# joedownard/skill-chaining-with-graphs

Hardware: AMD Instinct MI355X
Metric: env-steps/sec (whole node), 65 536 parallel Pinball envs at 1/2/4/8 MI355X (higher is better)
Workload: dtype f32

## Files before the change

### include/scg_abi.h

```cpp
#ifndef SCG_ABI_H
#define SCG_ABI_H
#include <stdint.h>

#ifdef __cplusplus
extern "C" {
#endif

#define SCG_ABI_VERSION 5
#define SCG_NUM_ACTIONS 5
#define SCG_FOURIER_ORDER 5
#define SCG_NUM_FEATURES 1296
#define SCG_MAX_OPTIONS 5
#define SCG_MAX_EDGES 256
#define SCG_CLF_STRIDE 8

typedef enum {
    SCG_OK = 0,
    SCG_ERR_INVALID = -1,
    SCG_ERR_NO_DEVICE = -2,
    SCG_ERR_HIP = -3,
    SCG_ERR_STATE = -4,
    SCG_ERR_ASYNC = -5
} scg_status;

typedef struct scg_ctx scg_ctx;

typedef struct {
    int32_t n_envs;
    int32_t n_options;
    int32_t fourier_order;
    int32_t device;
    int64_t env_id_base;
    uint64_t seed;
    float gamma, alpha, epsilon, r_option_success;
    int32_t max_episode_steps, max_option_steps;
    int32_t update_count_floor;
    int32_t reoffer_period;
} scg_config;

#define SCG_STEP_LEARN 1u
#define SCG_STEP_APPLY 2u
#define SCG_STEP_INTERRUPT 4u

int scg_abi_version(void);
int scg_block_envs(void);
const char *scg_strerror(int status);
const char *scg_last_error(const scg_ctx *ctx);

int scg_create(scg_ctx **out, const scg_config *cfg);
int scg_destroy(scg_ctx *ctx);
int scg_set_hparams(scg_ctx *ctx, float gamma, float alpha, float epsilon, float r_option_success,
                    int32_t max_episode_steps, int32_t max_option_steps, int32_t update_count_floor, int32_t reoffer_period);

int scg_set_map(scg_ctx *ctx, const float *edges, int32_t n_edges, const float *starts, int32_t n_starts,
                const float map_scalars[6], const float *scale);

int scg_step(scg_ctx *ctx, float *x, float *y, float *vx, float *vy, int32_t *option_id,
             int32_t *opt_steps, int32_t *ep_steps, float *qcache, uint8_t *action, float *reward,
             uint8_t *done, float *W, const float *clf, uint32_t enabled_mask, uint64_t t,
             uint32_t flags, void *stream);

typedef struct {
    float *ep_return;
    double *ret_sum;
    int32_t *episodes, *goals, *len_sum;
    int32_t *vf_steps, *entries, *declines, *successes;
    uint8_t *finished;
} scg_rollout_stats;
#define SCG_ROLLOUT_BEGIN 1u
#define SCG_ROLLOUT_ONE_EPISODE 2u
#define SCG_ROLLOUT_MAX_STEPS 1024
int scg_rollout(scg_ctx *ctx, float *x, float *y, float *vx, float *vy, int32_t *option_id, int32_t *opt_steps,
                int32_t *ep_steps, float *qcache, uint8_t *action, float *reward, uint8_t *done,
                const float *W, const float *clf, uint32_t enabled_mask, uint64_t t0, int32_t n_steps,
                uint32_t flags, const scg_rollout_stats *stats, void *stream);

typedef struct {
    uint8_t *outcome;
    int32_t *steps;
    float *ret, *disc_ret, *v0, *end_x, *end_y, *end_vx, *end_vy;
} scg_trial_out;
#define SCG_TRIAL_SUCCESS 1u
#define SCG_TRIAL_EPISODE_END 2u
#define SCG_TRIAL_LEFT_INITIATION 3u
#define SCG_TRIAL_TIMEOUT 4u
#define SCG_TRIAL_MAX_STEPS SCG_ROLLOUT_MAX_STEPS
int scg_option_trials(scg_ctx *ctx, int32_t n, const float *x, const float *y, const float *vx, const float *vy,
                      const int32_t *option, const float *W, const float *clf, uint32_t enabled_mask, uint64_t t0,
                      const scg_trial_out *out, void *stream);

typedef struct {
    int32_t first, n, rows;
    int32_t *len;
    float *x, *y, *vx, *vy, *reward;
    uint8_t *action, *done, *vf, *term;
    int8_t *option_id;
} scg_record;
#define SCG_ROLLOUT_BEGIN_AT 4u
int scg_rollout_record(scg_ctx *ctx, float *x, float *y, float *vx, float *vy, int32_t *option_id, int32_t *opt_steps,
                       int32_t *ep_steps, float *qcache, uint8_t *action, float *reward, uint8_t *done,
                       const float *W, const float *clf, uint32_t enabled_mask, uint64_t t0, int32_t n_steps,
                       uint32_t flags, const scg_rollout_stats *stats, const scg_record *rec, void *stream);
int scg_option_trials_record(scg_ctx *ctx, int32_t n, const float *x, const float *y, const float *vx, const float *vy,
                             const int32_t *option, const float *W, const float *clf, uint32_t enabled_mask, uint64_t t0,
                             const scg_trial_out *out, const scg_record *rec, void *stream);

#define SCG_ROLLOUT_TERM_INTERRUPTED 5u
int scg_rollout_interrupt(scg_ctx *ctx, float *x, float *y, float *vx, float *vy, int32_t *option_id, int32_t *opt_steps,
                          int32_t *ep_steps, float *qcache, uint8_t *action, float *reward, uint8_t *done,
                          const float *W, const float *clf, uint32_t enabled_mask, uint64_t t0, int32_t n_steps,
                          uint32_t flags, const scg_rollout_stats *stats, int32_t *interrupts, const scg_record *rec,
                          void *stream);

int scg_grad_buffers(scg_ctx *ctx, float **G, int32_t **n_k);
int scg_set_grad_buffers(scg_ctx *ctx, float *G, int32_t *n_k);
int scg_apply_update(scg_ctx *ctx, float *W, const float *G, const int32_t *n_k, void *stream);
int scg_set_grad_buffer_packed(scg_ctx *ctx, float *G_packed);
int scg_apply_update_packed(scg_ctx *ctx, float *W, const float *G_packed, void *stream);
int scg_apply_update_slots(scg_ctx *ctx, float *W, const float *slots, int32_t n_slots, int64_t slot_stride, void *stream);

int scg_peer_export(scg_ctx *ctx, void *handle_out);
int scg_peer_open(scg_ctx *ctx, int32_t n_ranks, int32_t rank, const void *handles);
int scg_peer_exchange_apply(scg_ctx *ctx, float *W, void *stream);


int scg_pinball_step(scg_ctx *ctx, int32_t n, float *x, float *y, float *vx, float *vy,
                     const uint8_t *action, float *reward, uint8_t *goal, void *stream);
int scg_fourier_features(scg_ctx *ctx, int32_t n, const float *x, const float *y, const float *vx,
                         const float *vy, float *phi, void *stream);
int scg_q_values(scg_ctx *ctx, int32_t n, const float *x, const float *y, const float *vx,
                 const float *vy, const float *Wk, float *q, void *stream);
int scg_q_update(scg_ctx *ctx, int32_t n, int32_t k, const float *x, const float *y, const float *vx,
                 const float *vy, const uint8_t *action, const float *r, const float *cont,
                 const float *xn, const float *yn, const float *vxn, const float *vyn, float *W,
                 uint32_t flags, void *stream);
int scg_classifier_predict(scg_ctx *ctx, int32_t n, const float *x, const float *y, const float *w8,
                           uint8_t *out, void *stream);
int scg_fit_initiation(scg_ctx *ctx, int32_t n_fit, const float *xy, const uint8_t *label,
                       const int32_t *offsets, float *w, int32_t iters, float lr, float l2, void *stream);

int scg_set_option_parents(scg_ctx *ctx, const int32_t *parents);

int scg_invalidate_order(scg_ctx *ctx);

int scg_set_trace_buffers(scg_ctx *ctx, float *ring_x, float *ring_y, int32_t ring_len, uint8_t *events,
                          int32_t *ev_len);
int scg_harvest(scg_ctx *ctx, int32_t n_sel, const int32_t *sel_env, const float *ring_x, const float *ring_y,
                int32_t ring_len, const int32_t *ev_len, int32_t l_pos, int32_t l_neg, float *out_xy,
                uint8_t *out_label, void *stream);

int scg_collect_examples(scg_ctx *ctx, uint32_t event_bits, uint8_t *prev_in, int32_t l_pos, int32_t l_neg,
                         float *ex_xy, uint8_t *ex_label, int32_t *count, int32_t cap, void *stream);
int scg_arm_collect(scg_ctx *ctx, uint32_t event_bits, const uint8_t *prev_in, int32_t l_pos, int32_t l_neg, const int32_t *count);
int scg_collect_frontier(scg_ctx *ctx, uint32_t target_mask, uint32_t cover_mask, const float *clf, int32_t l_pos, int32_t l_neg,
                         float *ex_xy, uint8_t *ex_label, int32_t *count, int32_t cap, void *stream);

int scg_set_gestation(scg_ctx *ctx, uint32_t gest_mask, int32_t *succ_counts);

#define SCG_ASYNC_FIT_TIMEOUT 0x1u
#define SCG_ASYNC_STEP_HANDOFF 0x2u
#define SCG_ASYNC_PEER_TIMEOUT 0x4u
int scg_async_status(scg_ctx *ctx, void *stream, int32_t synchronize, uint32_t *word_out);
int scg_clear_async_error(scg_ctx *ctx);
int scg_set_fit_timeout(scg_ctx *ctx, double seconds);
int scg_set_peer_timeout(scg_ctx *ctx, double seconds);
int scg_decode_async_word(uint32_t word, char *buf, int32_t buf_len);
int scg_debug_raise_async(scg_ctx *ctx, uint32_t word);

int scg_profile_reset(scg_ctx *ctx, int32_t enable);
int scg_profile_read(scg_ctx *ctx, double *kernel_ms_sum, int64_t *launches);

#ifdef __cplusplus
}
#endif
#endif
```

### skill-chaining-with-graphs_amd/_lib.py

```python
from __future__ import annotations

import ctypes as C
import os

_HERE = os.path.dirname(os.path.abspath(__file__))
LIB_PATH = os.environ.get("SCG_LIB") or os.path.join(_HERE, "csrc", "libscg_hip.so")

NUM_ACTIONS = 5
FOURIER_ORDER = 5
NUM_FEATURES = 1296
MAX_OPTIONS = 5
MAX_EDGES = 256
CLF_STRIDE = 8

STEP_LEARN = 1
STEP_APPLY = 2
STEP_INTERRUPT = 4
ROLLOUT_BEGIN = 1
ROLLOUT_ONE_EPISODE = 2
ROLLOUT_BEGIN_AT = 4
ROLLOUT_MAX_STEPS = 1024
TRIAL_SUCCESS = 1
TRIAL_EPISODE_END = 2
TRIAL_LEFT_INITIATION = 3
TRIAL_TIMEOUT = 4
TRIAL_MAX_STEPS = ROLLOUT_MAX_STEPS
ROLLOUT_TERM_INTERRUPTED = 5
ABI_VERSION = 5
ASYNC_FIT_TIMEOUT = 0x1
ASYNC_STEP_HANDOFF = 0x2
ASYNC_PEER_TIMEOUT = 0x4
PEER_HANDLE_BYTES = 64
PEER_MAX_RANKS = 8


class ScgError(RuntimeError):
    pass


class ScgConfig(C.Structure):
    _fields_ = [
        ("n_envs", C.c_int32),
        ("n_options", C.c_int32),
        ("fourier_order", C.c_int32),
        ("device", C.c_int32),
        ("env_id_base", C.c_int64),
        ("seed", C.c_uint64),
        ("gamma", C.c_float),
        ("alpha", C.c_float),
        ("epsilon", C.c_float),
        ("r_option_success", C.c_float),
        ("max_episode_steps", C.c_int32),
        ("max_option_steps", C.c_int32),
        ("update_count_floor", C.c_int32),
        ("reoffer_period", C.c_int32),
    ]


class RolloutStats(C.Structure):
    _fields_ = [
        ("ep_return", C.c_void_p),
        ("ret_sum", C.c_void_p),
        ("episodes", C.c_void_p),
        ("goals", C.c_void_p),
        ("len_sum", C.c_void_p),
        ("vf_steps", C.c_void_p),
        ("entries", C.c_void_p),
        ("declines", C.c_void_p),
        ("successes", C.c_void_p),
        ("finished", C.c_void_p),
    ]


class TrialOut(C.Structure):
    _fields_ = [
        ("outcome", C.c_void_p),
        ("steps", C.c_void_p),
        ("ret", C.c_void_p),
        ("disc_ret", C.c_void_p),
        ("v0", C.c_void_p),
        ("end_x", C.c_void_p),
        ("end_y", C.c_void_p),
        ("end_vx", C.c_void_p),
        ("end_vy", C.c_void_p),
    ]


class Record(C.Structure):
    _fields_ = [
        ("first", C.c_int32),
        ("n", C.c_int32),
        ("rows", C.c_int32),
        ("len", C.c_void_p),
        ("x", C.c_void_p),
        ("y", C.c_void_p),
        ("vx", C.c_void_p),
        ("vy", C.c_void_p),
        ("reward", C.c_void_p),
        ("action", C.c_void_p),
        ("done", C.c_void_p),
        ("vf", C.c_void_p),
        ("term", C.c_void_p),
        ("option_id", C.c_void_p),
    ]


_P = C.c_void_p
_SIGS = {
    "scg_abi_version": (C.c_int, []),
    "scg_block_envs": (C.c_int, []),
    "scg_strerror": (C.c_char_p, [C.c_int]),
    "scg_last_error": (C.c_char_p, [_P]),
    "scg_create": (C.c_int, [C.POINTER(_P), C.POINTER(ScgConfig)]),
    "scg_destroy": (C.c_int, [_P]),
    "scg_set_hparams": (C.c_int, [_P, C.c_float, C.c_float, C.c_float, C.c_float, C.c_int32, C.c_int32, C.c_int32, C.c_int32]),
    "scg_set_map": (C.c_int, [_P, _P, C.c_int32, _P, C.c_int32, _P, _P]),
    "scg_step": (C.c_int, [_P] + [_P] * 13 + [C.c_uint32, C.c_uint64, C.c_uint32, _P]),
    "scg_rollout": (C.c_int, [_P] + [_P] * 13 + [C.c_uint32, C.c_uint64, C.c_int32, C.c_uint32, C.POINTER(RolloutStats), _P]),
    "scg_option_trials": (C.c_int, [_P, C.c_int32] + [_P] * 7 + [C.c_uint32, C.c_uint64, C.POINTER(TrialOut), _P]),
    "scg_rollout_record": (C.c_int, [_P] + [_P] * 13 + [C.c_uint32, C.c_uint64, C.c_int32, C.c_uint32, C.POINTER(RolloutStats),
                                                         C.POINTER(Record), _P]),
    "scg_option_trials_record": (C.c_int, [_P, C.c_int32] + [_P] * 7 + [C.c_uint32, C.c_uint64, C.POINTER(TrialOut),
                                                                       C.POINTER(Record), _P]),
    "scg_rollout_interrupt": (C.c_int, [_P] + [_P] * 13 + [C.c_uint32, C.c_uint64, C.c_int32, C.c_uint32, C.POINTER(RolloutStats),
                                                            _P, C.POINTER(Record), _P]),
    "scg_grad_buffers": (C.c_int, [_P, C.POINTER(_P), C.POINTER(_P)]),
    "scg_set_grad_buffers": (C.c_int, [_P, _P, _P]),
    "scg_apply_update": (C.c_int, [_P, _P, _P, _P, _P]),
    "scg_set_grad_buffer_packed": (C.c_int, [_P, _P]),
    "scg_apply_update_packed": (C.c_int, [_P, _P, _P, _P]),
    "scg_apply_update_slots": (C.c_int, [_P, _P, _P, C.c_int32, C.c_int64, _P]),
    "scg_pinball_step": (C.c_int, [_P, C.c_int32] + [_P] * 7 + [_P]),
    "scg_fourier_features": (C.c_int, [_P, C.c_int32] + [_P] * 5 + [_P]),
    "scg_q_values": (C.c_int, [_P, C.c_int32] + [_P] * 6 + [_P]),
    "scg_q_update": (C.c_int, [_P, C.c_int32, C.c_int32] + [_P] * 12 + [C.c_uint32, _P]),
    "scg_classifier_predict": (C.c_int, [_P, C.c_int32] + [_P] * 4 + [_P]),
    "scg_set_option_parents": (C.c_int, [_P, _P]),
    "scg_invalidate_order": (C.c_int, [_P]),
    "scg_set_trace_buffers": (C.c_int, [_P, _P, _P, C.c_int32, _P, _P]),
    "scg_harvest": (C.c_int, [_P, C.c_int32, _P, _P, _P, C.c_int32, _P, C.c_int32, C.c_int32, _P, _P, _P]),
    "scg_collect_examples": (C.c_int, [_P, C.c_uint32, _P, C.c_int32, C.c_int32, _P, _P, _P, C.c_int32, _P]),
    "scg_arm_collect": (C.c_int, [_P, C.c_uint32, _P, C.c_int32, C.c_int32, _P]),
    "scg_collect_frontier": (C.c_int, [_P, C.c_uint32, C.c_uint32, _P, C.c_int32, C.c_int32, _P, _P, _P, C.c_int32, _P]),
    "scg_set_gestation": (C.c_int, [_P, C.c_uint32, _P]),
    "scg_profile_reset": (C.c_int, [_P, C.c_int32]),
    "scg_profile_read": (C.c_int, [_P, C.POINTER(C.c_double), C.POINTER(C.c_int64)]),
    "scg_fit_initiation": (C.c_int, [_P, C.c_int32, _P, _P, _P, _P, C.c_int32, C.c_float, C.c_float, _P]),
    "scg_async_status": (C.c_int, [_P, _P, C.c_int32, C.POINTER(C.c_uint32)]),
    "scg_clear_async_error": (C.c_int, [_P]),
    "scg_set_fit_timeout": (C.c_int, [_P, C.c_double]),
    "scg_set_peer_timeout": (C.c_int, [_P, C.c_double]),
    "scg_peer_export": (C.c_int, [_P, _P]),
    "scg_peer_open": (C.c_int, [_P, C.c_int32, C.c_int32, _P]),
    "scg_peer_exchange_apply": (C.c_int, [_P, _P, _P]),
    "scg_decode_async_word": (C.c_int, [C.c_uint32, C.c_char_p, C.c_int32]),
    "scg_debug_raise_async": (C.c_int, [_P, C.c_uint32]),
}
EXPORTED_SYMBOLS = tuple(_SIGS)

BLOCK_ENVS_DEFAULT = 256
BLOCK_ENVS_BUILDS = (64, 128, 256)

CHIP_CUS = 256


def auto_block_envs(n_envs: int) -> int:
    for b in BLOCK_ENVS_BUILDS:
        if -(-int(n_envs) // b) <= CHIP_CUS:
            return b
    return BLOCK_ENVS_DEFAULT


_libs = {}


def lib_path(block_envs: int | None = None) -> str:
    if block_envs in (None, BLOCK_ENVS_DEFAULT):
        return LIB_PATH
    if block_envs not in BLOCK_ENVS_BUILDS:
        raise ScgError(f"block_envs must be one of {BLOCK_ENVS_BUILDS}")
    return os.path.join(_HERE, "csrc", f"libscg_hip_b{block_envs}.so")


def load(block_envs: int | None = None, path: str | None = None) -> C.CDLL:
    key = (BLOCK_ENVS_DEFAULT if block_envs is None else int(block_envs)) if path is None else os.path.abspath(path)
    if key in _libs:
        return _libs[key]
    if path is None:
        path = lib_path(key)
    if not os.path.exists(path):
        raise ScgError(
            f"{path} is missing: the HIP extension has not been built "
            "(run `python -c 'import __graft_entry__ as g; g.build()'` or `make -C "
            f"{os.path.dirname(path)}`). There is no CPU fallback."
        )
    lib = C.CDLL(path)
    try:
        ver = int(lib.scg_abi_version())
    except AttributeError:
        raise ScgError(f"{path} does not export scg_abi_version: not a libscg_hip.so") from None
    if ver != ABI_VERSION:
        raise ScgError(f"{path} implements ABI version {ver}, this binding expects {ABI_VERSION} "
                       "(include/scg_abi.h): rebuild the library (a stale .so?)")
    for name, (res, args) in _SIGS.items():
        try:
            fn = getattr(lib, name)
        except AttributeError:
            raise ScgError(f"{path} does not export {name} although it reports ABI version {ver}: rebuild it") from None
        fn.restype = res
        fn.argtypes = args
    if block_envs is not None and isinstance(key, int) and int(lib.scg_block_envs()) != key:
        raise ScgError(f"{path} is built for {int(lib.scg_block_envs())}-env blocks, not {key}: rebuild it")
    _libs[key] = lib
    return lib


def block_envs(block_envs: int | None = None) -> int:
    return int(load(block_envs).scg_block_envs())


def check(status: int, ctx=None, what: str = "") -> None:
    if status == 0:
        return
    lib = load()
    msg = lib.scg_last_error(ctx).decode() if True else ""
    raise ScgError(f"{what or 'scg call'} failed ({lib.scg_strerror(status).decode()}): {msg}")
```

### skill-chaining-with-graphs_amd/core.py

```python
from __future__ import annotations

import ctypes as C
import os
from typing import Optional, Sequence

import numpy as np
import torch

from . import _lib
from ._lib import (CLF_STRIDE, MAX_OPTIONS, NUM_ACTIONS, NUM_FEATURES, STEP_APPLY, STEP_INTERRUPT, STEP_LEARN, ScgConfig,
                   ScgError)
from .maps import PinballMap


def fourier_scale_table(order: int = 5, n_vars: int = 4) -> np.ndarray:
    n = order + 1
    idx = np.arange(n ** n_vars)
    c = np.stack([(idx // n ** (n_vars - 1 - d)) % n for d in range(n_vars)], 1).astype(np.float64)
    norm = np.sqrt((c * c).sum(1))
    norm[0] = 1.0
    return (1.0 / norm).astype(np.float32)


def _ptr(t: Optional[torch.Tensor]) -> C.c_void_p:
# ... 259 lines not shown
        self._chk(count, torch.int32, 1, "count")
        if prev_in is not None:
            self._chk(prev_in, torch.uint8, self.n_envs, "prev_in")
        if l_pos < 0 or l_neg < 0 or l_pos + l_neg < 1 or not (0 < event_bits < 64):
            raise ScgError("collect_examples: bad argument")
        self._call("scg_collect_examples", C.c_uint32(event_bits), _ptr(prev_in), l_pos, l_neg, _ptr(ex_xy), _ptr(ex_label),
                   _ptr(count), cap, self._stream())
        if rearm:
            self._call("scg_arm_collect", C.c_uint32(event_bits), _ptr(prev_in), l_pos, l_neg, _ptr(count))
            self._armed = (prev_in, count)
        else:
            self.disarm_collect()

    def collect_frontier(self, target_mask: int, cover_mask: int, clf: torch.Tensor, l_pos: int, l_neg: int,
                         ex_xy: torch.Tensor, ex_label: torch.Tensor, count: torch.Tensor) -> None:
        if getattr(self, "_trace", None) is None:
            raise ScgError("collect_frontier: trace buffers are not attached (set_trace_buffers)")
        cap = ex_label.numel() // self.n_vf
        if cap < 1 or ex_label.numel() != self.n_vf * cap:
            raise ScgError(f"collect_frontier: ex_label must hold n_vf = {self.n_vf} buffers of cap >= 1 examples")
        self._chk(ex_xy, torch.float32, 2 * self.n_vf * cap, "ex_xy"); self._chk(ex_label, torch.uint8, self.n_vf * cap, "ex_label")
        self._chk(count, torch.int32, self.n_vf, "count"); self._chk(clf, torch.float32, self.n_vf * CLF_STRIDE, "clf")
        nodes = (1 << self.n_vf) - 1
        if l_pos < 0 or l_neg < 0 or l_pos + l_neg < 1 or not (0 <= target_mask <= nodes) or not (0 <= cover_mask <= nodes) \
                or cover_mask & 1 or target_mask & ~cover_mask & ~1:
            raise ScgError("collect_frontier: bad argument")
        self._call("scg_collect_frontier", C.c_uint32(target_mask), C.c_uint32(cover_mask), _ptr(clf), l_pos, l_neg, _ptr(ex_xy),
                   _ptr(ex_label), _ptr(count), cap, self._stream())

    def disarm_collect(self) -> None:
        self._call("scg_arm_collect", C.c_uint32(0), None, 0, 0, None)
        self._armed = None

    def set_gestation(self, gest_mask: int) -> torch.Tensor:
        if not hasattr(self, "_gest_succ"):
            self._gest_succ = torch.zeros(self.n_vf, dtype=torch.int32, device=self.device)
        self._call("scg_set_gestation", C.c_uint32(gest_mask), _ptr(self._gest_succ))
        self.gest_mask = gest_mask
        return self._gest_succ

    def grad_buffers(self):
        if not hasattr(self, "_gbuf"):
            G = torch.zeros((self.n_vf, NUM_ACTIONS, NUM_FEATURES), dtype=torch.float32, device=self.device)
            n = torch.zeros((self.n_vf,), dtype=torch.int32, device=self.device)
            self._call("scg_set_grad_buffers", _ptr(G), _ptr(n))
            self._gbuf = (G, n)
            self.__dict__.pop("_gpacked", None)
        return self._gbuf

    def grad_packed(self) -> torch.Tensor:
        if not hasattr(self, "_gpacked"):
            gp = torch.zeros(self.n_vf * NUM_ACTIONS * NUM_FEATURES + self.n_vf, dtype=torch.float32, device=self.device)
            self._call("scg_set_grad_buffer_packed", _ptr(gp))
            self._gpacked = gp
            self.__dict__.pop("_gbuf", None)
        return self._gpacked

    def apply_update_packed(self, W: torch.Tensor, gp: torch.Tensor) -> None:
        self._chk(W, torch.float32, self.n_vf * NUM_ACTIONS * NUM_FEATURES, "W")
        self._chk(gp, torch.float32, self.n_vf * NUM_ACTIONS * NUM_FEATURES + self.n_vf, "G_packed")
        self._call("scg_apply_update_packed", _ptr(W), _ptr(gp), self._stream())

    def apply_update_slots(self, W: torch.Tensor, slots: torch.Tensor) -> None:
        per = self.n_vf * NUM_ACTIONS * NUM_FEATURES + self.n_vf
        if slots.dim() != 2 or slots.shape[1] != per or not slots.is_contiguous():
            raise ScgError(f"slots must be a contiguous [n_ranks, {per}] tensor")
        self._chk(W, torch.float32, self.n_vf * NUM_ACTIONS * NUM_FEATURES, "W")
        self._chk(slots, torch.float32, slots.shape[0] * per, "slots")
        self._call("scg_apply_update_slots", _ptr(W), _ptr(slots), C.c_int32(slots.shape[0]), C.c_int64(per), self._stream())

    def apply_update(self, W: torch.Tensor, G: torch.Tensor, n_k: torch.Tensor) -> None:
        self._chk(W, torch.float32, self.n_vf * NUM_ACTIONS * NUM_FEATURES, "W")
        self._chk(G, torch.float32, self.n_vf * NUM_ACTIONS * NUM_FEATURES, "G")
        self._chk(n_k, torch.int32, self.n_vf, "n_k")
        self._call("scg_apply_update", _ptr(W), _ptr(G), _ptr(n_k), self._stream())

    def _chk4(self, s: Sequence[torch.Tensor], n: int, name: str):
        if len(s) != 4:
            raise ScgError(f"{name}: need (x, y, vx, vy)")
        return [self._chk(t, torch.float32, n, f"{name}[{i}]") for i, t in enumerate(s)]

    def pinball_step(self, s, action: torch.Tensor):
        n = s[0].numel()
        x, y, vx, vy = self._chk4(s, n, "state")
        self._chk(action, torch.uint8, n, "action")
        if n and int(action.max()) >= NUM_ACTIONS:
            raise ScgError("action out of range [0, 5)")
        reward = torch.empty(n, dtype=torch.float32, device=self.device)
        goal = torch.empty(n, dtype=torch.uint8, device=self.device)
        self._call("scg_pinball_step", n, _ptr(x), _ptr(y), _ptr(vx), _ptr(vy), _ptr(action), _ptr(reward),
                   _ptr(goal), self._stream())
        return reward, goal

    def features(self, s) -> torch.Tensor:
        n = s[0].numel()
        x, y, vx, vy = self._chk4(s, n, "state")
        phi = torch.empty((n, NUM_FEATURES), dtype=torch.float32, device=self.device)
        self._call("scg_fourier_features", n, _ptr(x), _ptr(y), _ptr(vx), _ptr(vy), _ptr(phi), self._stream())
        return phi

    def q_values(self, s, Wk: torch.Tensor) -> torch.Tensor:
        n = s[0].numel()
        x, y, vx, vy = self._chk4(s, n, "state")
        self._chk(Wk, torch.float32, NUM_ACTIONS * NUM_FEATURES, "Wk")
        q = torch.empty((NUM_ACTIONS, n), dtype=torch.float32, device=self.device)
        self._call("scg_q_values", n, _ptr(x), _ptr(y), _ptr(vx), _ptr(vy), _ptr(Wk), _ptr(q), self._stream())
        return q

    def q_update(self, k: int, s, action, r, cont, sn, W: torch.Tensor, apply: bool = True) -> None:
        n = s[0].numel()
        if n > self.n_envs:
            raise ScgError("q_update: more transitions than the context's n_envs")
        x, y, vx, vy = self._chk4(s, n, "s")
        xn, yn, vxn, vyn = self._chk4(sn, n, "s_next")
        self._chk(action, torch.uint8, n, "action"); self._chk(r, torch.float32, n, "r")
        self._chk(cont, torch.float32, n, "cont")
        self._chk(W, torch.float32, self.n_vf * NUM_ACTIONS * NUM_FEATURES, "W")
        if n and int(action.max()) >= NUM_ACTIONS:
            raise ScgError("action out of range [0, 5)")
        self._call("scg_q_update", n, k, _ptr(x), _ptr(y), _ptr(vx), _ptr(vy), _ptr(action), _ptr(r), _ptr(cont),
                   _ptr(xn), _ptr(yn), _ptr(vxn), _ptr(vyn), _ptr(W), C.c_uint32(STEP_APPLY if apply else 0),
                   self._stream())

    def classifier_predict(self, x: torch.Tensor, y: torch.Tensor, w8: torch.Tensor) -> torch.Tensor:
        n = x.numel()
        self._chk(x, torch.float32, n, "x"); self._chk(y, torch.float32, n, "y")
        self._chk(w8, torch.float32, CLF_STRIDE, "w8")
        out = torch.empty(n, dtype=torch.uint8, device=self.device)
        self._call("scg_classifier_predict", n, _ptr(x), _ptr(y), _ptr(w8), _ptr(out), self._stream())
        return out

    def fit_initiation(self, xy: torch.Tensor, label: torch.Tensor, offsets: torch.Tensor, w: torch.Tensor,
                       iters: int = 200, lr: float = 1.0, l2: float = 1e-4) -> None:
        n_fit = offsets.numel() - 1
        self._chk(offsets, torch.int32, n_fit + 1, "offsets")
        off = offsets.cpu()
        m = int(off[-1])
        if n_fit < 0 or int(off[0]) != 0 or bool((off[1:] < off[:-1]).any()):
            raise ScgError("offsets must start at 0 and be non-decreasing")
        self._chk(xy, torch.float32, 2 * m, "xy"); self._chk(label, torch.uint8, m, "label")
        self._chk(w, torch.float32, n_fit * CLF_STRIDE, "w")
        self._call("scg_fit_initiation", n_fit, _ptr(xy), _ptr(label), _ptr(offsets), _ptr(w), iters,
                   C.c_float(lr), C.c_float(l2), self._stream())
        self.async_status(synchronize=True)

    def async_status(self, synchronize: bool = False) -> int:
        word = C.c_uint32(0)
        self._call("scg_async_status", self._stream(), 1 if synchronize else 0, C.byref(word))
        return int(word.value)

    def clear_async_error(self) -> None:
        self._call("scg_clear_async_error")

    def set_fit_timeout(self, seconds: float) -> None:
        self._call("scg_set_fit_timeout", C.c_double(seconds))

    def peer_export(self) -> bytes:
        buf = C.create_string_buffer(_lib.PEER_HANDLE_BYTES)
        self._call("scg_peer_export", C.cast(buf, C.c_void_p))
        return buf.raw

    def peer_open(self, n_ranks: int, rank: int, handles) -> None:
        handles = [bytes(h) for h in handles]
        if len(handles) != n_ranks or any(len(h) != _lib.PEER_HANDLE_BYTES for h in handles):
            raise ScgError(f"peer_open: need {n_ranks} handles of {_lib.PEER_HANDLE_BYTES} bytes")
        blob = C.create_string_buffer(b"".join(handles), n_ranks * _lib.PEER_HANDLE_BYTES)
        self._call("scg_peer_open", C.c_int32(n_ranks), C.c_int32(rank), C.cast(blob, C.c_void_p))
        self.peer_ranks = int(n_ranks)

    def peer_exchange_apply(self, W: torch.Tensor) -> None:
        self._chk(W, torch.float32, self.n_vf * NUM_ACTIONS * NUM_FEATURES, "W")
        self._call("scg_peer_exchange_apply", _ptr(W), self._stream())

    def set_peer_timeout(self, seconds: float) -> None:
        self._call("scg_set_peer_timeout", C.c_double(seconds))

    @property
    def step_grid(self) -> int:
        return -(-self.n_envs // self.block_envs)


class EnvState:

    def __init__(self, n: int, device: torch.device, pmap: PinballMap):
        z = lambda dt: torch.zeros(n, dtype=dt, device=device)
        sx, sy = float(pmap.starts[0][0]), float(pmap.starts[0][1])
        self.n = n
        self.x = torch.full((n,), sx, dtype=torch.float32, device=device)
        self.y = torch.full((n,), sy, dtype=torch.float32, device=device)
        self.vx, self.vy = z(torch.float32), z(torch.float32)
        self.option_id, self.opt_steps, self.ep_steps = z(torch.int32), z(torch.int32), z(torch.int32)
        self.qcache = torch.zeros((NUM_ACTIONS, n), dtype=torch.float32, device=device)
        self.action, self.done = z(torch.uint8), z(torch.uint8)
        self.reward = z(torch.float32)

    def state(self):
        return (self.x, self.y, self.vx, self.vy)
```

### skill-chaining-with-graphs_amd/csrc/scg_kernels.hip

```cpp
#include "scg_device.hpp"
#include "../../include/scg_abi.h"
#include <cstdio>
#include <cstdlib>
#include <cstring>
#include <cmath>
#include <mutex>
#include <new>
#include <type_traits>
#include <vector>

using namespace scg;
typedef float f4v __attribute__((ext_vector_type(4)));
typedef unsigned u4v __attribute__((ext_vector_type(4)));

template <typename T>
__device__ __forceinline__ void gstore(T *p, T v) { *p = v; }

__device__ __forceinline__ void store_wt(float *p, f4v v) {
    asm volatile("global_store_dwordx4 %0, %1, off sc1\n\ts_nop 2" :: "v"(p), "v"(v) : "memory");
}

constexpr int OREC = 4;

struct StepArgs {
    float *x, *y, *vx, *vy;
    int32_t *option_id, *opt_steps, *ep_steps;
    int32_t *hist_next;
    float4 *qalt;
    float4 *outrec;
    float *qcache;
    uint8_t *action;
    float *reward;
    uint8_t *done;
    const float *cont_in;
    const float *xn, *yn, *vxn, *vyn;
    const float *W;
    const float *clf;
    const float *edges;
    const uint64_t *cellmask;
    const int32_t *perm;
    float *ring_x, *ring_y;
    uint8_t *events;
    int32_t *ev_len;
    int32_t ring_mask;
    const float *starts;
    float *slabs;
    int32_t *cnts;
    unsigned long long *stamps;
    uint32_t *async_word;
    int32_t *fail_flag;
    int32_t n, n_vf, k_lo, k_hi;
    uint32_t enabled, learn;
    uint32_t gest;
    int32_t *gest_succ;
    uint32_t parents;
    uint64_t t, seed;
    int64_t env_base;
    float gamma, epsilon, r_succ;
    int32_t max_ep, max_opt;
    uint32_t reoffer_mask;
    MapScalars ms;
};

__device__ __forceinline__ void block_lds_sync() {
    asm volatile("s_waitcnt lgkmcnt(0)\n\ts_barrier" ::: "memory");
}

__device__ __forceinline__ bool in_set(const StepArgs &A, int k, float x, float y) {
    if (k < 1 || k >= A.n_vf) return false;
    if (!((A.enabled >> k) & 1u)) return false;
    return clf_z(A.clf + CLF_STRIDE * k, x, y) > 0.0f;
}

#include "scg_eval.hpp"
#include "scg_step_kernel.hpp"
#include "scg_rollout_kernel.hpp"
#include "scg_trial_kernel.hpp"

__attribute__((visibility("hidden"))) hipError_t launch_rollout_record(const RolloutRecArgs &A, int grid, hipStream_t s);
__attribute__((visibility("hidden"))) hipError_t launch_trial_record(const TrialRecArgs &A, int grid, hipStream_t s);
__attribute__((visibility("hidden"))) hipError_t launch_rollout_interrupt(const RolloutIntArgs &A, int grid, hipStream_t s);
__attribute__((visibility("hidden"))) hipError_t launch_rollout_interrupt_record(const RolloutIntRecArgs &A, int grid, hipStream_t s);

struct ReduceArgs {
    const float *slabs;
    const int32_t *cnts;
    float *G;
    int32_t *n_k;
    float *nk_f;
    float *W;
    const float *scale;
    int32_t nblk, n_vf;
    float alpha;
    uint32_t apply;
    int32_t nk_floor;
    const int32_t *option_id;
    int32_t *hist, *hist_zero, *perm;
    int32_t n, nrow;
    const float4 *outrec;
    const float4 *qalt;
    int32_t *invperm;
    float *x, *y, *vx, *vy, *reward;
    int32_t *option_id_out, *opt_steps, *ep_steps;
    uint8_t *action, *done;
    float *qcache;
    int32_t sort;
    const int32_t *fail_flag;
    const uint8_t *c_events, *c_prev;
    const int32_t *c_evlen, *c_count;
    int32_t *c_rows;
    uint32_t c_bits;
    int32_t c_L, c_ring_len;
};

constexpr int SEG = 16;
constexpr int RED_WAVES = 16;
constexpr int RED_THREADS = 64 * RED_WAVES;
constexpr int RED_SPW = 2;
constexpr int RED_COLS = NACT * NF / 4;
constexpr int RED_NCOL = (RED_COLS + 63) / 64;

__device__ __forceinline__ uint32_t div_magic(uint32_t d) { return 0xFFFFFFFFu / d + 1u; }
__device__ __forceinline__ int div_by(int r, int d, uint32_t m) { return d == 1 ? r : (int)__umulhi((uint32_t)r, m); }
__device__ __forceinline__ int collect_v(int e, int n, const uint8_t *events, const uint8_t *prev_in, uint32_t bits,
                                         const int32_t *ev_len, int ring_len, int L, bool &in_out);
constexpr int NKEY = 7, HSTRIDE = 8;
__device__ __forceinline__ int sort_key(int o, int n_vf) {
    if (o <= 0) return o > -n_vf ? 0 : n_vf;
    return o < n_vf ? o : n_vf;
}
struct OrderLayout {
    int chunked, c, g, U, Ftot;
    uint32_t mc, mg;
    int start[NKEY];
    int cnt[NKEY], n[NKEY], F[NKEY];
    int pad_lo[NKEY], pad_n[NKEY], pad_pos[NKEY], tail_lo, tail_pos;
};
__device__ __forceinline__ void order_layout(const int tot[NKEY], int n_envs, OrderLayout &L) {
    int S = 0, Rn = 0;
#pragma unroll
    for (int k = 1; k < NKEY; ++k) { S += tot[k]; Rn += tot[k] > 0 ? 1 : 0; L.n[k] = tot[k]; }
    L.n[0] = tot[0];
    const int Bf = n_envs / BLOCK_ENVS;
    int c = BLOCK_ENVS;
    if (Bf > Rn && S > 0) c = min(BLOCK_ENVS, (S + (Bf - Rn) - 1) / (Bf - Rn));
    int U = 0, F = 0;
    L.start[0] = 0; L.cnt[0] = 0; L.F[0] = 0;
    L.mc = div_magic((uint32_t)c);
    L.mg = div_magic((uint32_t)max(BLOCK_ENVS - c, 1));
#pragma unroll
    for (int k = 1; k < NKEY; ++k) {
        L.cnt[k] = div_by(tot[k] + c - 1, c, L.mc);
        L.start[k] = U * BLOCK_ENVS; L.F[k] = F;
        U += L.cnt[k]; F += L.cnt[k] * BLOCK_ENVS - tot[k];
    }
    L.c = c; L.g = BLOCK_ENVS - c; L.U = U; L.Ftot = F;
    L.chunked = (U * BLOCK_ENVS <= n_envs) ? 1 : 0;
    if (!L.chunked) {
        int P = 0, used = 0;
        L.c = 1 << 30;
        L.mc = div_magic(1u << 30);
        L.pad_lo[0] = 0; L.pad_n[0] = 0; L.pad_pos[0] = 0;
#pragma unroll
        for (int k = 1; k < NKEY; ++k) {
            L.start[k] = P; P += tot[k];
            const int need = tot[k] > 0 ? (BLOCK_ENVS - P % BLOCK_ENVS) % BLOCK_ENVS : 0;
            const int pad = min(need, tot[0] - used);
            L.pad_lo[k] = used; L.pad_n[k] = pad; L.pad_pos[k] = P; used += pad; P += pad;
        }
        L.tail_lo = used; L.tail_pos = P;
    }
}
__device__ __forceinline__ int order_posk(const OrderLayout &L, int start, int r) {
    const int t = div_by(r, L.c, L.mc);
    return start + BLOCK_ENVS * t + (r - t * L.c);
}
__device__ __forceinline__ int order_pos0(const OrderLayout &L, int r) {
    if (!L.chunked) {
        int pos = L.tail_pos + (r - L.tail_lo);
#pragma unroll
        for (int k = 1; k < NKEY; ++k)
            if (r >= L.pad_lo[k] && r < L.pad_lo[k] + L.pad_n[k]) pos = L.pad_pos[k] + (r - L.pad_lo[k]);
        return pos;
    }
    int pos = L.U * BLOCK_ENVS + (r - L.Ftot);
    int st = 0, cn = 0, nk = 0, f0 = 0;
    bool in_run = false;
#pragma unroll
    for (int k = 1; k < NKEY; ++k) {
        const int fills = L.cnt[k] * BLOCK_ENVS - L.n[k];
        if (r >= L.F[k] && r < L.F[k] + fills) { in_run = true; st = L.start[k]; cn = L.cnt[k]; nk = L.n[k]; f0 = L.F[k]; }
    }
    if (in_run) {
        const int rp = r - f0, nfull = cn - 1;
        if (L.g > 0 && rp < nfull * L.g) {
            const int t = div_by(rp, L.g, L.mg);
            pos = st + BLOCK_ENVS * t + L.c + (rp - t * L.g);
        } else {
            pos = st + BLOCK_ENVS * nfull + (nk - nfull * L.c) + (rp - nfull * L.g);
        }
    }
    return pos;
}

__device__ __forceinline__ void commit_and_place_row(const ReduceArgs &R, int row, int wv, int lane, int (*s_x)[40]) {
    int zoff = 0;
    asm volatile("" : "+v"(zoff));
    const int step_failed = R.fail_flag[zoff];
    const bool act = wv < 4 && row < R.nrow;
    const int e = row * 256 + wv * 64 + lane;
    const bool ok = act && e < R.n;
    const int pos_old = ok ? R.invperm[e] : 0;
    int tot[NKEY], pre[NKEY];
#pragma unroll
    for (int k = 0; k < NKEY; ++k) { tot[k] = 0; pre[k] = 0; }
    if (act && R.sort) {
        for (int r = wv * 64 + lane; r < R.nrow; r += 256) {
#pragma unroll
            for (int k = 0; k < NKEY; ++k) {
                const int h = R.hist[r * HSTRIDE + k];
                tot[k] += h;
                if (r < row) pre[k] += h;
            }
        }
    }
    float4 ra = make_float4(0.0f, 0.0f, 0.0f, 0.0f), rb = ra, rq = ra;
    float q4 = 0.0f;
    if (ok) {
        const float4 *r = R.outrec + (size_t)pos_old * OREC;
        const float4 r3 = r[3];
        ra = r[0]; rb = r[1]; rq = r[2]; q4 = r3.x;
        if (__float_as_uint(r3.y) == OREC_DECLINED) {
            rq = R.qalt[(size_t)pos_old * 2]; q4 = R.qalt[(size_t)pos_old * 2 + 1].x;
            rb.y = __uint_as_float(__float_as_uint(rb.y) | 0x01000000u);
        }
    }
    int key = -1;
    uint64_t km[NKEY];
    if (act) {
        if (R.sort) {
#pragma unroll
            for (int k = 0; k < NKEY; ++k) {
#pragma unroll
                for (int m = 1; m < 64; m <<= 1) { tot[k] += __shfl_xor(tot[k], m, 64); pre[k] += __shfl_xor(pre[k], m, 64); }
            }
        }
        const unsigned bits = __float_as_uint(rb.y);
        if (ok && !step_failed) {
            const int on = (int)((bits >> 16) & 255u);
            const bool declined = (bits >> 24) & 1u;
            const int oid = declined ? -on : (on ? on : -(int)((bits >> 28) & 7u));
            key = sort_key(oid, R.n_vf);
            R.x[e] = ra.x; R.y[e] = ra.y; R.vx[e] = ra.z; R.vy[e] = ra.w;
            R.reward[e] = rb.x; R.action[e] = (uint8_t)(bits & 255u); R.done[e] = (uint8_t)((bits >> 8) & 255u);
            R.option_id_out[e] = oid; R.opt_steps[e] = __float_as_int(rb.z); R.ep_steps[e] = __float_as_int(rb.w);
            if (R.qcache) {
                const size_t n = (size_t)R.n;
                R.qcache[e] = rq.x; R.qcache[n + e] = rq.y; R.qcache[2 * n + e] = rq.z;
                R.qcache[3 * n + e] = rq.w; R.qcache[4 * n + e] = q4;
            }
        }
        if (R.sort) {
#pragma unroll
            for (int k = 0; k < NKEY; ++k) km[k] = __ballot(key == k);
            if (lane < 3 * NKEY) {
                int v = 0;
#pragma unroll
                for (int k = 0; k < NKEY; ++k) {
                    if (lane == k) v = tot[k];
                    if (lane == NKEY + k) v = pre[k];
                    if (lane == 2 * NKEY + k) v = __popcll(km[k]);
                }
                s_x[wv][lane] = v;
            }
        }
    }
    if (R.c_rows && act) {
        bool in;
        int v = collect_v(e, R.n, R.c_events, R.c_prev, R.c_bits, R.c_evlen, R.c_ring_len, R.c_L, in);
#pragma unroll
        for (int m = 1; m < 64; m <<= 1) v += __shfl_xor(v, m, 64);
        if (lane == 0) s_x[wv][3 * NKEY] = v;
    }
    if (!R.sort && !R.c_rows) return;
    __syncthreads();
    if (R.c_rows && wv == 0 && lane == 0 && row < R.nrow) {
        R.c_rows[row] = s_x[0][3 * NKEY] + s_x[1][3 * NKEY] + s_x[2][3 * NKEY] + s_x[3][3 * NKEY];
        if (row == 0) R.c_rows[R.nrow] = *R.c_count;
    }
    if (!R.sort || !act) return;
    int off[NKEY];
#pragma unroll
    for (int k = 0; k < NKEY; ++k) {
        tot[k] = s_x[0][k] + s_x[1][k] + s_x[2][k] + s_x[3][k];
        off[k] = s_x[0][NKEY + k] + s_x[1][NKEY + k] + s_x[2][NKEY + k] + s_x[3][NKEY + k];
#pragma unroll
        for (int w = 0; w < 3; ++w) off[k] += w < wv ? s_x[w][2 * NKEY + k] : 0;
    }
    OrderLayout L;
    order_layout(tot, R.n, L);
    int rk = -1, st = 0;
#pragma unroll
    for (int k = 0; k < NKEY; ++k)
        if (key == k) { rk = off[k] + __popcll(km[k] & ((1ull << lane) - 1ull)); st = L.start[k]; }
    if (rk >= 0 && !step_failed) {
        const int pos = key == 0 ? order_pos0(L, rk) : order_posk(L, st, rk);
        R.perm[pos] = e; R.invperm[e] = pos;
    }
    if (wv == 0 && lane < HSTRIDE) R.hist_zero[row * HSTRIDE + lane] = 0;
}

template <int BATCH>
__global__ __launch_bounds__(RED_THREADS, BATCH == 16 ? 4 : 8) void reduce_kernel(const ReduceArgs R) {
    __shared__ float4 s_T[RED_WAVES * RED_SPW][64];
    __shared__ int s_cnt[RED_WAVES * RED_SPW];
    __shared__ int s_x[4][40];
    const int sy_rows = (int)gridDim.y - R.n_vf;
    const int k = (int)blockIdx.y >= sy_rows ? (int)blockIdx.y - sy_rows : -1;
    const int rowy = (int)blockIdx.y;
    const int tid = threadIdx.x, lane = tid & 63, wave = __builtin_amdgcn_readfirstlane(tid >> 6);
    if (k < 0) {
        const int row = rowy * (int)gridDim.x + blockIdx.x;
        commit_and_place_row(R, row, wave, lane, s_x);
        return;
    }
    const int i4 = blockIdx.x * 64 + lane;
    const bool live = i4 < RED_COLS;
    const size_t slab_stride = (size_t)R.n_vf * RED_COLS * sizeof(float4);
    const char *slab_k = reinterpret_cast<const char *>(R.slabs) + (size_t)k * RED_COLS * sizeof(float4);
    const unsigned col_off = (unsigned)(live ? i4 : 0) * (unsigned)sizeof(float4);
    const int nseg = (R.nblk + SEG - 1) / SEG;
    float4 S = make_float4(0.0f, 0.0f, 0.0f, 0.0f);
    int nk = 0;
    float4 w_old = make_float4(0.0f, 0.0f, 0.0f, 0.0f), sc = w_old;
    int step_failed = 0;
    for (int sg0 = 0; sg0 < nseg; sg0 += RED_WAVES * RED_SPW) {
        int cs[RED_SPW];
#pragma unroll
        for (int j = 0; j < RED_SPW; ++j) {
            const int bl = (sg0 + j * RED_WAVES + wave) * SEG + lane;
            cs[j] = (lane < SEG && bl < R.nblk) ? R.cnts[(unsigned)(bl * R.n_vf + k)] : 0;
        }
#pragma unroll
        for (int j = 0; j < RED_SPW; ++j) {
            const int b0 = (sg0 + j * RED_WAVES + wave) * SEG;
            int c = cs[j];
            const unsigned mask = (unsigned)__ballot(c > 0);
#pragma unroll
            for (int m = 1; m < SEG; m <<= 1) c += __shfl_xor(c, m, 64);
            float4 T = make_float4(0.0f, 0.0f, 0.0f, 0.0f);
            if (mask) {
                const __amdgpu_buffer_rsrc_t seg = __builtin_amdgcn_make_buffer_rsrc(
                    const_cast<char *>(slab_k + (size_t)b0 * slab_stride), 0, 0x7fffffff, 0x00020000);
#pragma unroll
                for (int h = 0; h < SEG; h += BATCH) {
                    if (!((mask >> h) & ((1u << BATCH) - 1u))) continue;
                    u4v v[BATCH];
#pragma unroll
                    for (int u = 0; u < BATCH; ++u) {
                        v[u] = (u4v){0u, 0u, 0u, 0u};
                        if ((mask >> (h + u)) & 1u) v[u] = __builtin_amdgcn_raw_buffer_load_b128(seg, (int)col_off, (int)((h + u) * (unsigned)slab_stride), 0);
                    }
#pragma unroll
                    for (int u = 0; u < BATCH; ++u) {
                        if ((mask >> (h + u)) & 1u) {
                            T.x = T.x + __uint_as_float(v[u][0]); T.y = T.y + __uint_as_float(v[u][1]);
                            T.z = T.z + __uint_as_float(v[u][2]); T.w = T.w + __uint_as_float(v[u][3]);
                        }
                    }
                }
            }
            s_T[j * RED_WAVES + wave][lane] = T;
            if (lane == 0) s_cnt[j * RED_WAVES + wave] = c;
        }
        if (wave == 0 && R.apply && sg0 + RED_WAVES * RED_SPW >= nseg) {
            step_failed = *R.fail_flag;
            int col = live ? i4 : 0;
            asm volatile("" : "+v"(col));
            w_old = reinterpret_cast<const float4 *>(R.W)[(size_t)k * RED_COLS + col];
            sc = *reinterpret_cast<const float4 *>(R.scale + (col * 4) % NF);
        }
        __syncthreads();
        if (wave == 0) {
#pragma unroll
            for (int u = 0; u < RED_WAVES * RED_SPW; ++u) {
                const int cu = s_cnt[u];
                if (cu > 0) {
                    const float4 t = s_T[u][lane];
                    S.x = S.x + t.x; S.y = S.y + t.y; S.z = S.z + t.z; S.w = S.w + t.w;
                    nk += cu;
                }
            }
        }
        __syncthreads();
    }
    if (wave != 0) return;
    if (blockIdx.x == 0 && lane == 0) {
        R.n_k[k] = nk;
        if (R.nk_f) R.nk_f[k] = (float)nk;
    }
    if (!live) return;
    reinterpret_cast<float4 *>(R.G)[(size_t)k * RED_COLS + i4] = S;
    if (R.apply && nk > 0 && !step_failed) {
        const float step = R.alpha / (float)max(nk, R.nk_floor);
        float4 w = w_old;
        w.x = fmaf(step * sc.x, S.x, w.x); w.y = fmaf(step * sc.y, S.y, w.y);
        w.z = fmaf(step * sc.z, S.z, w.z); w.w = fmaf(step * sc.w, S.w, w.w);
        int col = i4;
        asm volatile("" : "+v"(col));
        reinterpret_cast<float4 *>(R.W)[(size_t)k * RED_COLS + col] = w;
    }
}

__global__ __launch_bounds__(256) void commit_kernel(const ReduceArgs R) {
    __shared__ int s_x[4][40];
    commit_and_place_row(R, blockIdx.x, threadIdx.x >> 6, threadIdx.x & 63, s_x);
}

__global__ __launch_bounds__(256) void apply_kernel(float *W, const float *G, const int32_t *n_k, const float *nk_f,
                                                    const float *scale, float alpha, int nk_floor) {
    const int k = blockIdx.y;
    const int i = blockIdx.x * 256 + threadIdx.x;
    if (i >= NACT * NF) return;
    const int nk = n_k ? n_k[k] : (int)(nk_f[k] + 0.5f);
    if (nk <= 0) return;
    const float step = alpha / (float)max(nk, nk_floor);
    const int f = i % NF;
    float *w = W + (size_t)k * NACT * NF + i;
    *w = fmaf(step * scale[f], G[(size_t)k * NACT * NF + i], *w);
}

__global__ __launch_bounds__(256) void apply_slots_kernel(float *W, const float *slots, int n_slots, long stride, int n_vf,
                                                          const float *scale, float alpha, int nk_floor) {
    const int k = blockIdx.y;
    const int i = blockIdx.x * 256 + threadIdx.x;
    if (i >= NACT * NF) return;
    const size_t at = (size_t)k * NACT * NF + i, cnt_at = (size_t)n_vf * NACT * NF + k;
    float g = slots[at], nkf = slots[cnt_at];
    for (int r = 1; r < n_slots; ++r) {
        g = g + slots[(size_t)r * stride + at];
        nkf = nkf + slots[(size_t)r * stride + cnt_at];
    }
    const int nk = (int)(nkf + 0.5f);
    if (nk <= 0) return;
    const float step = alpha / (float)max(nk, nk_floor);
    float *w = W + at;
    *w = fmaf(step * scale[i % NF], g, *w);
}

constexpr int PEER_MAX = 8;
constexpr size_t PEER_HDR = 256;

struct PeerView {
    const float *buf[PEER_MAX][2];
    const uint32_t *epoch[PEER_MAX];
    const uint32_t *voidw[PEER_MAX];
};

__device__ __forceinline__ bool epoch_reached(uint32_t v, uint32_t need) { return (int32_t)(v - need) >= 0; }

__global__ __launch_bounds__(64) void peer_publish_kernel(uint32_t *epoch, uint32_t *voidw, int parity, const int32_t *fail,
                                                          uint32_t value) {
    if (threadIdx.x != 0) return;
    const int32_t f = __hip_atomic_load(fail, __ATOMIC_RELAXED, __HIP_MEMORY_SCOPE_AGENT);
    __hip_atomic_store(&voidw[parity], f ? 1u : 0u, __ATOMIC_RELAXED, __HIP_MEMORY_SCOPE_SYSTEM);
    __builtin_amdgcn_fence(__ATOMIC_RELEASE, "");
    asm volatile("s_waitcnt vmcnt(0)" ::: "memory");
    __hip_atomic_store(epoch, value, __ATOMIC_RELAXED, __HIP_MEMORY_SCOPE_SYSTEM);
}

__global__ __launch_bounds__(64) void peer_wait_kernel(const PeerView P, int n_ranks, int parity, uint32_t need,
                                                       unsigned long long timeout_ticks, int32_t *go, uint32_t *async_word) {
    const int lane = threadIdx.x;
    bool late = false, voided = false;
    if (lane < n_ranks) {
        unsigned long long t0 = 0;
        int spins = 0;
        while (!epoch_reached(__hip_atomic_load(P.epoch[lane], __ATOMIC_RELAXED, __HIP_MEMORY_SCOPE_SYSTEM), need)) {
            __builtin_amdgcn_s_sleep(2);
            if ((++spins & 63) == 0) {
                const unsigned long long now = __builtin_amdgcn_s_memrealtime();
                if (t0 == 0) t0 = now;
                else if (now - t0 > timeout_ticks) { late = true; break; }
            }
        }
    }
    __builtin_amdgcn_fence(__ATOMIC_ACQUIRE, "");
    if (lane < n_ranks && !late)
        voided = __hip_atomic_load(&P.voidw[lane][parity], __ATOMIC_RELAXED, __HIP_MEMORY_SCOPE_SYSTEM) != 0u;
    const bool any_late = __ballot(late) != 0, any_void = __ballot(voided) != 0;
    if (lane == 0) {
        if (any_late) __hip_atomic_fetch_or(async_word, SCG_ASYNC_PEER_TIMEOUT, __ATOMIC_RELAXED, __HIP_MEMORY_SCOPE_SYSTEM);
        else if (any_void) __hip_atomic_fetch_or(async_word, SCG_ASYNC_STEP_HANDOFF, __ATOMIC_RELAXED, __HIP_MEMORY_SCOPE_SYSTEM);
        __hip_atomic_store(go, (any_late || any_void) ? 0 : 1, __ATOMIC_RELAXED, __HIP_MEMORY_SCOPE_AGENT);
    }
}

__global__ __launch_bounds__(256) void apply_peers_kernel(float *W, const PeerView P, int n_ranks, int parity, uint32_t need,
                                                          const int32_t *go, int n_vf, const float *scale, float alpha,
                                                          int nk_floor) {
    __shared__ int s_ok;
    if (threadIdx.x == 0) {
        int ok = __hip_atomic_load(go, __ATOMIC_RELAXED, __HIP_MEMORY_SCOPE_AGENT);
        for (int r = 0; r < n_ranks; ++r)
            ok &= epoch_reached(__hip_atomic_load(P.epoch[r], __ATOMIC_RELAXED, __HIP_MEMORY_SCOPE_SYSTEM), need) ? 1 : 0;
        __builtin_amdgcn_fence(__ATOMIC_ACQUIRE, "");
        s_ok = ok;
    }
    __syncthreads();
    if (!s_ok) return;
    const int k = blockIdx.y;
    const int i = blockIdx.x * 256 + threadIdx.x;
    if (i >= NACT * NF) return;
    const size_t at = (size_t)k * NACT * NF + i, cnt_at = (size_t)n_vf * NACT * NF + k;
    float g = P.buf[0][parity][at], nkf = P.buf[0][parity][cnt_at];
    for (int r = 1; r < n_ranks; ++r) {
        g = g + P.buf[r][parity][at];
        nkf = nkf + P.buf[r][parity][cnt_at];
    }
    const int nk = (int)(nkf + 0.5f);
    if (nk <= 0) return;
    const float step = alpha / (float)max(nk, nk_floor);
    float *w = W + at;
    *w = fmaf(step * scale[i % NF], g, *w);
}

__global__ __launch_bounds__(256) void sort_hist_kernel(const int32_t *option_id, int n, int n_vf, int32_t *hist) {
    __shared__ int s_c[4][HSTRIDE];
    const int tid = threadIdx.x, lane = tid & 63, wave = tid >> 6;
    const int e = blockIdx.x * 256 + tid;
    const int o = e < n ? sort_key(option_id[e], n_vf) : -1;
#pragma unroll
    for (int k = 0; k < NKEY; ++k) {
        const uint64_t m = __ballot(o == k);
        if (lane == 0) s_c[wave][k] = __popcll(m);
    }
    __syncthreads();
    if (tid < NKEY) hist[blockIdx.x * HSTRIDE + tid] = s_c[0][tid] + s_c[1][tid] + s_c[2][tid] + s_c[3][tid];
}

__global__ __launch_bounds__(256) void sort_scatter_kernel(const int32_t *option_id, int n, int n_vf, int nblk,
                                                           const int32_t *hist, int32_t *perm, int32_t *invperm) {
    __shared__ int s_c[4][HSTRIDE];
    __shared__ int s_off[HSTRIDE];
    const int tid = threadIdx.x, lane = tid & 63, wave = tid >> 6, b = blockIdx.x;
    __shared__ int s_tot[HSTRIDE], s_pre[HSTRIDE], s_part[4][2 * HSTRIDE];
    int tot[NKEY], pre[NKEY];
#pragma unroll
    for (int kk = 0; kk < NKEY; ++kk) { tot[kk] = 0; pre[kk] = 0; }
    for (int bb0 = 0; bb0 < nblk; bb0 += 256) {
        const int bb = bb0 + tid;
        if (bb < nblk) {
#pragma unroll
            for (int kk = 0; kk < NKEY; ++kk) {
                const int h = hist[bb * HSTRIDE + kk];
                tot[kk] += h;
                if (bb < b) pre[kk] += h;
            }
        }
    }
#pragma unroll
    for (int kk = 0; kk < NKEY; ++kk) {
#pragma unroll
        for (int m = 1; m < 64; m <<= 1) { tot[kk] += __shfl_xor(tot[kk], m, 64); pre[kk] += __shfl_xor(pre[kk], m, 64); }
        if (lane == 0) { s_part[wave][kk] = tot[kk]; s_part[wave][HSTRIDE + kk] = pre[kk]; }
    }
    __syncthreads();
    if (tid < NKEY) {
        s_tot[tid] = s_part[0][tid] + s_part[1][tid] + s_part[2][tid] + s_part[3][tid];
// ... 264 lines not shown
}

__global__ __launch_bounds__(64) void features_kernel(int n, const float *x, const float *y, const float *vx,
                                                      const float *vy, float *phi) {
    __shared__ float2 s_pw[20];
    __shared__ float2 s_abcd[72];
    const int lane = threadIdx.x;
    for (int e = blockIdx.x; e < n; e += gridDim.x) {
        if (lane == 0) state_powers(x[e], y[e], vx[e], vy[e], s_pw);
        wave_lds_sync();
        for (int p = lane; p < 72; p += 64) {
            const int q = p % 36, d0 = p < 36 ? 0 : 2;
            float2 v = pow_at(s_pw, d0 + 1, q % 6);
            for (int c = 1; c <= q / 6; ++c) v = cmul(v, pow_at(s_pw, d0, 1));
            s_abcd[p] = v;
        }
        wave_lds_sync();
        for (int f = lane; f < NF; f += 64) {
            const float2 ab = s_abcd[f / 36], cd = s_abcd[36 + f % 36];
            phi[(size_t)e * NF + f] = fmaf(-ab.y, cd.y, ab.x * cd.x);
        }
        wave_lds_sync();
    }
}

__global__ __launch_bounds__(256) void predict_kernel(int n, const float *x, const float *y, const float *w8,
                                                      uint8_t *out) {
    const int e = blockIdx.x * 256 + threadIdx.x;
    if (e < n) out[e] = clf_z(w8, x[e], y[e]) > 0.0f ? 1 : 0;
}

constexpr int FIT_G = 8, FIT_T = 1024, FIT_EPT = 8, FIT_BATCH = 8;
constexpr int FIT_STRIDE = FIT_G * FIT_T;

__global__ __launch_bounds__(FIT_T) void fit_kernel(const float *xy, const uint8_t *label, const int32_t *offsets,
                                                    float *w, int iters, float lr, float l2, int q0,
                                                    unsigned long long *part, unsigned long long timeout_ticks,
                                                    uint32_t *async_word) {
    __shared__ float sw[8];
    __shared__ float swave[FIT_T / 64][6];
    __shared__ int s_abort;
    const int ql = blockIdx.y, q = q0 + ql, j = blockIdx.x;
    const int tid = threadIdx.x, lane = tid & 63, wave = tid >> 6;
    const int i0 = offsets[q], M = offsets[q + 1] - offsets[q];
    if (M <= 0) return;
    if (tid < 8) sw[tid] = w[CLF_STRIDE * q + tid];
    if (tid == 0) s_abort = 0;
    const int gamma = j * FIT_T + tid;
    float cu[FIT_EPT], cv[FIT_EPT], cl[FIT_EPT];
#pragma unroll
    for (int e = 0; e < FIT_EPT; ++e) {
        const int i = gamma + FIT_STRIDE * e;
        cu[e] = 0.0f; cv[e] = 0.0f; cl[e] = 0.0f;
        if (i < M) {
            cu[e] = fmaf(xy[2 * (size_t)(i0 + i)], 2.0f, -1.0f);
            cv[e] = fmaf(xy[2 * (size_t)(i0 + i) + 1], 2.0f, -1.0f);
            cl[e] = (float)label[i0 + i];
        }
    }
    const float invM = 1.0f / (float)M;
    unsigned long long *my_part = part + (size_t)ql * 2 * FIT_G * 8;
    for (int it = 0; it < iters; ++it) {
        __syncthreads();
        float wl[6];
#pragma unroll
        for (int jj = 0; jj < 6; ++jj) wl[jj] = sw[jj];
        float g[6] = {0.0f, 0.0f, 0.0f, 0.0f, 0.0f, 0.0f};
        auto one = [&](float u, float v, float lbl) {
            const float psi[6] = {1.0f, u, v, u * u, u * v, v * v};
            float z = wl[0];
            z = fmaf(wl[1], u, z); z = fmaf(wl[2], v, z);
            z = fmaf(wl[3], psi[3], z); z = fmaf(wl[4], psi[4], z); z = fmaf(wl[5], psi[5], z);
            const float e = sigmoid_spec(z) - lbl;
#pragma unroll
            for (int jj = 0; jj < 6; ++jj) g[jj] = fmaf(e, psi[jj], g[jj]);
        };
#pragma unroll
        for (int e = 0; e < FIT_EPT; ++e)
            if (gamma + FIT_STRIDE * e < M) one(cu[e], cv[e], cl[e]);
        for (int i = gamma + FIT_STRIDE * FIT_EPT; i < M; i += FIT_STRIDE)
            one(fmaf(xy[2 * (size_t)(i0 + i)], 2.0f, -1.0f), fmaf(xy[2 * (size_t)(i0 + i) + 1], 2.0f, -1.0f), (float)label[i0 + i]);
#pragma unroll
        for (int jj = 0; jj < 6; ++jj) {
            g[jj] = wave_sum(g[jj]);
            if (lane == 0) swave[wave][jj] = g[jj];
        }
        __syncthreads();
        unsigned long long *buf = my_part + (it & 1) * FIT_G * 8;
        const unsigned long long tag = (unsigned long long)(unsigned)(it + 1) << 32;
        if (tid < 6) {
            float ps = swave[0][tid];
#pragma unroll
            for (int wv = 1; wv < FIT_T / 64; ++wv) ps = ps + swave[wv][tid];
            __hip_atomic_store(&buf[j * 8 + tid], tag | __float_as_uint(ps), __ATOMIC_RELAXED, __HIP_MEMORY_SCOPE_AGENT);
        }
        if (wave == 0) {
            unsigned long long v = tag;
            if (lane < 6 * FIT_G) {
                const unsigned long long *src = &buf[(lane / 6) * 8 + lane % 6];
                unsigned long long t0 = 0;
                int spins = 0;
                while (((v = __hip_atomic_load(src, __ATOMIC_RELAXED, __HIP_MEMORY_SCOPE_AGENT)) >> 32) != (tag >> 32)) {
                    __builtin_amdgcn_s_sleep(1);
                    if ((++spins & 255) == 0) {
                        const unsigned long long now = __builtin_amdgcn_s_memrealtime();
                        if (t0 == 0) t0 = now;
                        else if (now - t0 > timeout_ticks) { s_abort = 1; break; }
                    }
                }
            }
            const float val = __uint_as_float((unsigned)v);
            const int c = lane < 6 ? lane : 0;
            float gs = __shfl(val, c, 64);
#pragma unroll
            for (int jw = 1; jw < FIT_G; ++jw) gs = gs + __shfl(val, jw * 6 + c, 64);
            if (lane < 6) {
                const float reg = (lane > 0) ? l2 * sw[lane] : 0.0f;
                sw[lane] = sw[lane] - lr * ((gs * invM) + reg);
            }
        }
        __syncthreads();
        if (s_abort) break;
    }
    __syncthreads();
    if (s_abort) {
        if (j == 0 && tid == 0 && async_word)
            __hip_atomic_fetch_or(async_word, SCG_ASYNC_FIT_TIMEOUT | (0x100u << (q & 15)), __ATOMIC_RELAXED, __HIP_MEMORY_SCOPE_SYSTEM);
        return;
    }
    if (j == 0 && tid < 6) w[CLF_STRIDE * q + tid] = sw[tid];
}

struct scg_ctx {
    scg_config cfg;
    int n_vf;
    int nblk;
    int n_cu;
    bool have_map;
    MapScalars ms;
    float *d_edges, *d_starts, *d_scale;
    uint64_t *d_cellmask;
    int32_t *d_perm, *d_hist;
    int32_t *d_collect_rows;
    int32_t *d_frontier_rows;
    uint32_t arm_bits;
    const uint8_t *arm_prev;
    const int32_t *arm_count;
    int32_t arm_L;
    bool arm_rows_ready;
    unsigned long long *d_fit_part;
    uint32_t *h_async;
    uint32_t *d_async;
    int32_t *d_fail;
    double fit_timeout_s;
    float4 *d_outrec;
    float4 *d_qalt;
    int32_t *d_invperm;
    int32_t *d_hist2[2];
    int hist_parity;
    bool hist_dirty;
    bool order_valid;
    const int32_t *order_ids;
    uint32_t parents;
    uint32_t gest;
    int32_t *gest_succ;
    float *ring_x, *ring_y;
    uint8_t *events;
    int32_t *ev_len;
    int32_t ring_len;
    unsigned long long *d_stamps;
    float *d_slabs;
    int32_t *d_cnts;
    float *d_G;
    int32_t *d_nk;
    float *G_out;
    int32_t *nk_out;
    float *nkf_out;
    bool prof_on;
    int prof_every;
    long long prof_seen;
    std::vector<hipEvent_t> *prof_ev;
    size_t prof_used;
    char *peer_region;
    size_t peer_bytes, peer_op_stride;
    hipIpcMemHandle_t peer_handle;
    int peer_n, peer_rank;
    char *peer_base[PEER_MAX];
    bool peer_mapped[PEER_MAX];
    uint32_t peer_e;
    int32_t *d_peer_go;
    double peer_timeout_s;
    char err[256];
};

static std::mutex g_peer_mu;
static std::vector<std::pair<hipIpcMemHandle_t, char *>> g_peer_regions;

static thread_local char g_err[256] = "";

#define SCG_HIP(ctx, call)                                                                     \
    do {                                                                                       \
        hipError_t e_ = (call);                                                                \
        if (e_ != hipSuccess) {                                                                \
            snprintf((ctx) ? (ctx)->err : g_err, 256, "%s failed: %s", #call, hipGetErrorString(e_)); \
            return SCG_ERR_HIP;                                                                \
        }                                                                                      \
    } while (0)

static int fail(scg_ctx *ctx, int code, const char *msg) {
    snprintf(ctx ? ctx->err : g_err, 256, "%s", msg);
    return code;
}

static int decode_async(uint32_t word, char *buf, size_t n) {
    if (word == 0) { if (buf && n) buf[0] = 0; return SCG_OK; }
    if (buf && n) {
        if (word & SCG_ASYNC_STEP_HANDOFF)
            snprintf(buf, n, "an earlier scg_step gave up inside a workgroup: a bounded hand-off poll between its wavefront subsets ran "
                     "out (a logic error or a hung wavefront); the block's partial gradients were dropped and the step's outputs for "
                     "its envs are unspecified — restore the state. scg_clear_async_error() re-arms the context");
        else if (word & SCG_ASYNC_PEER_TIMEOUT)
            snprintf(buf, n, "an earlier scg_peer_exchange_apply gave up: the peer wait ran out (a peer rank did not publish its "
                     "operand within the peer timeout: stopped, hung or out of step); the weights were left unchanged. "
                     "scg_clear_async_error() re-arms the context");
        else if (word & SCG_ASYNC_FIT_TIMEOUT)
            snprintf(buf, n, "an earlier scg_fit_initiation gave up (problem mask 0x%x): its workgroups did not become "
                     "co-resident within the fit timeout (card shared with other work?); the affected classifier rows were "
                     "left unchanged. scg_clear_async_error() re-arms the context", (word >> 8) & 0xffffu);
        else
            snprintf(buf, n, "unknown asynchronous device status 0x%x", word);
    }
    return SCG_ERR_ASYNC;
}
static int async_pending(scg_ctx *c);
#define SCG_CHECK_ASYNC(c) do { if (async_pending(c)) return SCG_ERR_ASYNC; } while (0)

struct DeviceGuard {
    int prev = -1;
    bool ok = true;
    explicit DeviceGuard(int dev) {
        int cur = -1;
        if (hipGetDevice(&cur) != hipSuccess) { ok = false; return; }
        if (cur != dev) {
            if (hipSetDevice(dev) != hipSuccess) { ok = false; return; }
            prev = cur;
        }
    }
    ~DeviceGuard() { if (prev >= 0) (void)hipSetDevice(prev); }
    DeviceGuard(const DeviceGuard &) = delete;
    DeviceGuard &operator=(const DeviceGuard &) = delete;
};
#define SCG_ON_DEVICE(c, what)                                                                   \
    DeviceGuard dev_guard_((c)->cfg.device);                                                     \
    if (!dev_guard_.ok) return fail((c), SCG_ERR_HIP, what ": cannot make the context's device current")

static int async_pending(scg_ctx *c) {
    if (!c || !c->h_async) return 0;
    const uint32_t w = *reinterpret_cast<volatile uint32_t *>(c->h_async);
    if (w == 0) return 0;
    decode_async(w, c->err, sizeof(c->err));
    return 1;
}

extern "C" {

int scg_abi_version(void) { return SCG_ABI_VERSION; }

int scg_decode_async_word(uint32_t word, char *buf, int32_t buf_len) {
    return decode_async(word, buf, buf_len > 0 ? (size_t)buf_len : 0);
}

int scg_async_status(scg_ctx *c, void *stream, int32_t synchronize, uint32_t *word_out) {
    if (!c) return fail(nullptr, SCG_ERR_INVALID, "scg_async_status: null ctx");
    if (synchronize) {
        SCG_ON_DEVICE(c, "scg_async_status");
        SCG_HIP(c, hipStreamSynchronize(reinterpret_cast<hipStream_t>(stream)));
    }
    const uint32_t w = c->h_async ? *reinterpret_cast<volatile uint32_t *>(c->h_async) : 0u;
    if (word_out) *word_out = w;
    return decode_async(w, c->err, sizeof(c->err));
}

int scg_clear_async_error(scg_ctx *c) {
    if (!c) return fail(nullptr, SCG_ERR_INVALID, "scg_clear_async_error: null ctx");
    if (c->h_async) *reinterpret_cast<volatile uint32_t *>(c->h_async) = 0u;
    if (c->d_fail) {
        DeviceGuard g(c->cfg.device);
        if (g.ok) (void)hipMemset(c->d_fail, 0, sizeof(int32_t));
    }
    c->order_valid = false; c->hist_dirty = true; c->arm_rows_ready = false;
    return SCG_OK;
}

int scg_set_fit_timeout(scg_ctx *c, double seconds) {
    if (!c) return fail(nullptr, SCG_ERR_INVALID, "scg_set_fit_timeout: null ctx");
    if (!(seconds >= 0.0) || seconds > 3600.0) return fail(c, SCG_ERR_INVALID, "scg_set_fit_timeout: seconds must be in [0, 3600]");
    c->fit_timeout_s = seconds;
    return SCG_OK;
}

int scg_set_peer_timeout(scg_ctx *c, double seconds) {
    if (!c) return fail(nullptr, SCG_ERR_INVALID, "scg_set_peer_timeout: null ctx");
    if (!(seconds >= 0.0) || seconds > 3600.0) return fail(c, SCG_ERR_INVALID, "scg_set_peer_timeout: seconds must be in [0, 3600]");
    c->peer_timeout_s = seconds;
    return SCG_OK;
}

int scg_debug_raise_async(scg_ctx *c, uint32_t word) {
    if (!c || !c->h_async) return fail(c, SCG_ERR_INVALID, "scg_debug_raise_async: null ctx");
    *reinterpret_cast<volatile uint32_t *>(c->h_async) |= word;
    return SCG_OK;
}

int scg_block_envs(void) { return BLOCK_ENVS; }

const char *scg_strerror(int status) {
    switch (status) {
        case SCG_OK: return "ok";
        case SCG_ERR_INVALID: return "invalid argument";
        case SCG_ERR_NO_DEVICE: return "no usable HIP device";
        case SCG_ERR_HIP: return "HIP runtime error";
        case SCG_ERR_STATE: return "call order / state error";
        case SCG_ERR_ASYNC: return "an earlier launch failed on the device";
        default: return "unknown status";
    }
}

const char *scg_last_error(const scg_ctx *ctx) { return ctx ? ctx->err : g_err; }

int scg_create(scg_ctx **out, const scg_config *cfg) {
    if (!out || !cfg) return fail(nullptr, SCG_ERR_INVALID, "scg_create: null argument");
    *out = nullptr;
    if (cfg->n_envs < 1) return fail(nullptr, SCG_ERR_INVALID, "scg_create: n_envs must be >= 1");
    if (cfg->n_options < 0 || cfg->n_options > SCG_MAX_OPTIONS)
        return fail(nullptr, SCG_ERR_INVALID, "scg_create: n_options out of range [0,5]");
    if (cfg->update_count_floor < 0) return fail(nullptr, SCG_ERR_INVALID, "scg_create: update_count_floor must be >= 0");
    if (cfg->reoffer_period < 0 || (cfg->reoffer_period & (cfg->reoffer_period - 1)))
        return fail(nullptr, SCG_ERR_INVALID, "scg_create: reoffer_period must be a power of two (or 0)");
    if (cfg->fourier_order != SCG_FOURIER_ORDER)
        return fail(nullptr, SCG_ERR_INVALID, "scg_create: only Fourier order 5 is built");
    int ndev = 0;
    if (hipGetDeviceCount(&ndev) != hipSuccess || ndev < 1)
        return fail(nullptr, SCG_ERR_NO_DEVICE, "scg_create: no HIP device visible");
    if (cfg->device < 0 || cfg->device >= ndev)
        return fail(nullptr, SCG_ERR_INVALID, "scg_create: device ordinal out of range");
    scg_ctx *c = new (std::nothrow) scg_ctx();
    if (!c) return fail(nullptr, SCG_ERR_INVALID, "scg_create: out of host memory");
    memset(c, 0, sizeof(*c));
    c->cfg = *cfg;
    c->n_vf = cfg->n_options + 1;
    c->nblk = (cfg->n_envs + BLOCK_ENVS - 1) / BLOCK_ENVS;
    if (hipDeviceGetAttribute(&c->n_cu, hipDeviceAttributeMultiprocessorCount, cfg->device) != hipSuccess || c->n_cu <= 0) c->n_cu = 256;
    int st = SCG_OK;
    DeviceGuard dev_guard_(cfg->device);
    do {
        if (!dev_guard_.ok) { st = SCG_ERR_HIP; break; }
        const size_t slab_bytes = (size_t)c->nblk * c->n_vf * NACT * NF * sizeof(float);
        if (hipMalloc(&c->d_slabs, slab_bytes) != hipSuccess) { st = SCG_ERR_HIP; break; }
        if (hipMalloc(&c->d_cnts, (size_t)c->nblk * c->n_vf * sizeof(int32_t)) != hipSuccess) { st = SCG_ERR_HIP; break; }
        if (hipMalloc(&c->d_G, (size_t)c->n_vf * NACT * NF * sizeof(float)) != hipSuccess) { st = SCG_ERR_HIP; break; }
        if (hipMalloc(&c->d_nk, MAX_VF * sizeof(int32_t)) != hipSuccess) { st = SCG_ERR_HIP; break; }
        if (hipMalloc(&c->d_edges, MAX_EDGES * 8 * sizeof(float)) != hipSuccess) { st = SCG_ERR_HIP; break; }
        if (hipMalloc(&c->d_scale, NF * sizeof(float)) != hipSuccess) { st = SCG_ERR_HIP; break; }
        if (hipMalloc(&c->d_perm, (size_t)c->nblk * BLOCK_ENVS * sizeof(int32_t)) != hipSuccess) { st = SCG_ERR_HIP; break; }
        if (hipMalloc(&c->d_hist, (size_t)((c->cfg.n_envs + 255) / 256) * HSTRIDE * sizeof(int32_t)) != hipSuccess) { st = SCG_ERR_HIP; break; }
        if (hipMalloc(&c->d_collect_rows, (size_t)((cfg->n_envs + COL_ROW - 1) / COL_ROW + 1) * sizeof(int32_t)) != hipSuccess) { st = SCG_ERR_HIP; break; }
        if (hipMalloc(&c->d_frontier_rows, (size_t)MAX_VF * ((cfg->n_envs + COL_ROW - 1) / COL_ROW + 1) * sizeof(int32_t)) != hipSuccess) { st = SCG_ERR_HIP; break; }
        if (hipMalloc(&c->d_fit_part, (size_t)FIT_BATCH * 2 * FIT_G * 8 * sizeof(unsigned long long)) != hipSuccess) { st = SCG_ERR_HIP; break; }
        if (hipHostMalloc(reinterpret_cast<void **>(&c->h_async), 64, hipHostMallocMapped) != hipSuccess) { st = SCG_ERR_HIP; break; }
        *c->h_async = 0u;
        if (hipHostGetDevicePointer(reinterpret_cast<void **>(&c->d_async), c->h_async, 0) != hipSuccess) { st = SCG_ERR_HIP; break; }
        if (hipMalloc(&c->d_fail, sizeof(int32_t)) != hipSuccess || hipMemset(c->d_fail, 0, sizeof(int32_t)) != hipSuccess) { st = SCG_ERR_HIP; break; }
        if (hipMalloc(&c->d_outrec, (size_t)c->nblk * BLOCK_ENVS * OREC * sizeof(float4)) != hipSuccess) { st = SCG_ERR_HIP; break; }
        if (hipMalloc(&c->d_qalt, (size_t)c->nblk * BLOCK_ENVS * 2 * sizeof(float4)) != hipSuccess) { st = SCG_ERR_HIP; break; }
        if (hipMalloc(&c->d_invperm, (size_t)c->nblk * BLOCK_ENVS * sizeof(int32_t)) != hipSuccess) { st = SCG_ERR_HIP; break; }
        {
            const size_t hb = (size_t)((c->cfg.n_envs + 255) / 256) * HSTRIDE * sizeof(int32_t);
            if (hipMalloc(&c->d_hist2[0], hb) != hipSuccess || hipMalloc(&c->d_hist2[1], hb) != hipSuccess) { st = SCG_ERR_HIP; break; }
            if (hipMemset(c->d_hist2[0], 0, hb) != hipSuccess || hipMemset(c->d_hist2[1], 0, hb) != hipSuccess) { st = SCG_ERR_HIP; break; }
        }
        if (hipMalloc(&c->d_cellmask, (size_t)CELL_G * CELL_G * 4 * sizeof(uint64_t)) != hipSuccess) { st = SCG_ERR_HIP; break; }
        if (hipMemset(c->d_cnts, 0, (size_t)c->nblk * c->n_vf * sizeof(int32_t)) != hipSuccess) { st = SCG_ERR_HIP; break; }
        if (hipMemset(c->d_G, 0, (size_t)c->n_vf * NACT * NF * sizeof(float)) != hipSuccess) { st = SCG_ERR_HIP; break; }
        if (hipMemset(c->d_nk, 0, MAX_VF * sizeof(int32_t)) != hipSuccess) { st = SCG_ERR_HIP; break; }
    } while (0);
    if (st != SCG_OK) {
        snprintf(g_err, 256, "scg_create: device allocation/setup failed: %s", hipGetErrorString(hipGetLastError()));
        scg_destroy(c);
        return st;
    }
#ifdef SCG_STAMPS_LITE
    if (hipMalloc(&c->d_stamps, (size_t)c->nblk * STAMP_SLOTS * sizeof(unsigned long long)) == hipSuccess)
        (void)hipMemset(c->d_stamps, 0, (size_t)c->nblk * STAMP_SLOTS * sizeof(unsigned long long));
#endif
    c->parents = 0;
    for (int k = 1; k < MAX_VF; ++k) c->parents |= (uint32_t)(k - 1) << (3 * k);
    c->G_out = c->d_G; c->nk_out = c->d_nk;
    c->fit_timeout_s = 2.0;
    c->peer_timeout_s = 2.0;
    *out = c;
    return SCG_OK;
}

int scg_destroy(scg_ctx *c) {
    if (!c) return SCG_OK;
    (void)hipFree(c->d_slabs); (void)hipFree(c->d_cnts); (void)hipFree(c->d_G); (void)hipFree(c->d_nk);
    (void)hipFree(c->d_hist2[0]); (void)hipFree(c->d_hist2[1]); (void)hipFree(c->d_outrec); (void)hipFree(c->d_qalt); (void)hipFree(c->d_invperm);
    (void)hipFree(c->d_edges); (void)hipFree(c->d_starts); (void)hipFree(c->d_scale); (void)hipFree(c->d_cellmask); (void)hipFree(c->d_perm); (void)hipFree(c->d_hist);
    (void)hipFree(c->d_fit_part); (void)hipFree(c->d_collect_rows); (void)hipFree(c->d_frontier_rows); (void)hipFree(c->d_fail);
    if (c->h_async) (void)hipHostFree(c->h_async);
    if (c->peer_region) {
        DeviceGuard g(c->cfg.device);
        for (int r = 0; r < PEER_MAX; ++r)
            if (c->peer_mapped[r]) (void)hipIpcCloseMemHandle(c->peer_base[r]);
        {
            std::lock_guard<std::mutex> lk(g_peer_mu);
            for (size_t i = 0; i < g_peer_regions.size(); ++i)
                if (g_peer_regions[i].second == c->peer_region) { g_peer_regions.erase(g_peer_regions.begin() + i); break; }
        }
        (void)hipFree(c->peer_region); (void)hipFree(c->d_peer_go);
    }
    if (c->prof_ev) {
        for (hipEvent_t e : *c->prof_ev) (void)hipEventDestroy(e);
        delete c->prof_ev;
    }
    delete c;
    return SCG_OK;
}

int scg_set_hparams(scg_ctx *c, float gamma, float alpha, float epsilon, float r_option_success,
                    int32_t max_episode_steps, int32_t max_option_steps, int32_t update_count_floor, int32_t reoffer_period) {
    if (!c) return fail(nullptr, SCG_ERR_INVALID, "scg_set_hparams: null ctx");
    c->cfg.gamma = gamma; c->cfg.alpha = alpha; c->cfg.epsilon = epsilon;
    c->cfg.r_option_success = r_option_success;
    c->cfg.max_episode_steps = max_episode_steps; c->cfg.max_option_steps = max_option_steps;
    c->cfg.update_count_floor = update_count_floor < 0 ? 0 : update_count_floor;
    if (reoffer_period < 0 || (reoffer_period & (reoffer_period - 1))) return fail(c, SCG_ERR_INVALID, "scg_set_hparams: reoffer_period must be a power of two (or 0)");
    c->cfg.reoffer_period = reoffer_period;
    return SCG_OK;
}

int scg_set_map(scg_ctx *c, const float *edges, int32_t n_edges, const float *starts, int32_t n_starts,
                const float map_scalars[6], const float *scale) {
    if (!c) return fail(nullptr, SCG_ERR_INVALID, "scg_set_map: null ctx");
    if (!edges || !starts || !map_scalars || !scale) return fail(c, SCG_ERR_INVALID, "scg_set_map: null argument");
    if (n_edges < 0 || n_edges > MAX_EDGES) return fail(c, SCG_ERR_INVALID, "scg_set_map: n_edges out of range [0,256]");
    if (n_starts < 1) return fail(c, SCG_ERR_INVALID, "scg_set_map: need at least one start position");
    SCG_ON_DEVICE(c, "scg_set_map");
    if (c->d_starts) { (void)hipFree(c->d_starts); c->d_starts = nullptr; }
    SCG_HIP(c, hipMalloc(&c->d_starts, (size_t)n_starts * 2 * sizeof(float)));
    if (n_edges > 0) SCG_HIP(c, hipMemcpy(c->d_edges, edges, (size_t)n_edges * 8 * sizeof(float), hipMemcpyHostToDevice));
    SCG_HIP(c, hipMemcpy(c->d_starts, starts, (size_t)n_starts * 2 * sizeof(float), hipMemcpyHostToDevice));
    SCG_HIP(c, hipMemcpy(c->d_scale, scale, NF * sizeof(float), hipMemcpyHostToDevice));
    const float R = map_scalars[0];
    c->ms.hstep = map_scalars[1]; c->ms.R2 = map_scalars[2];
    c->ms.TX = map_scalars[3]; c->ms.TY = map_scalars[4]; c->ms.TR2 = map_scalars[5];
    c->ms.R = R; c->ms.TR = (float)(std::sqrt((double)map_scalars[5]) * 1.0001);
    {
        std::vector<uint64_t> cm((size_t)CELL_G * CELL_G * 4, 0);
        const double vmax = 2.0 * std::sqrt(2.0) * 1.001;
        const double reach = (double)R * (1.02 + 1.10 * vmax) * 1.01 + 0.5 * std::sqrt(2.0) / CELL_G + 1e-6;
        for (int cy = 0; cy < CELL_G; ++cy)
            for (int cx = 0; cx < CELL_G; ++cx) {
                const double px = (cx + 0.5) / CELL_G, py = (cy + 0.5) / CELL_G;
                for (int j = 0; j < n_edges; ++j) {
                    const float *E = edges + 8 * j;
                    const double dx = px - E[0], dy = py - E[1];
                    double t = (dx * E[2] + dy * E[3]) * E[4];
                    t = t < 0 ? 0 : (t > 1 ? 1 : t);
                    const double qx = E[0] + E[2] * t - px, qy = E[1] + E[3] * t - py;
                    if (std::sqrt(qx * qx + qy * qy) <= reach)
                        cm[((size_t)cy * CELL_G + cx) * 4 + (j >> 6)] |= (1ull << (j & 63));
                }
            }
        SCG_HIP(c, hipMemcpy(c->d_cellmask, cm.data(), cm.size() * sizeof(uint64_t), hipMemcpyHostToDevice));
    }
    c->ms.n_edges = n_edges; c->ms.n_starts = n_starts;
    c->have_map = true;
    return SCG_OK;
}

struct PeerTarget {
    scg_ctx *c;
    float *G, *nkf;
    int32_t *nk;
    explicit PeerTarget(scg_ctx *ctx) : c(ctx), G(ctx->G_out), nkf(ctx->nkf_out), nk(ctx->nk_out) {
        if (!c->peer_n) return;
        float *op = reinterpret_cast<float *>(c->peer_region + PEER_HDR + (c->peer_e & 1u) * c->peer_op_stride);
        c->G_out = op; c->nkf_out = op + (size_t)c->n_vf * NACT * NF; c->nk_out = c->d_nk;
    }
    ~PeerTarget() { c->G_out = G; c->nkf_out = nkf; c->nk_out = nk; }
};

extern "C++" template <typename Args>
static void fill_shared(const scg_ctx *c, Args &A) {
    memset(&A, 0, sizeof(A));
    A.n = c->cfg.n_envs; A.n_vf = c->n_vf;
    A.seed = c->cfg.seed; A.env_base = c->cfg.env_id_base;
    A.epsilon = c->cfg.epsilon; A.max_ep = c->cfg.max_episode_steps; A.max_opt = c->cfg.max_option_steps;
    A.reoffer_mask = c->cfg.reoffer_period > 1 ? (uint32_t)(c->cfg.reoffer_period - 1) : 0u;
    A.parents = c->parents; A.gest = c->gest;
    A.ms = c->ms;
    A.edges = c->d_edges; A.starts = c->d_starts; A.cellmask = c->d_cellmask;
}

static void fill_common(const scg_ctx *c, StepArgs &A) {
    fill_shared(c, A);
    A.gamma = c->cfg.gamma; A.r_succ = c->cfg.r_option_success;
    A.slabs = c->d_slabs; A.cnts = c->d_cnts;
    A.gest_succ = c->gest_succ;
    A.ring_x = c->ring_x; A.ring_y = c->ring_y; A.events = c->events; A.ev_len = c->ev_len;
    A.ring_mask = c->ring_len > 0 ? c->ring_len - 1 : 0;
    A.stamps = c->d_stamps;
    A.async_word = c->d_async; A.fail_flag = c->d_fail;
}

static int launch_reduce(scg_ctx *c, float *W, uint32_t apply, int nblk, hipStream_t s,
                         const StepArgs *st = nullptr, bool sort = false, bool reduce = true) {
    ReduceArgs R;
    memset(&R, 0, sizeof(R));
    R.slabs = c->d_slabs; R.cnts = c->d_cnts; R.G = c->G_out; R.n_k = c->nk_out; R.nk_f = c->nkf_out; R.W = W; R.scale = c->d_scale;
    R.nblk = nblk; R.n_vf = c->n_vf; R.alpha = c->cfg.alpha; R.apply = apply; R.fail_flag = c->d_fail; R.nk_floor = c->cfg.update_count_floor;
    const int nrow = st ? (c->cfg.n_envs + 255) / 256 : 0;
    R.n = c->cfg.n_envs; R.nrow = nrow;
    if (st) {
        R.outrec = c->d_outrec; R.qalt = c->d_qalt; R.invperm = c->d_invperm; R.perm = c->d_perm; R.sort = sort ? 1 : 0;
        R.hist = c->d_hist2[c->hist_parity]; R.hist_zero = c->d_hist2[c->hist_parity ^ 1];
        R.x = st->x; R.y = st->y; R.vx = st->vx; R.vy = st->vy; R.reward = st->reward;
        R.option_id_out = st->option_id; R.opt_steps = st->opt_steps; R.ep_steps = st->ep_steps;
        R.action = st->action; R.done = st->done;
        R.qcache = st->k_hi >= 0 ? st->qcache : nullptr;
        if (c->arm_bits && c->events && c->ring_x) {
            R.c_events = c->events; R.c_prev = c->arm_prev; R.c_evlen = c->ev_len; R.c_count = c->arm_count;
            R.c_rows = c->d_collect_rows; R.c_bits = c->arm_bits; R.c_L = c->arm_L; R.c_ring_len = c->ring_len;
        }
    }
    if (!reduce) {
        hipLaunchKernelGGL(commit_kernel, dim3(nrow), dim3(256), 0, s, R);
        SCG_HIP(c, hipGetLastError());
        return SCG_OK;
    }
    const int sy = (nrow + RED_NCOL - 1) / RED_NCOL;
    if (RED_NCOL * (c->n_vf + sy) <= c->n_cu)
        hipLaunchKernelGGL(reduce_kernel<16>, dim3(RED_NCOL, c->n_vf + sy), dim3(RED_THREADS), 0, s, R);
    else
        hipLaunchKernelGGL(reduce_kernel<8>, dim3(RED_NCOL, c->n_vf + sy), dim3(RED_THREADS), 0, s, R);
    SCG_HIP(c, hipGetLastError());
    return SCG_OK;
}

int scg_step(scg_ctx *c, float *x, float *y, float *vx, float *vy, int32_t *option_id, int32_t *opt_steps,
             int32_t *ep_steps, float *qcache, uint8_t *action, float *reward, uint8_t *done, float *W,
             const float *clf, uint32_t enabled_mask, uint64_t t, uint32_t flags, void *stream) {
    if (!c) return fail(nullptr, SCG_ERR_INVALID, "scg_step: null ctx");
    if (!c->have_map) return fail(c, SCG_ERR_STATE, "scg_step: scg_set_map has not been called");
    if (!x || !y || !vx || !vy || !option_id || !opt_steps || !ep_steps || !qcache || !action || !reward ||
        !done || !W || !clf)
        return fail(c, SCG_ERR_INVALID, "scg_step: null array argument");
    if (c->peer_n && (flags & SCG_STEP_LEARN) && (flags & SCG_STEP_APPLY))
        return fail(c, SCG_ERR_INVALID, "scg_step: SCG_STEP_APPLY with a peer region open (the update is scg_peer_exchange_apply's)");
    if ((flags & SCG_STEP_INTERRUPT) && !(flags & SCG_STEP_LEARN))
        return fail(c, SCG_ERR_INVALID, "scg_step: SCG_STEP_INTERRUPT without SCG_STEP_LEARN (acting-only interruption is scg_rollout_interrupt)");
    SCG_CHECK_ASYNC(c);
    SCG_ON_DEVICE(c, "scg_step");
    if (c->arm_bits) {
        const void *ptrs[2] = {c->arm_count, c->arm_prev};
        for (const void *p : ptrs) {
            if (!p) continue;
            hipPointerAttribute_t at;
            if (hipPointerGetAttributes(&at, p) != hipSuccess || at.type != hipMemoryTypeDevice) {
                (void)hipGetLastError();
                c->arm_bits = 0; c->arm_rows_ready = false;
                return fail(c, SCG_ERR_STATE, "scg_step: the buffers announced with scg_arm_collect are no longer device memory "
                                              "(freed before scg_arm_collect(0)?); the trigger has been disarmed");
            }
        }
    }
    hipStream_t s = reinterpret_cast<hipStream_t>(stream);
    StepArgs A;
    fill_common(c, A);
    A.x = x; A.y = y; A.vx = vx; A.vy = vy;
    A.option_id = option_id; A.opt_steps = opt_steps; A.ep_steps = ep_steps; A.qcache = qcache;
    A.action = action; A.reward = reward; A.done = done;
    A.W = W; A.clf = clf;
    A.k_lo = 0; A.k_hi = c->n_vf - 1;
    A.enabled = enabled_mask; A.learn = (flags & SCG_STEP_LEARN) ? 1u : 0u; A.t = t;
    if (flags & 0x100u) A.k_hi = -1;
    if (!(c->order_valid && c->order_ids == option_id)) {
        const int nrow = (c->cfg.n_envs + 255) / 256;
        hipLaunchKernelGGL(sort_hist_kernel, dim3(nrow), dim3(256), 0, s, option_id, c->cfg.n_envs, c->n_vf, c->d_hist);
        hipLaunchKernelGGL(sort_scatter_kernel, dim3(nrow), dim3(256), 0, s, option_id, c->cfg.n_envs, c->n_vf, nrow,
                           c->d_hist, c->d_perm, c->d_invperm);
        SCG_HIP(c, hipGetLastError());
    }
    c->order_valid = false;
    if (c->hist_dirty) {
        const size_t hb = (size_t)((c->cfg.n_envs + 255) / 256) * HSTRIDE * sizeof(int32_t);
        SCG_HIP(c, hipMemsetAsync(c->d_hist2[0], 0, hb, s));
        SCG_HIP(c, hipMemsetAsync(c->d_hist2[1], 0, hb, s));
        c->hist_dirty = false;
    }
    const bool fold = (flags & SCG_STEP_LEARN) && !(flags & 0x200u);
    A.hist_next = fold ? c->d_hist2[c->hist_parity] : nullptr;
    A.perm = c->d_perm; A.outrec = c->d_outrec; A.qalt = c->d_qalt;
    hipEvent_t ev0 = nullptr, ev1 = nullptr;
    if (c->prof_on && (c->prof_seen++ % c->prof_every) == c->prof_every / 2) {
        if (!c->prof_ev) c->prof_ev = new std::vector<hipEvent_t>();
        while (c->prof_ev->size() < c->prof_used + 2) {
            hipEvent_t e;
            SCG_HIP(c, hipEventCreate(&e));
            c->prof_ev->push_back(e);
        }
        ev0 = (*c->prof_ev)[c->prof_used]; ev1 = (*c->prof_ev)[c->prof_used + 1];
        c->prof_used += 2;
        SCG_HIP(c, hipEventRecord(ev0, s));
    }
    if (flags & SCG_STEP_INTERRUPT)
        hipLaunchKernelGGL(td_kernel<MODE_FUSED_INT>, dim3(c->nblk), dim3(THREADS), 0, s, A);
    else
        hipLaunchKernelGGL(td_kernel<MODE_FUSED>, dim3(c->nblk), dim3(THREADS), 0, s, A);
    SCG_HIP(c, hipGetLastError());
    if (ev1) SCG_HIP(c, hipEventRecord(ev1, s));
    c->arm_rows_ready = c->arm_bits && c->events && c->ring_x;
    if (!(flags & SCG_STEP_LEARN)) return launch_reduce(c, W, 0u, c->nblk, s, &A, false, false);
    PeerTarget peer_target(c);
    if (!fold) return launch_reduce(c, W, (flags & SCG_STEP_APPLY) ? 1u : 0u, c->nblk, s, &A, false);
    c->hist_dirty = true;
    const int rc = launch_reduce(c, W, (flags & SCG_STEP_APPLY) ? 1u : 0u, c->nblk, s, &A, true);
    if (rc != SCG_OK) return rc;
    c->hist_dirty = false;
    c->hist_parity ^= 1;
    c->order_valid = true; c->order_ids = option_id;
    return SCG_OK;
}

static bool rollout_epw(const scg_ctx *c, int n, int &epw) {
    epw = 2;
    while (epw < RO_MAX_EPW && (long long)n >= (long long)c->n_cu * RO_WAVES * epw * 2) epw *= 2;
    if (const char *ov = getenv("SCG_ROLLOUT_EPW")) {
        const int v = atoi(ov);
        if (v < 2 || v > RO_MAX_EPW || (v & (v - 1))) return false;
        epw = v;
    }
    return true;
}

static int fail_in(scg_ctx *c, int code, const char *fn, const char *why) {
    char msg[256];
    snprintf(msg, sizeof(msg), "%s: %s", fn, why);
    return fail(c, code, msg);
}

static int check_record(scg_ctx *c, const char *fn, const scg_record *rec, int N, long long min_rows) {
    const char *why = !rec->len ? "rec->len is required" : rec->n < 1 ? "rec->n must be >= 1"
                    : rec->first < 0 || (long long)rec->first + rec->n > N ? "rec->first .. first+n-1 outside the envs / entries"
                    : rec->rows < min_rows ? "rec->rows too small for the launch's pseudo-steps" : nullptr;
    return why ? fail_in(c, SCG_ERR_INVALID, fn, why) : SCG_OK;
}

static int rollout_launch(const char *fn, scg_ctx *c, float *x, float *y, float *vx, float *vy, int32_t *option_id, int32_t *opt_steps,
                          int32_t *ep_steps, float *qcache, uint8_t *action, float *reward, uint8_t *done,
                          const float *W, const float *clf, uint32_t enabled_mask, uint64_t t0, int32_t n_steps,
                          uint32_t flags, const scg_rollout_stats *stats, const scg_record *rec, bool at, void *stream,
                          bool intr = false, int32_t *interrupts = nullptr) {
    if (!c) return fail_in(nullptr, SCG_ERR_INVALID, fn, "null ctx");
    if (!c->have_map) return fail_in(c, SCG_ERR_STATE, fn, "scg_set_map has not been called");
    if (!x || !y || !vx || !vy || !option_id || !opt_steps || !ep_steps || !qcache || !action || !reward ||
        !done || !W || !clf)
        return fail_in(c, SCG_ERR_INVALID, fn, "null array argument");
    if (flags & ~(SCG_ROLLOUT_BEGIN | SCG_ROLLOUT_ONE_EPISODE)) return fail_in(c, SCG_ERR_INVALID, fn, "unknown flag");
    if (n_steps < 0 || n_steps > SCG_ROLLOUT_MAX_STEPS)
        return fail_in(c, SCG_ERR_INVALID, fn, "n_steps out of range [0, SCG_ROLLOUT_MAX_STEPS]");
    if (n_steps == 0 && !(flags & SCG_ROLLOUT_BEGIN))
        return fail_in(c, SCG_ERR_INVALID, fn, "n_steps == 0 without SCG_ROLLOUT_BEGIN (or _BEGIN_AT)");
    if ((flags & SCG_ROLLOUT_ONE_EPISODE) && !(stats && stats->finished))
        return fail_in(c, SCG_ERR_INVALID, fn, "SCG_ROLLOUT_ONE_EPISODE needs stats->finished");
    if (rec) {
        const int rc = check_record(c, fn, rec, c->cfg.n_envs, (long long)n_steps + ((flags & SCG_ROLLOUT_BEGIN) ? 1 : 0));
        if (rc != SCG_OK) return rc;
    }
    SCG_CHECK_ASYNC(c);
    DeviceGuard dev_guard_(c->cfg.device);
    if (!dev_guard_.ok) return fail_in(c, SCG_ERR_HIP, fn, "cannot make the context's device current");
    RolloutArgs R;
    fill_shared(c, R);
    R.x = x; R.y = y; R.vx = vx; R.vy = vy; R.option_id = option_id; R.opt_steps = opt_steps; R.ep_steps = ep_steps;
    R.qcache = qcache; R.action = action; R.reward = reward; R.done = done; R.W = W; R.clf = clf;
    if (stats) R.st = *stats;
    R.n_steps = n_steps;
    R.begin = (flags & SCG_ROLLOUT_BEGIN) ? 1u : 0u; R.one_episode = (flags & SCG_ROLLOUT_ONE_EPISODE) ? 1u : 0u;
    R.enabled = enabled_mask; R.t0 = t0;
    int epw;
    if (!rollout_epw(c, c->cfg.n_envs, epw)) return fail_in(c, SCG_ERR_INVALID, fn, "SCG_ROLLOUT_EPW must be 2, 4, 8, 16 or 32");
    R.epw = epw;
    const int grid = (c->cfg.n_envs + RO_WAVES * epw - 1) / (RO_WAVES * epw);
    c->order_valid = false;
    if (intr && (rec || at)) {
        RolloutIntRecArgs RR;
        memset(&RR, 0, sizeof(RR));
        static_cast<RolloutArgs &>(RR) = R;
        if (rec) RR.rec = *rec;
        RR.begin_at = at ? 1u : 0u;
        RR.interrupts = interrupts;
        SCG_HIP(c, launch_rollout_interrupt_record(RR, grid, reinterpret_cast<hipStream_t>(stream)));
        return SCG_OK;
    }
    if (intr) {
        RolloutIntArgs RI;
        memset(&RI, 0, sizeof(RI));
        static_cast<RolloutArgs &>(RI) = R;
        RI.interrupts = interrupts;
        SCG_HIP(c, launch_rollout_interrupt(RI, grid, reinterpret_cast<hipStream_t>(stream)));
        return SCG_OK;
    }
    if (rec || at) {
        RolloutRecArgs RR;
        memset(&RR, 0, sizeof(RR));
        static_cast<RolloutArgs &>(RR) = R;
        if (rec) RR.rec = *rec;
        RR.begin_at = at ? 1u : 0u;
        SCG_HIP(c, launch_rollout_record(RR, grid, reinterpret_cast<hipStream_t>(stream)));
        return SCG_OK;
    }
    hipLaunchKernelGGL((rollout_kernel<false, RolloutArgs>), dim3(grid), dim3(RO_THREADS), 0, reinterpret_cast<hipStream_t>(stream), R);
    SCG_HIP(c, hipGetLastError());
    return SCG_OK;
}

int scg_rollout(scg_ctx *c, float *x, float *y, float *vx, float *vy, int32_t *option_id, int32_t *opt_steps,
                int32_t *ep_steps, float *qcache, uint8_t *action, float *reward, uint8_t *done,
                const float *W, const float *clf, uint32_t enabled_mask, uint64_t t0, int32_t n_steps,
                uint32_t flags, const scg_rollout_stats *stats, void *stream) {
    return rollout_launch("scg_rollout", c, x, y, vx, vy, option_id, opt_steps, ep_steps, qcache, action, reward, done, W, clf,
                          enabled_mask, t0, n_steps, flags, stats, nullptr, false, stream);
}

int scg_rollout_record(scg_ctx *c, float *x, float *y, float *vx, float *vy, int32_t *option_id, int32_t *opt_steps,
                       int32_t *ep_steps, float *qcache, uint8_t *action, float *reward, uint8_t *done,
                       const float *W, const float *clf, uint32_t enabled_mask, uint64_t t0, int32_t n_steps,
                       uint32_t flags, const scg_rollout_stats *stats, const scg_record *rec, void *stream) {
    if (!c) return fail(nullptr, SCG_ERR_INVALID, "scg_rollout_record: null ctx");
    const bool at = (flags & SCG_ROLLOUT_BEGIN_AT) != 0;
    if (at && (flags & SCG_ROLLOUT_BEGIN))
        return fail(c, SCG_ERR_INVALID, "scg_rollout_record: SCG_ROLLOUT_BEGIN and SCG_ROLLOUT_BEGIN_AT together");
    const uint32_t fl = at ? (flags & ~SCG_ROLLOUT_BEGIN_AT) | SCG_ROLLOUT_BEGIN : flags;
    return rollout_launch("scg_rollout_record", c, x, y, vx, vy, option_id, opt_steps, ep_steps, qcache, action, reward, done,
                          W, clf, enabled_mask, t0, n_steps, fl, stats, rec, at, stream);
}

int scg_rollout_interrupt(scg_ctx *c, float *x, float *y, float *vx, float *vy, int32_t *option_id, int32_t *opt_steps,
                          int32_t *ep_steps, float *qcache, uint8_t *action, float *reward, uint8_t *done,
                          const float *W, const float *clf, uint32_t enabled_mask, uint64_t t0, int32_t n_steps,
                          uint32_t flags, const scg_rollout_stats *stats, int32_t *interrupts, const scg_record *rec,
                          void *stream) {
    if (!c) return fail(nullptr, SCG_ERR_INVALID, "scg_rollout_interrupt: null ctx");
    const bool at = (flags & SCG_ROLLOUT_BEGIN_AT) != 0;
    if (at && (flags & SCG_ROLLOUT_BEGIN))
        return fail(c, SCG_ERR_INVALID, "scg_rollout_interrupt: SCG_ROLLOUT_BEGIN and SCG_ROLLOUT_BEGIN_AT together");
    const uint32_t fl = at ? (flags & ~SCG_ROLLOUT_BEGIN_AT) | SCG_ROLLOUT_BEGIN : flags;
    return rollout_launch("scg_rollout_interrupt", c, x, y, vx, vy, option_id, opt_steps, ep_steps, qcache, action, reward, done,
                          W, clf, enabled_mask, t0, n_steps, fl, stats, rec, at, stream, true, interrupts);
}

static int trials_launch(const char *fn, scg_ctx *c, int32_t n, const float *x, const float *y, const float *vx, const float *vy,
                         const int32_t *option, const float *W, const float *clf, uint32_t enabled_mask, uint64_t t0,
                         const scg_trial_out *out, const scg_record *rec, void *stream) {
    if (!c) return fail_in(nullptr, SCG_ERR_INVALID, fn, "null ctx");
    if (!c->have_map) return fail_in(c, SCG_ERR_STATE, fn, "scg_set_map has not been called");
    if (!x || !y || !vx || !vy || !option || !W || !clf || !out || !out->outcome)
        return fail_in(c, SCG_ERR_INVALID, fn, "null array argument (or out->outcome)");
    if (n < 1) return fail_in(c, SCG_ERR_INVALID, fn, "n must be >= 1");
    if (std::min(c->cfg.max_option_steps, c->cfg.max_episode_steps) > SCG_TRIAL_MAX_STEPS)
        return fail_in(c, SCG_ERR_INVALID, fn, "min(max_option_steps, max_episode_steps) exceeds SCG_TRIAL_MAX_STEPS");
    if (rec) {
        const int rc = check_record(c, fn, rec, n, 1);
        if (rc != SCG_OK) return rc;
// ... 472 lines not shown
```

### skill-chaining-with-graphs_amd/csrc/scg_step_kernel.hpp

```cpp
#pragma once

constexpr int P_WAVES = BLOCK_ENVS / 64;
constexpr int LIST0 = P_WAVES;
constexpr int HELPER0 = 7;
constexpr int N_HELP = WAVES - HELPER0;
constexpr int P_POOL = HELPER0;
static_assert(HELPER0 >= P_WAVES && N_HELP >= 8 && N_HELP * 64 * 3 >= 12 * 2 * 64, "stage_w by the helper waves: at most three float4 per thread");
constexpr int OFF_RC = 0;
constexpr int OFF_INT = OFF_RC + 6 * BLOCK_ENVS * 4;
constexpr int OFF_Z1 = OFF_INT + 6 * BLOCK_ENVS;
constexpr int U2_CH = 9 * WAVES;
constexpr int US = 2 * U2_CH + 4;
constexpr int R_TAB = 2 * W_FLOATS;
constexpr int R_S = R_TAB, R_EDGES = R_S + 8 * BLOCK_ENVS, R_PITEMS = R_EDGES + MAX_EDGES * 8;
constexpr int cmax3(int a, int b, int c) { return a > b ? (a > c ? a : c) : (b > c ? b : c); }
constexpr int R_FLOATS = cmax3(R_TAB + WAVES * E_TAB_FLOATS, 3 * 36 * US, R_PITEMS + P_WAVES * PITEMS);
constexpr int OFF_R = OFF_Z1 + BLOCK_ENVS * 2 * 4 * 8;
constexpr int OFF_ELIST = OFF_R + R_FLOATS * 4;
constexpr int OFF_ULIST = OFF_ELIST + 2 * BLOCK_ENVS * 2;
constexpr int OFF_MAXQ = OFF_ULIST + BLOCK_ENVS * 2;
constexpr int OFF_QSA = OFF_MAXQ + 2 * BLOCK_ENVS * 4;
constexpr int OFF_EFLAG = OFF_QSA + 2 * BLOCK_ENVS * 4;
constexpr int OFF_CLF = OFF_EFLAG + 64;
constexpr int OFF_MISC = OFF_CLF + MAX_VF * CLF_STRIDE * 4;
// ... 292 lines not shown
            if (mk != (c == 64 ? ~0ull : ((1ull << c) - 1ull))) prefix = false;
            if (c > 0 && m != 64 * h) prefix = false;
            m += c;
        }
        if (prefix) { kB = k0; mB = m; }
    };
    auto u1_geometry = [&](uint64_t (&mk)[P_WAVES][NACT], int (&at)[P_WAVES]) {
#pragma unroll
        for (int h = 0; h < P_WAVES; ++h) at[h] = 64 * h + lane < nb ? (int)s_a[64 * h + lane] : -1;
        int off = 0;
#pragma unroll
        for (int a = 0; a < NACT; ++a) {
            int rl = 0, nbq = 0;
#pragma unroll
            for (int h = 0; h < P_WAVES; ++h) {
                mk[h][a] = __ballot(at[h] == a);
                rl += __popcll(mk[h][a]);
                const int lim = mB - 64 * h;
                const uint64_t pre = lim >= 64 ? ~0ull : (lim > 0 ? ((1ull << lim) - 1ull) : 0ull);
                nbq += __popcll(mk[h][a] & pre);
            }
            run_len[a] = rl; run_off[a] = off; nBa[a] = nbq; off += rl;
        }
    };
    const bool helpers = FUSED && A.learn && A.k_hi >= 0;

    if (tid < M_INTS) s_misc[tid] = (tid == M_PRESENT || tid == M_UPD) ? 1 : 0;
    block_lds_sync();
    SCG_LITE(1);
    int e_pre = e0 + tid;
    if (FUSED) {
        if (wave < P_WAVES) {
            if (tid < nb && A.perm) e_pre = A.perm[e0 + tid];
        } else {
            if (helpers && wave >= HELPER0) stage_w(A.W, 0, tid - HELPER0 * 64, N_HELP * 64);
            for (int i = tid - P_WAVES * 64; i < A.ms.n_edges * 8; i += THREADS - P_WAVES * 64) s_edges[i] = A.edges[i];
            if (tid - P_WAVES * 64 < A.n_vf * CLF_STRIDE) s_clf[tid - P_WAVES * 64] = A.clf[tid - P_WAVES * 64];
            lds_arrive(&s_misc[M_C_TOP], 1);
        }
    }

    if (helpers) { if (wave < P_WAVES) __builtin_amdgcn_s_setprio(PRIO_P); else if (wave >= HELPER0) __builtin_amdgcn_s_setprio(PRIO_HELP); }
    if (wave < P_WAVES) {
        const int i = tid;
        const bool valid = i < nb;
        const int e = e_pre;
        if (FUSED) {
            uint32_t u[4] = {0u, 0u, 0u, 0u};
            int a = NACT - 1, ep0 = 0, o = 0, o_in = 0, osteps = 0;
            float sx = 0.5f, sy = 0.5f, svx = 0.0f, svy = 0.0f;
            float qc[NACT] = {0.0f, 0.0f, 0.0f, 0.0f, 0.0f};
            if (valid) {
                sx = A.x[e]; sy = A.y[e]; svx = A.vx[e]; svy = A.vy[e];
#pragma unroll
                for (int aa = 0; aa < NACT; ++aa) qc[aa] = A.qcache[(size_t)aa * N + e];
                ep0 = A.ep_steps[e]; o = A.option_id[e]; osteps = A.opt_steps[e];
                o_in = o;
                o = (o >= 1 && o < A.n_vf) ? o : 0;
                s_s[0 * BLOCK_ENVS + i] = sx; s_s[1 * BLOCK_ENVS + i] = sy;
                s_s[2 * BLOCK_ENVS + i] = svx; s_s[3 * BLOCK_ENVS + i] = svy;
                s_ot[i] = (uint8_t)o;
            } else {
                s_ot[i] = 255;
            }
            lds_arrive(&s_misc[M_C_PUBS], 64);
            if (valid) {
                env_draw((uint64_t)(A.env_base + e), A.t, A.seed, u);
                a = act_spec(u, qc, A.epsilon);
                s_a[i] = (uint8_t)a;
            } else {
                s_a[i] = 0;
            }
            lds_arrive(&s_misc[M_C_PUB], 64);
            bool goal;
            bool par;
            float *xs_mine = s_s + 4 * BLOCK_ENVS + wave * 64;
            lds_await(&s_misc[M_C_TOP], WAVES - P_WAVES);
            const int groups = pinball_wave_prepare_any(s_edges, A.cellmask, A.ms, valid, sx, sy, svx, svy, a, goal, par,
                                                        s_pitems + wave * PITEMS, xs_mine, BLOCK_ENVS);
            if (lane == 0) s_misc[M_GROUPS + wave] = groups;
            lds_arrive(&s_misc[M_C_PREP], 1);
            {
                lds_await(&s_misc[M_C_PREP], P_WAVES);
                int gsum[P_WAVES + 1];
                gsum[0] = 0;
#pragma unroll
                for (int w2 = 0; w2 < P_WAVES; ++w2) gsum[w2 + 1] = gsum[w2] + s_misc[M_GROUPS + w2];
#ifdef SCG_STAMPS_LITE
                if (A.stamps && wave == 0 && lane == 0) A.stamps[(size_t)blockIdx.x * STAMP_SLOTS + 42] = (unsigned long long)gsum[P_WAVES];
#endif
                for (int q = wave; q < gsum[P_WAVES]; q += P_POOL) {
                    int owner = 0, first = 0;
#pragma unroll
                    for (int w2 = 1; w2 < P_WAVES; ++w2) if (q >= gsum[w2]) { owner = w2; first = gsum[w2]; }
                    pinball_wave_group(s_edges, A.ms, s_pitems + owner * PITEMS + 64 * (q - first),
                                       s_s + 4 * BLOCK_ENVS + owner * 64, BLOCK_ENVS, s_ia + owner * 64);
                }
                lds_arrive(&s_misc[M_C_POOL], 1);
                lds_await(&s_misc[M_C_POOL], P_POOL);
            }
            const float rew = pinball_wave_finish(par, sx, sy, svx, svy, a, goal, xs_mine, BLOCK_ENVS, s_ia + wave * 64);
            int hkey = -1;
            if (valid) {
                const int eps1 = ep0 + 1;
                const int dn = episode_end(goal, eps1, A.max_ep);
                float nx = sx, ny = sy, nvx = svx, nvy = svy;
                if (dn) restart_state(u[2], A.starts, A.ms.n_starts, nx, ny, nvx, nvy);
                s_s[4 * BLOCK_ENVS + i] = nx; s_s[5 * BLOCK_ENVS + i] = ny;
                s_s[6 * BLOCK_ENVS + i] = nvx; s_s[7 * BLOCK_ENVS + i] = nvy;
                unsigned inA, inB, inS = 0;
                member_masks(s_clf, A.n_vf, A.enabled | A.gest, sx, sy, nx, ny, inA, inB);
#pragma unroll
                for (int k = 1; k < MAX_VF; ++k) {
                    if (k < A.n_vf && ((A.gest >> k) & 1u) && clf_z(s_clf + CLF_STRIDE * k, s_s[0 * BLOCK_ENVS + i], s_s[1 * BLOCK_ENVS + i]) > 0.0f)
                        inS |= 1u << k;
                }
                bool keep = false;
                float ro = 0.0f, co = 0.0f;
                if (o >= 1) {
                    bool succ;
                    keep = option_keep(A.parents, o, inA, goal, dn, osteps, A.max_opt, succ);
                    ro = rew + (succ ? A.r_succ : 0.0f);
                    co = keep ? A.gamma : 0.0f;
                }
                const int cand = keep ? o : select_option(A.parents, inB, A.enabled);
                const int stay = reoffer_stay(keep, cand, dn, o_in, A.t, (uint64_t)(A.env_base + e), A.reoffer_mask);
                const int on = stay ? 0 : cand;
                s_on[i] = (uint8_t)on;
                if constexpr (INT) s_ic[i] = (uint8_t)(keep ? IC_KEEP | (unsigned)select_option(A.parents, inB, A.enabled) : 0u);
                s_gs[i] = (uint8_t)inS; s_ia[i] = (uint8_t)((inA & 0x3Eu) | (goal ? 1u : 0u) | ((!keep && on >= 1) ? IA_ENTERING : 0u));
                {
                    const unsigned pm = (1u << o) | (1u << (on & 31)) | inS, um = (1u << o) | inS;
                    unsigned pw = 0, uw = 0;
#pragma unroll
                    for (int k = 0; k < MAX_VF + 1; ++k) {
                        if (__ballot((pm >> k) & 1u)) pw |= 1u << k;
                        if (__ballot((um >> k) & 1u)) uw |= 1u << k;
                    }
                    if (lane == __builtin_ctzll(__ballot(true))) {
                        atomicOr(reinterpret_cast<unsigned *>(&s_misc[M_PRESENT]), pw);
                        atomicOr(reinterpret_cast<unsigned *>(&s_misc[M_UPD]), uw);
                    }
                }
                if (inS && A.gest_succ) {
#pragma unroll
                    for (int k = 1; k < MAX_VF; ++k) {
                        const unsigned par2 = target_of(A.parents, k);
                        if (((inS >> k) & 1u) && ((par2 == 0) ? goal : (bool)((inA >> par2) & 1u))) atomicAdd(&A.gest_succ[k], 1);
                    }
                }
                s_r0[i] = rew; s_c0[i] = dn ? 0.0f : A.gamma; s_ro[i] = ro; s_co[i] = co;
                {
                    const int osn = keep ? osteps + 1 : 0, epn = dn ? 0 : eps1;
                    float4 *orec = A.outrec + (size_t)(e0 + i) * OREC;
                    orec[0] = make_float4(nx, ny, nvx, nvy);
                    orec[1] = make_float4(rew, __uint_as_float((unsigned)a | ((unsigned)dn << 8) | ((unsigned)on << 16) | ((unsigned)stay << 28)),
                                          __int_as_float(osn), __int_as_float(epn));
                    reinterpret_cast<float *>(orec + 3)[1] = 0.0f;
                }
                if (A.ring_x) {
                    const size_t row = (size_t)(ep0 & A.ring_mask) * N + e;
                    A.ring_x[row] = s_s[0 * BLOCK_ENVS + i]; A.ring_y[row] = s_s[1 * BLOCK_ENVS + i];
                }
                if (A.events) { A.events[e] = (uint8_t)((goal ? 1u : 0u) | (inA & 0x3Eu)); A.ev_len[e] = eps1; }
                hkey = (e >> 8) * 8 + on;
            } else {
                s_on[i] = 255; s_gs[i] = 0; s_ia[i] = 0;
                if constexpr (INT) s_ic[i] = 0;
            }
            if (A.hist_next) {
                uint64_t rem = __ballot(hkey >= 0);
                while (rem) {
                    const int src = (int)__builtin_ctzll(rem);
                    const int k0 = __shfl(hkey, src, 64);
                    const uint64_t m = __ballot(hkey == k0);
                    if (lane == src) atomicAdd(&A.hist_next[k0], (int)__popcll(m));
                    rem &= ~m;
                }
            }
        } else if (valid) {
            if (MODE == MODE_TRANS) {
                s_s[0 * BLOCK_ENVS + i] = A.x[e]; s_s[1 * BLOCK_ENVS + i] = A.y[e];
                s_s[2 * BLOCK_ENVS + i] = A.vx[e]; s_s[3 * BLOCK_ENVS + i] = A.vy[e];
                s_s[4 * BLOCK_ENVS + i] = A.xn[e]; s_s[5 * BLOCK_ENVS + i] = A.yn[e];
                s_s[6 * BLOCK_ENVS + i] = A.vxn[e]; s_s[7 * BLOCK_ENVS + i] = A.vyn[e];
                s_a[i] = A.action[e]; s_ot[i] = (uint8_t)A.k_lo; s_on[i] = 255; s_gs[i] = 0; s_ia[i] = 0;
                const float r = A.reward[e], c = A.cont_in[e];
                s_r0[i] = r; s_c0[i] = c; s_ro[i] = r; s_co[i] = c;
            } else {
                s_s[4 * BLOCK_ENVS + i] = A.x[e]; s_s[5 * BLOCK_ENVS + i] = A.y[e];
                s_s[6 * BLOCK_ENVS + i] = A.vx[e]; s_s[7 * BLOCK_ENVS + i] = A.vy[e];
                s_a[i] = 0; s_ot[i] = 255; s_on[i] = (uint8_t)A.k_lo; s_gs[i] = 0; s_ia[i] = 0;
                s_r0[i] = 0.0f; s_c0[i] = 0.0f; s_ro[i] = 0.0f; s_co[i] = 0.0f;
            }
        } else {
            s_a[i] = 0; s_ot[i] = 255; s_on[i] = 255; s_gs[i] = 0; s_ia[i] = 0;
        }
    } else if (FUSED && wave < P_POOL) {
        lds_await(&s_misc[M_C_PREP], P_WAVES);
        int gsum[P_WAVES + 1];
        gsum[0] = 0;
#pragma unroll
        for (int w2 = 0; w2 < P_WAVES; ++w2) gsum[w2 + 1] = gsum[w2] + s_misc[M_GROUPS + w2];
        for (int q = wave; q < gsum[P_WAVES]; q += P_POOL) {
            int owner = 0, first = 0;
#pragma unroll
            for (int w2 = 1; w2 < P_WAVES; ++w2) if (q >= gsum[w2]) { owner = w2; first = gsum[w2]; }
            pinball_wave_group(s_edges, A.ms, s_pitems + owner * PITEMS + 64 * (q - first),
                               s_s + 4 * BLOCK_ENVS + owner * 64, BLOCK_ENVS, s_ia + owner * 64);
        }
        lds_arrive(&s_misc[M_C_POOL], 1);
    } else if (helpers && wave >= HELPER0) {
        const int ht = tid - HELPER0 * 64, hw = wave - HELPER0;
        constexpr int NHT = N_HELP * 64;
        lds_await(&s_misc[M_C_PUBS], 64 * P_WAVES);
        decide_b();
        if (hw == 0 && lane == 0) { s_misc[M_KB] = kB; s_misc[M_MB] = mB; }
        if (kB >= 1) stage_w(A.W + (size_t)kB * NACT * NF, W_FLOATS, ht, NHT);
        for (int u = ht; u < BLOCK_ENVS * 2; u += NHT) {
            const int i = u & (BLOCK_ENVS - 1), h = u / BLOCK_ENVS;
            if (i < nb) {
                const float v0 = s_s[(2 * h) * BLOCK_ENVS + i], v1 = s_s[(2 * h + 1) * BLOCK_ENVS + i];
                const float2 za = sincospi_cs(h ? fmaf(v0, 0.25f, 0.5f) : v0), zb = sincospi_cs(h ? fmaf(v1, 0.25f, 0.5f) : v1);
                *reinterpret_cast<float4 *>(s_z1 + (i * 2 + 0) * 4 + 2 * h) = make_float4(za.x, za.y, zb.x, zb.y);
            }
        }
        lds_await(&s_misc[M_C_PUB], 64 * P_WAVES);
        {
            uint64_t mk[P_WAVES][NACT];
            int at[P_WAVES];
            u1_geometry(mk, at);
            if (hw == 0) {
                const uint64_t below = (1ull << lane) - 1ull;
#pragma unroll
                for (int a = 0; a < NACT; ++a) {
                    int before = 0;
#pragma unroll
                    for (int h = 0; h < P_WAVES; ++h) {
                        if (at[h] == a) s_ulist[run_off[a] + before + __popcll(mk[h][a] & below)] = (uint16_t)(64 * h + lane);
                        before += __popcll(mk[h][a]);
                    }
                }
            }
        }
#ifdef SCG_TEST_DROP_ARRIVE
        if (!(hw == 0 && blockIdx.x == 1 && A.t == 0x7e57ull))
#endif
        lds_arrive(&s_misc[M_C_HELP], 1);
        lds_await(&s_misc[M_C_HELP], N_HELP);
        run_u1_dyn();
    }
    else if (FUSED && wave == HELPER0) {
        lds_await(&s_misc[M_C_PUBS], 64 * P_WAVES);
        decide_b();
        if (lane == 0) { s_misc[M_KB] = kB; s_misc[M_MB] = mB; }
    }
    if (helpers) { if ((unsigned)(wave - LIST0) < (unsigned)LIST_WAVES) __builtin_amdgcn_s_setprio(PRIO_LIST); else __builtin_amdgcn_s_setprio(0); }
    SCG_LITE(2);
    block_lds_sync();
    SCG_LITE(3);

    for (int u = tid; u < BLOCK_ENVS * 8; u += THREADS) {
        const int i = (u >> 2) & (BLOCK_ENVS - 1), d = u & 3, sg = u / (4 * BLOCK_ENVS);
        if (i < nb && (MODE != MODE_QVAL || sg == 1) && !(helpers && sg == 0)) {
            const float sv = s_s[(4 * sg + d) * BLOCK_ENVS + i];
            s_z1[(i * 2 + sg) * 4 + d] = sincospi_cs(d < 2 ? sv : fmaf(sv, 0.25f, 0.5f));
        }
    }
    if (FUSED && A.k_hi >= 0) {
        kB = __builtin_amdgcn_readfirstlane(s_misc[M_KB]); mB = __builtin_amdgcn_readfirstlane(s_misc[M_MB]);
    } else { kB = -1; mB = 0; }

    const unsigned present = (FUSED) ? (unsigned)__builtin_amdgcn_readfirstlane(s_misc[M_PRESENT]) : ~0u;
    const unsigned updm = (FUSED) ? (A.learn ? (unsigned)__builtin_amdgcn_readfirstlane(s_misc[M_UPD]) : 0u) : ~0u;
    unsigned single = (FUSED && A.k_hi >= 0) ? (updm & present & ~1u & ~(kB >= 1 ? 1u << kB : 0u)) : 0u;
    const unsigned eval_only = (FUSED && A.k_hi >= 0) ? (present & ~updm & ~1u & ~(kB >= 1 ? 1u << kB : 0u)) : 0u;
    if (FUSED && tid < A.n_vf && A.cnts && tid != 0 && tid != kB && !((single >> tid) & 1u))
        A.cnts[(size_t)b * A.n_vf + tid] = 0;
    const int n_pass0 = A.k_hi >= A.k_lo ? 1 : 0;
    const unsigned single0 = single;
    auto gate = [&](int kdec) {
        if (!FUSED) return;
        int ln;
        asm volatile("v_mbcnt_lo_u32_b32 %0, -1, 0\n\tv_mbcnt_hi_u32_b32 %0, -1, %0" : "=v"(ln));
        const int ti = (wave << 6) | ln;
        if (ti >= nb || !(s_ia[ti] & IA_ENTERING)) return;
        const int cand = s_on[ti];
        const bool mine = kdec < 0 ? (cand >= 1 && cand < MAX_VF && !((single0 >> cand) & 1u)) : cand == kdec;
        if (!mine) return;
        const float cm = kdec < 0 ? s_maxq[BLOCK_ENVS + ti] : s_maxq[ti];
        const float rm = (kdec >= 0 || single0 != 0u) ? s_qsa[BLOCK_ENVS + ti] : s_maxq[ti];
        if (cm >= rm) return;
        s_on[ti] = 0;
        reinterpret_cast<float *>(A.outrec + (size_t)(e0 + ti) * OREC + 3)[1] = __uint_as_float(OREC_DECLINED);
        if (A.hist_next) {
            const int e = A.perm ? A.perm[e0 + ti] : e0 + ti;
            atomicAdd(&A.hist_next[(e >> 8) * 8 + cand], -1);
            atomicAdd(&A.hist_next[(e >> 8) * 8], 1);
        }
    };
    auto interrupt_rewrite = [&](int kdec) {
        if constexpr (INT) {
            int ln;
            asm volatile("v_mbcnt_lo_u32_b32 %0, -1, 0\n\tv_mbcnt_hi_u32_b32 %0, -1, %0" : "=v"(ln));
            const int ti = (wave << 6) | ln;
            if (ti >= nb || !(s_ic[ti] & IC_KEEP)) return;
            const int o = s_ot[ti];
            if (o != (kdec < 0 ? kB : kdec)) return;
            const float mo = kdec < 0 ? s_maxq[BLOCK_ENVS + ti] : s_maxq[ti];
            const float m0 = kdec < 0 ? s_maxq[ti] : s_qsa[BLOCK_ENVS + ti];
            if (mo >= m0) return;
            float *rec = reinterpret_cast<float *>(A.outrec + (size_t)(e0 + ti) * OREC);
            rec[5] = __uint_as_float((unsigned)s_a[ti] | ((s_ic[ti] & 7u) << 16));
            rec[6] = __int_as_float(0);
            rec[13] = __uint_as_float(OREC_DECLINED);
            if (A.hist_next) {
                const int e = A.perm ? A.perm[e0 + ti] : e0 + ti;
                atomicAdd(&A.hist_next[(e >> 8) * 8 + o], -1);
                atomicAdd(&A.hist_next[(e >> 8) * 8], 1);
            }
        }
    };
    const bool blk_fail = FUSED && __builtin_amdgcn_readfirstlane(s_misc[M_FAIL]) != 0;
    if (blk_fail && tid < A.n_vf && A.cnts) A.cnts[(size_t)b * A.n_vf + tid] = 0;
    for (int pass = 0; pass < n_pass0 + MAX_VF && !blk_fail; ++pass) {
        int lane_p;
        asm volatile("v_mbcnt_lo_u32_b32 %0, -1, 0\n\tv_mbcnt_hi_u32_b32 %0, -1, %0" : "=v"(lane_p));
        const int tid_p = (wave << 6) | lane_p;
        const int tid = tid_p, lane = lane_p;
        int kA, kBp;
        bool dense;
        if (pass == 0) {
            if (!n_pass0) continue;
            kA = FUSED ? 0 : A.k_lo; kBp = kB; dense = true;
        } else {
            if (!single) break;
            kA = __builtin_ctz(single); single &= single - 1; kBp = -1; dense = false;
        }
        const bool u1_done = helpers && pass == 0;
        if (pass > 0) block_lds_sync();
        if (FUSED && pass > 0 && kA == __builtin_ctz(single0)) {
            if (tid < nb) s_qsa[BLOCK_ENVS + tid] = s_maxq[tid];
        }
        const int ft = tid - LIST0 * 64, lw = wave - LIST0;
        bool evA = false, evB = false, up = false;
        int at = -1;
        if ((unsigned)ft < (unsigned)nb) {
            const int ot = s_ot[ft], on = s_on[ft];
            const bool own = (FUSED && kA == 0) || ot == kA;
            const bool gst = FUSED && !own && ((s_gs[ft] >> kA) & 1);
            up = (MODE != MODE_QVAL) && A.learn && (own || gst);
            float rk = s_r0[ft], cont = s_c0[ft];
            if (FUSED && kA != 0) {
                if (ot == kA) { rk = s_ro[ft]; cont = s_co[ft]; }
                else {
                    const unsigned ia = s_ia[ft];
                    const bool succ = option_succ(A.parents, kA, ia, ia & 1u);
                    const bool fail = !succ && !((ia >> kA) & 1u);
                    rk = rk + (succ ? A.r_succ : 0.0f);
                    cont = (cont == 0.0f || succ || fail) ? 0.0f : A.gamma;
                }
                s_rk[ft] = rk; s_ck[ft] = cont;
            }
            evA = (on == kA) || (up && cont > 0.0f) || (FUSED && kA == 0 && (s_ia[ft] & IA_ENTERING));
            if constexpr (INT) evA = evA || (kA == 0 && (s_ic[ft] & IC_KEEP));
            if (kBp >= 1) evB = (on == kBp) || (ot == kBp && A.learn && s_co[ft] > 0.0f);
            at = s_a[ft];
            s_ev[ft] = (uint8_t)((evA ? 1 : 0) | (evB ? 2 : 0));
        }
        const int pg_b = (mB + 7) >> 3;
        const bool cmp = dense ? (evB && (ft >> 3) >= pg_b) : evA;
        const bool eo_pass = pass == 0 && FUSED && eval_only != 0;
        const int on_me = (unsigned)ft < (unsigned)nb ? (int)s_on[ft] : 0;
        const bool eo = eo_pass && (unsigned)ft < (unsigned)nb && ((eval_only >> (on_me & 7)) & 1u);
        uint64_t me[MAX_VF];
        if (ft == 0) s_misc[M_ECTR] = 0;
        uint64_t mb[1 + NACT];
        if ((unsigned)lw < (unsigned)LIST_WAVES) {
            mb[0] = __ballot(cmp);
#pragma unroll
            for (int k = 1; k < MAX_VF; ++k) me[k] = eo_pass ? __ballot(eo && on_me == k) : 0ull;
            if (lane >= 11 && lane < 10 + MAX_VF) {
                const int k = lane - 10;
                s_misc[M_CNT + lw * 16 + lane] = __popcll(k == 1 ? me[1] : k == 2 ? me[2] : k == 3 ? me[3] : k == 4 ? me[4] : me[5]);
            }
#pragma unroll
            for (int a = 0; a < NACT; ++a) mb[1 + a] = __ballot(up && at == a);
            const int lim = (kBp >= 1 ? mB : 0) - 64 * lw;
            const uint64_t pre = lim >= 64 ? ~0ull : (lim > 0 ? ((1ull << lim) - 1ull) : 0ull);
            if (lane < 1 + 2 * NACT) {
                const int sl = lane <= NACT ? lane : lane - NACT;
                const uint64_t mine = sl == 0 ? mb[0] : sl == 1 ? mb[1] : sl == 2 ? mb[2] : sl == 3 ? mb[3] : sl == 4 ? mb[4] : mb[5];
                s_misc[M_CNT + lw * 16 + lane] = __popcll(lane <= NACT ? mine : (mine & pre));
            }
            if (dense) {
                const uint64_t ma = __ballot(evA), mbb = __ballot(evB);
                if (lane < 8) {
                    const int pgrp = lw * 8 + lane;
                    s_eflag[pgrp] = (uint8_t)((((ma >> (8 * lane)) & 0xffull) ? 1 : 0) | ((((mbb >> (8 * lane)) & 0xffull) && pgrp < pg_b) ? 2 : 0));
                }
            }
        }
        if (!u1_done) {
            const float *Wa = A.W + (MODE == MODE_QVAL ? 0 : (size_t)__builtin_amdgcn_readfirstlane(kA) * NACT * NF);
            stage_w_cold(Wa, s_W, tid);
            if (kBp >= 1) stage_w_cold(A.W + (size_t)__builtin_amdgcn_readfirstlane(kBp) * NACT * NF, s_W + W_FLOATS, tid);
        }
        block_lds_sync();
        int n_cmp = 0, nupdB = 0;
        {
            int se = 0;
#pragma unroll
            for (int w2 = 0; w2 < LIST_WAVES; ++w2) se += s_misc[M_CNT + w2 * 16];
            n_cmp = __builtin_amdgcn_readfirstlane(se);
            int off = 0;
#pragma unroll
            for (int a = 0; a < NACT; ++a) {
                int sr = 0, sb = 0;
#pragma unroll
                for (int w2 = 0; w2 < LIST_WAVES; ++w2) { sr += s_misc[M_CNT + w2 * 16 + 1 + a]; sb += s_misc[M_CNT + w2 * 16 + 1 + NACT + a]; }
                run_len[a] = __builtin_amdgcn_readfirstlane(sr);
                nBa[a] = __builtin_amdgcn_readfirstlane(sb);
                run_off[a] = off;
                off += run_len[a];
                nupdB += nBa[a];
            }
        }
        const int nupd = run_off[NACT - 1] + run_len[NACT - 1];
        int eo_cnt[MAX_VF], eo_base[MAX_VF], eo_units_l = 0;
#pragma unroll
        for (int k = 0; k < MAX_VF; ++k) { eo_cnt[k] = 0; eo_base[k] = 0; }
        if (eo_pass && (unsigned)lw < (unsigned)LIST_WAVES) {
            int base = (n_cmp + 7) & ~7;
#pragma unroll
            for (int k = 1; k < MAX_VF; ++k) {
                int c = 0;
#pragma unroll
                for (int w2 = 0; w2 < LIST_WAVES; ++w2) c += s_misc[M_CNT + w2 * 16 + 10 + k];
                eo_cnt[k] = __builtin_amdgcn_readfirstlane(c);
                eo_base[k] = base;
                base += (eo_cnt[k] + 7) & ~7;
                eo_units_l += (eo_cnt[k] + 7) >> 3;
            }
            if (lw == 0 && lane < MAX_VF) {
                const int k = lane;
                s_misc[M_EO + k] = k == 0 ? 0 : k == 1 ? eo_cnt[1] : k == 2 ? eo_cnt[2] : k == 3 ? eo_cnt[3] : k == 4 ? eo_cnt[4] : eo_cnt[5];
                s_misc[M_EO + 6 + k] = k == 0 ? eo_units_l : k == 1 ? eo_base[1] : k == 2 ? eo_base[2] : k == 3 ? eo_base[3] : k == 4 ? eo_base[4] : eo_base[5];
            }
        }
        if ((unsigned)lw < (unsigned)LIST_WAVES) {
            const uint64_t below = (1ull << lane) - 1ull;
            if (eo) {
                int off = zero_i();
                for (int w2 = 0; w2 < lw; ++w2) off += s_misc[M_CNT + w2 * 16 + 10 + on_me];
                const uint64_t mine = on_me == 1 ? me[1] : on_me == 2 ? me[2] : on_me == 3 ? me[3] : on_me == 4 ? me[4] : me[5];
                const int eb = on_me == 1 ? eo_base[1] : on_me == 2 ? eo_base[2] : on_me == 3 ? eo_base[3] : on_me == 4 ? eo_base[4] : eo_base[5];
                s_elist[eb + off + __popcll(mine & below)] = (uint16_t)ft;
            }
            if (cmp) {
                int off = zero_i();
                for (int w2 = 0; w2 < lw; ++w2) off += s_misc[M_CNT + w2 * 16];
                s_elist[off + __popcll(mb[0] & below)] = (uint16_t)ft;
            }
            if (up && !u1_done) {
                int off = zero_i();
                const uint64_t mine = at == 0 ? mb[1] : at == 1 ? mb[2] : at == 2 ? mb[3] : at == 3 ? mb[4] : mb[5];
                for (int w2 = 0; w2 < lw; ++w2) off += s_misc[M_CNT + w2 * 16 + 1 + at];
                s_ulist[sel5(run_off, at) + off + __popcll(mine & below)] = (uint16_t)ft;
            }
        }
        block_lds_sync();
        if (tid == 0 && A.cnts) {
            A.cnts[(size_t)b * A.n_vf + kA] = nupd;
            if (kBp >= 1) A.cnts[(size_t)b * A.n_vf + kBp] = nupdB;
        }
        if (pass == 0) SCG_LITE(4);
        const int npg = dense ? (nb + 7) >> 3 : 0;
        const int n_own = (n_cmp + 7) >> 3;
        const int eo_units = eo_pass ? __builtin_amdgcn_readfirstlane(s_misc[M_EO + 6]) : 0;
        const int n_units = npg + n_own + eo_units;
        if (n_units + nupd == 0) continue;
        {
        const int n_cu = n_own + eo_units;
        for (;;) {
            int it = 0;
            if (lane == 0) it = atomicAdd(&s_misc[M_ECTR], 1);
            it = __builtin_amdgcn_readfirstlane(it);
            if (it >= n_cu + npg) break;
            const bool du = it >= n_cu;
            const int u = du ? it - n_cu : it;
            int base, cnt, kg = -1;
            unsigned fl;
            if (du) { base = 8 * u; cnt = min(8, nb - base); fl = (unsigned)__builtin_amdgcn_readfirstlane((int)s_eflag[u]); }
            else if (u < n_own) { base = 8 * u; cnt = min(8, n_cmp - base); fl = dense ? 2u : 1u; }
            else {
                int c = u - n_own;
                base = 0; cnt = 0; fl = 1u;
#pragma unroll
                for (int k = 1; k < MAX_VF; ++k) {
                    const int ck = __builtin_amdgcn_readfirstlane(s_misc[M_EO + k]), uk = (ck + 7) >> 3;
                    if (kg < 0 && c < uk) { kg = k; base = __builtin_amdgcn_readfirstlane(s_misc[M_EO + 6 + k]) + 8 * c; cnt = min(8, ck - 8 * c); }
                    if (kg < 0) c -= uk;
                }
            }
            if (!fl) continue;
            SCG_LANE_ROLES();
            {
                const int j = min(bi, cnt - 1);
                build_tables(s_z1 + ((du ? base + j : (int)s_elist[base + j]) * 2 + 1) * 4, cp, bcol, cdk, abq);
            }
            wave_lds_sync();
            float B[9];
            load_b(cdk, n16, g, B);
            const bool have = ocol_item < cnt;
            const int il = du ? base + min(ocol_item, cnt - 1) : (int)s_elist[base + min(ocol_item, cnt - 1)];
            if (kg >= 1) {
                float qo[NACT];
                int n16o = n16, go = g;
                asm volatile("" : "+v"(n16o), "+v"(go));
                contract_mem<EO_TG>(A.W + (size_t)kg * NACT * NF, B, qo, n16o, go, ab_lane);
                if (out_lane && have) {
                    float4 *orec = A.outrec + (size_t)(e0 + il) * OREC;
                    orec[2] = make_float4(qo[0], qo[1], qo[2], qo[3]);
                    orec[3].x = qo[4];
                    float mx = qo[0];
#pragma unroll
                    for (int a = 1; a < NACT; ++a) mx = fmaxf(mx, qo[a]);
                    s_maxq[BLOCK_ENVS + il] = mx;
                }
                wave_lds_sync();
                continue;
            }
#pragma unroll 1
            for (int v = 0; v < 2; ++v) {
                if (!((fl >> v) & 1u)) continue;
                float qo[NACT];
                contract_lds<E_TG>(v * W_FLOATS, B, qo, g, w4, w8, ab_lane);
                if (out_lane && have && ((s_ev[il] >> v) & 1)) {
                    const int kv = v ? kBp : kA;
                    if (FUSED) {
                        bool alt = kv == 0 && (s_ia[il] & IA_ENTERING);
                        if constexpr (INT) alt = alt || (kv == 0 && (s_ic[il] & IC_KEEP));
                        if (alt) {
                            float4 *qa = A.qalt + (size_t)(e0 + il) * 2;
                            qa[0] = make_float4(qo[0], qo[1], qo[2], qo[3]);
                            qa[1].x = qo[4];
                        }
                        if (s_on[il] == kv) {
                            float4 *orec = A.outrec + (size_t)(e0 + il) * OREC;
                            orec[2] = make_float4(qo[0], qo[1], qo[2], qo[3]);
                            orec[3].x = qo[4];
                        }
                    } else if (s_on[il] == kv) {
#pragma unroll
                        for (int a = 0; a < NACT; ++a) gstore(&A.qcache[(size_t)a * N + e0 + il], qo[a]);
                    }
                    float mx = qo[0];
#pragma unroll
                    for (int a = 1; a < NACT; ++a) mx = fmaxf(mx, qo[a]);
                    s_maxq[v * BLOCK_ENVS + il] = mx;
                }
            }
            wave_lds_sync();
        }
        }
        if (MODE != MODE_QVAL && nupd > 0 && !u1_done) run_u1(wave, WAVES, n_units);
        if (MODE == MODE_QVAL || nupd == 0) continue;
        if (pass == 0) SCG_LITE(5);
        block_lds_sync();
        if (pass == 0) SCG_LITE(6);

        int lane_u = lane;
        asm volatile("" : "+v"(lane_u));
        const int n16 = lane_u & 15, g = lane_u >> 4;
        int Ga[NACT], GBa[NACT];
        int Gtot = 0;
#pragma unroll
        for (int a = 0; a < NACT; ++a) { Ga[a] = (run_len[a] + 3) >> 2; GBa[a] = (nBa[a] + 3) >> 2; Gtot += Ga[a]; }
        constexpr int UCH = U2_CH, NBUILD = WAVES;
        const int nch = 4 * Gtot <= UCH ? 1 : 2;
        constexpr int USX = 2 * UCH + 4;
        static_assert(3 * 36 * USX <= R_FLOATS && NBUILD * 9 == UCH, "chunk tables fit region R");
        int wave_u = wave;
        asm volatile("" : "+s"(wave_u));
        const bool haveB = nupdB > 0;
        const bool worker = wave_u < 3 * NACT;
        const int ja = (wave_u * 11) >> 5, jm = wave_u - 3 * ja;
        const int j_GB = sel5(GBa, ja), j_nB = sel5(nBa, ja);
        f4v accU[2][3];
#pragma unroll
        for (int v = 0; v < 2; ++v) {
#pragma unroll
            for (int s = 0; s < 3; ++s) accU[v][s] = zero4();
        }
        const float *rA = (FUSED && kA != 0) ? s_rk : s_r0, *cA = (FUSED && kA != 0) ? s_ck : s_c0;
        const int bi9 = lane_u % 9, cp9 = lane_u / 9;
        auto chunk_geo = [&](int ch, int (&gb)[NACT], int (&gc)[NACT], int (&co)[NACT + 1]) {
            co[0] = 0;
#pragma unroll
            for (int a = 0; a < NACT; ++a) {
                const int half = Ga[a] >> 1;
                const int lo = ch == 0 ? 0 : half, hi = (nch == 1 || ch == 1) ? Ga[a] : half;
                gb[a] = lo; gc[a] = hi - lo;
                co[a + 1] = co[a] + 4 * gc[a];
            }
        };
        auto u2_build = [&](int ch, float *tab, int bw ) {
            int gb[NACT], gc[NACT], co[NACT + 1];
            chunk_geo(ch, gb, gc, co);
            float *ptabA = tab, *ptabB = tab + 36 * USX, *ctab = tab + 2 * 36 * USX;
            const int slot = 9 * bw + bi9;
            if (bw >= 0 && cp9 < 6 && slot < co[NACT]) {
                int a_ = 0;
#pragma unroll
                for (int a = 1; a < NACT; ++a) a_ += slot >= co[a] ? 1 : 0;
                const int rl = sel5(run_len, a_), ro = sel5(run_off, a_), nbq = sel5(nBa, a_), l4b = 4 * sel5(GBa, a_);
                const int j = 4 * sel5(gb, a_) + slot - sel5(co, a_);
                float *pdA = ptabA + cp9 * USX + 2 * slot, *pdB = ptabB + cp9 * USX + 2 * slot, *cdst = ctab + cp9 * USX + 2 * slot;
                if (j < rl) {
                    const int li = ro + j, il = s_ulist[li];
                    const float rr = rA[il], cont = cA[il];
                    const bool boot = FUSED && kA != 0 && cont == 0.0f && s_c0[il] > 0.0f;
                    float target = boot ? fmaf(A.gamma, s_qsa[BLOCK_ENVS + il], rr) : (cont > 0.0f ? fmaf(cont, s_maxq[il], rr) : rr);
                    if constexpr (INT) {
                        if (kA != 0 && (s_ic[il] & IC_KEEP) && s_ot[il] == kA && !(s_maxq[il] >= s_qsa[BLOCK_ENVS + il]))
                            target = fmaf(A.gamma, s_qsa[BLOCK_ENVS + il], rr);
                    }
                    const float d = target - s_qsa[li];
                    float2 ab[6], cd[6];
                    item_entries(s_z1 + (il * 2 + 0) * 4, cp9, ab, cd);
#pragma unroll
                    for (int c = 0; c < 6; ++c) {
                        *reinterpret_cast<float2 *>(pdA + 6 * c * USX) = make_float2(d * ab[c].x, d * (-ab[c].y));
                        *reinterpret_cast<float2 *>(cdst + 6 * c * USX) = make_float2(cd[c].x, cd[c].y);
                    }
                    if (j < nbq) {
                        const float rb = s_ro[il], cb2 = s_co[il];
                        float tb = (cb2 == 0.0f && s_c0[il] > 0.0f) ? fmaf(A.gamma, s_maxq[il], rb)
                                                                   : (cb2 > 0.0f ? fmaf(cb2, s_maxq[BLOCK_ENVS + il], rb) : rb);
                        if constexpr (INT) {
                            if ((s_ic[il] & IC_KEEP) && !(s_maxq[BLOCK_ENVS + il] >= s_maxq[il])) tb = fmaf(A.gamma, s_maxq[il], rb);
                        }
                        const float db = tb - s_qsa[BLOCK_ENVS + li];
#pragma unroll
                        for (int c = 0; c < 6; ++c)
                            *reinterpret_cast<float2 *>(pdB + 6 * c * USX) = make_float2(db * ab[c].x, db * (-ab[c].y));
                    } else if (j < l4b) {
#pragma unroll
                        for (int c = 0; c < 6; ++c) *reinterpret_cast<float2 *>(pdB + 6 * c * USX) = make_float2(0.0f, 0.0f);
                    }
                } else {
#pragma unroll
                    for (int c = 0; c < 6; ++c) {
                        *reinterpret_cast<float2 *>(pdA + 6 * c * USX) = make_float2(0.0f, 0.0f);
                        *reinterpret_cast<float2 *>(cdst + 6 * c * USX) = make_float2(0.0f, 0.0f);
                    }
                    if (j < l4b) {
#pragma unroll
                        for (int c = 0; c < 6; ++c) *reinterpret_cast<float2 *>(pdB + 6 * c * USX) = make_float2(0.0f, 0.0f);
                    }
                }
            }
        };
        auto u2_mfma = [&](int ch, const float *tab) {
            if (!worker) return;
            int gb[NACT], gc[NACT], co[NACT + 1];
            chunk_geo(ch, gb, gc, co);
            const float *ptabA = tab, *ctab = tab + 2 * 36 * USX;
            const int ngrp = sel5(gc, ja), g0 = sel5(gb, ja), so = sel5(co, ja);
            if (ngrp <= 0) return;
            const int ngrpB = haveB ? min(max(j_GB - g0, 0), ngrp) : 0;
            const int prow = min(16 * jm + n16, 35) * USX + 2 * g + 2 * so;
            const float *paA = ptabA + prow;
            const float *pb0 = ctab + n16 * USX + 2 * g + 2 * so,
                        *pb2 = ctab + min(32 + n16, 35) * USX + 2 * g + 2 * so;
            const int nvalid = j_nB - 4 * g0;
#define U2_LDS(P) ((unsigned)(size_t)(const __attribute__((address_space(3))) void *)(P))
            unsigned aP = U2_LDS(paA), a0 = U2_LDS(pb0), a2_ = U2_LDS(pb2);
            f4v x0 = accU[0][0], x1 = accU[0][1], x2 = accU[0][2], y0 = accU[1][0], y1 = accU[1][1], y2 = accU[1][2];
            const int nBfull = ngrpB > 0 && nvalid < 4 * ngrpB ? ngrpB - 1 : ngrpB;
            const int nAonly = ngrp - ngrpB;
            const unsigned long long nullmask = __ballot(4 * nBfull + g >= nvalid);
            unsigned cnt;
#define MF(ACC, A_, B_) "v_mfma_f32_16x16x4_f32 %[" ACC "], " A_ ", " B_ ", %[" ACC "]\n\t"
#define SX1 MF("x0", "v102", "v100") MF("x1", "v104", "v100") MF("x2", "v106", "v100") MF("x0", "v103", "v101") MF("x1", "v105", "v101") MF("x2", "v107", "v101")
#define SY1 MF("y0", "v102", "v108") MF("y1", "v104", "v108") MF("y2", "v106", "v108") MF("y0", "v103", "v109") MF("y1", "v105", "v109") MF("y2", "v107", "v109")
#define SX2 MF("x0", "v112", "v110") MF("x1", "v114", "v110") MF("x2", "v116", "v110") MF("x0", "v113", "v111") MF("x1", "v115", "v111") MF("x2", "v117", "v111")
#define SY2 MF("y0", "v112", "v118") MF("y1", "v114", "v118") MF("y2", "v116", "v118") MF("y0", "v113", "v119") MF("y1", "v115", "v119") MF("y2", "v117", "v119")
#define SYP MF("y0", "v112", "v108") MF("y1", "v114", "v108") MF("y2", "v116", "v108") MF("y0", "v113", "v109") MF("y1", "v115", "v109") MF("y2", "v117", "v109")
#define F1A(O) "ds_read_b64 v[100:101], %[aP] offset:" O "\n\tds_read_b64 v[102:103], %[a0] offset:" O "\n\tds_read_b64 v[104:105], %[a0] offset:%[o1]+" O "\n\tds_read_b64 v[106:107], %[a2] offset:" O "\n\t"
#define F2A(O) "ds_read_b64 v[110:111], %[aP] offset:" O "\n\tds_read_b64 v[112:113], %[a0] offset:" O "\n\tds_read_b64 v[114:115], %[a0] offset:%[o1]+" O "\n\tds_read_b64 v[116:117], %[a2] offset:" O "\n\t"
#define F1Q(O) "ds_read_b64 v[108:109], %[aP] offset:%[oq]+" O "\n\t"
#define F2Q(O) "ds_read_b64 v[118:119], %[aP] offset:%[oq]+" O "\n\t"
#define LW "s_waitcnt lgkmcnt(0)\n\t"
#define BUMP(N) "v_add_u32_e32 %[aP], " N ", %[aP]\n\tv_add_u32_e32 %[a0], " N ", %[a0]\n\tv_add_u32_e32 %[a2], " N ", %[a2]\n\t"
#define ZC(D, S) "v_cndmask_b32_e64 " D ", " S ", 0, %[nm]\n\t"
            asm volatile(
                "s_cmp_eq_u32 %[nBall], 0\n\ts_cbranch_scc1 10f\n\t"
                F1A("0") F1Q("0") LW
                "s_lshr_b32 %[cnt], %[nB], 2\n\ts_cmp_eq_u32 %[cnt], 0\n\ts_cbranch_scc1 2f\n"
                "1:\n\t" F2A("32") F2Q("32") SX1 SY1 LW F1A("64") F1Q("64") SX2 SY2 LW F2A("96") F2Q("96") SX1 SY1 LW F1A("128") F1Q("128") SX2 SY2 LW BUMP("0x80")
                "s_sub_u32 %[cnt], %[cnt], 1\n\ts_cmp_lg_u32 %[cnt], 0\n\ts_cbranch_scc1 1b\n"
                "2:\n\ts_bitcmp1_b32 %[nB], 1\n\ts_cbranch_scc0 3f\n\t" F2A("32") F2Q("32") SX1 SY1 LW F1A("64") F1Q("64") SX2 SY2 LW BUMP("64")
                "\n3:\n\ts_bitcmp1_b32 %[nB], 0\n\ts_cbranch_scc0 4f\n\t" SX1 SY1 F1A("32") F1Q("32") LW BUMP("32")
                "\n4:\n\ts_cmp_eq_u32 %[nBall], %[nB]\n\ts_cbranch_scc1 11f\n\t" SX1
                ZC("v112", "v102") ZC("v113", "v103") ZC("v114", "v104") ZC("v115", "v105") ZC("v116", "v106") ZC("v117", "v107") SYP F1A("32") LW BUMP("32")
                "s_branch 11f\n"
                "10:\n\ts_cmp_eq_u32 %[nA], 0\n\ts_cbranch_scc1 20f\n\t" F1A("0") LW
                "\n11:\n\ts_lshr_b32 %[cnt], %[nA], 2\n\ts_cmp_eq_u32 %[cnt], 0\n\ts_cbranch_scc1 13f\n"
                "12:\n\t" F2A("32") SX1 LW F1A("64") SX2 LW F2A("96") SX1 LW F1A("128") SX2 LW BUMP("0x80")
                "s_sub_u32 %[cnt], %[cnt], 1\n\ts_cmp_lg_u32 %[cnt], 0\n\ts_cbranch_scc1 12b\n"
                "13:\n\ts_bitcmp1_b32 %[nA], 1\n\ts_cbranch_scc0 14f\n\t" F2A("32") SX1 LW F1A("64") SX2 LW BUMP("64")
                "\n14:\n\ts_bitcmp1_b32 %[nA], 0\n\ts_cbranch_scc0 20f\n\t" SX1
                "\n20:\n\ts_nop 15\n\ts_nop 7"
                : [x0] "+v"(x0), [x1] "+v"(x1), [x2] "+v"(x2), [y0] "+v"(y0), [y1] "+v"(y1), [y2] "+v"(y2),
                  [aP] "+v"(aP), [a0] "+v"(a0), [a2] "+v"(a2_), [cnt] "=&s"(cnt)
                : [nB] "s"(nBfull), [nBall] "s"(ngrpB), [nA] "s"(nAonly), [nm] "s"(nullmask), [oq] "i"(36 * USX * 4), [o1] "i"(16 * USX * 4)
                : "v100", "v101", "v102", "v103", "v104", "v105", "v106", "v107", "v108", "v109", "v110", "v111", "v112", "v113", "v114", "v115", "v116",
                  "v117", "v118", "v119", "scc");
#undef MF
#undef SX1
#undef SY1
#undef SX2
#undef SY2
#undef SYP
#undef F1A
#undef F2A
#undef F1Q
#undef F2Q
#undef LW
#undef BUMP
#undef ZC
#undef U2_LDS
            accU[0][0] = x0; accU[0][1] = x1; accU[0][2] = x2; accU[1][0] = y0; accU[1][1] = y1; accU[1][2] = y2;
        };
        for (int ch = 0; ch < nch; ++ch) {
            if (ch > 0) block_lds_sync();
            u2_build(ch, s_R, wave);
            block_lds_sync();
            u2_mfma(ch, s_R);
        }
        if (!s_misc[M_FAIL]) {
            if (worker) {
#pragma unroll
                for (int v = 0; v < 2; ++v) {
                    if (v == 1 && !haveB) break;
                    const int kv = v ? kBp : kA;
                    float *slab_lane = A.slabs + ((size_t)b * A.n_vf + kv) * NACT * NF + ja * NF + (16 * jm + n16) * 36 + 4 * g;
#pragma unroll
                    for (int ni = 0; ni < 3; ++ni) {
                        const bool okl = (jm < 2 || n16 < 4) && (ni < 2 || g == 0);
                        if (okl) store_wt(slab_lane + 16 * ni, accU[v][ni]);
                    }
                }
            }
        } else if (tid == 0 && A.cnts) {
            A.cnts[(size_t)b * A.n_vf + kA] = 0;
            if (kBp >= 1) A.cnts[(size_t)b * A.n_vf + kBp] = 0;
        }
        if (pass == 0) SCG_LITE(7);
        if (pass > 0) gate(kA);
        if constexpr (INT) { if (pass > 0 || kB >= 1) interrupt_rewrite(pass > 0 ? kA : -1); }
    }
    if (FUSED && n_pass0 && !blk_fail) {
        if (!A.learn) block_lds_sync();
        gate(-1);
    }
    if (FUSED && A.async_word) {
        block_lds_sync();
        if (tid == 0 && s_misc[M_FAIL]) {
            __hip_atomic_fetch_or(A.async_word, SCG_ASYNC_STEP_HANDOFF, __ATOMIC_RELAXED, __HIP_MEMORY_SCOPE_SYSTEM);
            if (A.fail_flag) __hip_atomic_store(A.fail_flag, 1, __ATOMIC_RELAXED, __HIP_MEMORY_SCOPE_AGENT);
        }
    }
#ifdef SCG_STAMPS_LITE
    if (FUSED && A.stamps && lite_role >= 0 && lane == 0) {
        unsigned long long *o = A.stamps + (size_t)blockIdx.x * STAMP_SLOTS;
#pragma unroll
        for (int i = 1; i < 8; ++i) o[lite_role * 8 + i] += lt[i] ? lt[i] - lt[0] : 0ull;
        o[lite_role * 8] += __builtin_amdgcn_s_memtime() - lt[0];
        if (lite_role == 0) { o[32] = lite_r0; o[33] = __builtin_amdgcn_s_memrealtime(); }
    }
    if (FUSED && A.stamps && lane == 0) {
        unsigned hwid;
        asm volatile("s_getreg_b32 %0, hwreg(HW_REG_HW_ID)" : "=s"(hwid));
        reinterpret_cast<unsigned *>(A.stamps + (size_t)blockIdx.x * STAMP_SLOTS + 34)[wave] = hwid;
    }
#endif
}
```

Measured before the change: 841.9 million.

## Fuse reduce/apply and commit tail into step kernel via grid barrier

Adds an in-kernel tail to the fused step kernel: after the step work, blocks meet at a hierarchical software grid barrier and then run the gradient reduction, weight apply and commit/permute row placement themselves, so no separate reduce kernel launch is needed. Cross-workgroup data (outrec, qalt, cnts, hist, fail flag) now go through buffer stores/loads with a coherence aux bit or agent-scope atomics so that other blocks can read them after the barrier. This is meant to remove the launch gap and serialisation between the step and reduce kernels. In exchange it relies on all blocks being co-resident, adds a timeout/poison path with a new async error bit, and may slow the normal stores.

```diff
diff --git a/include/scg_abi.h b/include/scg_abi.h
--- a/include/scg_abi.h
+++ b/include/scg_abi.h
@@ -160,8 +160,11 @@
 #define SCG_ASYNC_FIT_TIMEOUT 0x1u
 #define SCG_ASYNC_STEP_HANDOFF 0x2u
 #define SCG_ASYNC_PEER_TIMEOUT 0x4u
+#define SCG_ASYNC_TAIL_BARRIER 0x8u
 int scg_async_status(scg_ctx *ctx, void *stream, int32_t synchronize, uint32_t *word_out);
 int scg_clear_async_error(scg_ctx *ctx);
+int scg_set_fused_tail(scg_ctx *ctx, int32_t on);
+int scg_last_step_launches(scg_ctx *ctx, int32_t *launches, int32_t *tail);
 int scg_set_fit_timeout(scg_ctx *ctx, double seconds);
 int scg_set_peer_timeout(scg_ctx *ctx, double seconds);
 int scg_decode_async_word(uint32_t word, char *buf, int32_t buf_len);
diff --git a/skill-chaining-with-graphs_amd/_lib.py b/skill-chaining-with-graphs_amd/_lib.py
--- a/skill-chaining-with-graphs_amd/_lib.py
+++ b/skill-chaining-with-graphs_amd/_lib.py
@@ -30,6 +30,7 @@
 ASYNC_FIT_TIMEOUT = 0x1
 ASYNC_STEP_HANDOFF = 0x2
 ASYNC_PEER_TIMEOUT = 0x4
+ASYNC_TAIL_BARRIER = 0x8
 PEER_HANDLE_BYTES = 64
 PEER_MAX_RANKS = 8
 
@@ -148,6 +149,8 @@
     "scg_fit_initiation": (C.c_int, [_P, C.c_int32, _P, _P, _P, _P, C.c_int32, C.c_float, C.c_float, _P]),
     "scg_async_status": (C.c_int, [_P, _P, C.c_int32, C.POINTER(C.c_uint32)]),
     "scg_clear_async_error": (C.c_int, [_P]),
+    "scg_set_fused_tail": (C.c_int, [_P, C.c_int32]),
+    "scg_last_step_launches": (C.c_int, [_P, C.POINTER(C.c_int32), C.POINTER(C.c_int32)]),
     "scg_set_fit_timeout": (C.c_int, [_P, C.c_double]),
     "scg_set_peer_timeout": (C.c_int, [_P, C.c_double]),
     "scg_peer_export": (C.c_int, [_P, _P]),
diff --git a/skill-chaining-with-graphs_amd/core.py b/skill-chaining-with-graphs_amd/core.py
--- a/skill-chaining-with-graphs_amd/core.py
+++ b/skill-chaining-with-graphs_amd/core.py
@@ -435,6 +435,14 @@
     def clear_async_error(self) -> None:
         self._call("scg_clear_async_error")
 
+    def set_fused_tail(self, on: bool) -> None:
+        self._call("scg_set_fused_tail", 1 if on else 0)
+
+    def last_step_launches(self):
+        n, t = C.c_int32(0), C.c_int32(0)
+        self._call("scg_last_step_launches", C.byref(n), C.byref(t))
+        return int(n.value), bool(t.value)
+
     def set_fit_timeout(self, seconds: float) -> None:
         self._call("scg_set_fit_timeout", C.c_double(seconds))
 
diff --git a/skill-chaining-with-graphs_amd/csrc/scg_kernels.hip b/skill-chaining-with-graphs_amd/csrc/scg_kernels.hip
--- a/skill-chaining-with-graphs_amd/csrc/scg_kernels.hip
+++ b/skill-chaining-with-graphs_amd/csrc/scg_kernels.hip
@@ -20,7 +20,55 @@
     asm volatile("global_store_dwordx4 %0, %1, off sc1\n\ts_nop 2" :: "v"(p), "v"(v) : "memory");
 }
 
+constexpr int XWG_AUX = 16;
+__device__ __forceinline__ __amdgpu_buffer_rsrc_t xwg_rsrc(const void *base) {
+    return __builtin_amdgcn_make_buffer_rsrc(const_cast<void *>(base), 0, 0x7fffffff, 0x00020000);
+}
+__device__ __forceinline__ void store_xwg(__amdgpu_buffer_rsrc_t rs, int off, float4 v) {
+    __builtin_amdgcn_raw_buffer_store_b128((u4v){__float_as_uint(v.x), __float_as_uint(v.y), __float_as_uint(v.z), __float_as_uint(v.w)}, rs, off, 0, XWG_AUX);
+}
+__device__ __forceinline__ void store_xwg(__amdgpu_buffer_rsrc_t rs, int off, float v) {
+    __builtin_amdgcn_raw_buffer_store_b32(__float_as_uint(v), rs, off, 0, XWG_AUX);
+}
+__device__ __forceinline__ void store_xwg(int32_t *p, int32_t v) { __hip_atomic_store(p, v, __ATOMIC_RELAXED, __HIP_MEMORY_SCOPE_AGENT); }
+__device__ __forceinline__ float4 load_xwg(__amdgpu_buffer_rsrc_t rs, int off) {
+    const u4v v = __builtin_amdgcn_raw_buffer_load_b128(rs, off, 0, XWG_AUX);
+    return make_float4(__uint_as_float(v[0]), __uint_as_float(v[1]), __uint_as_float(v[2]), __uint_as_float(v[3]));
+}
+__device__ __forceinline__ int32_t load_xwg(const int32_t *p) { return __hip_atomic_load(p, __ATOMIC_RELAXED, __HIP_MEMORY_SCOPE_AGENT); }
+
 constexpr int OREC = 4;
+
+struct ReduceArgs {
+    const float *slabs;
+    const int32_t *cnts;
+    float *G;
+    int32_t *n_k;
+    float *nk_f;
+    float *W;
+    const float *scale;
+    int32_t nblk, n_vf;
+    float alpha;
+    uint32_t apply;
+    int32_t nk_floor;
+    const int32_t *option_id;
+    int32_t *hist, *hist_zero, *perm;
+    int32_t n, nrow;
+    const float4 *outrec;
+    const float4 *qalt;
+    int32_t *invperm;
+    float *x, *y, *vx, *vy, *reward;
+    int32_t *option_id_out, *opt_steps, *ep_steps;
+    uint8_t *action, *done;
+    float *qcache;
+    int32_t sort;
+    const int32_t *fail_flag;
+    const uint8_t *c_events, *c_prev;
+    const int32_t *c_evlen, *c_count;
+    int32_t *c_rows;
+    uint32_t c_bits;
+    int32_t c_L, c_ring_len;
+};
 
 struct StepArgs {
     float *x, *y, *vx, *vy;
@@ -60,6 +108,10 @@
     int32_t max_ep, max_opt;
     uint32_t reoffer_mask;
     MapScalars ms;
+    uint32_t tail;
+    uint32_t *bar;
+    unsigned long long bar_ticks;
+    ReduceArgs R;
 };
 
 __device__ __forceinline__ void block_lds_sync() {
@@ -72,6 +124,9 @@
     return clf_z(A.clf + CLF_STRIDE * k, x, y) > 0.0f;
 }
 
+__device__ __attribute__((noinline, noreturn)) void step_tail(int b, unsigned lds_base);
+#define SCG_TAIL_LITE(i)
+
 #include "scg_eval.hpp"
 #include "scg_step_kernel.hpp"
 #include "scg_rollout_kernel.hpp"
@@ -81,37 +136,6 @@
 __attribute__((visibility("hidden"))) hipError_t launch_trial_record(const TrialRecArgs &A, int grid, hipStream_t s);
 __attribute__((visibility("hidden"))) hipError_t launch_rollout_interrupt(const RolloutIntArgs &A, int grid, hipStream_t s);
 __attribute__((visibility("hidden"))) hipError_t launch_rollout_interrupt_record(const RolloutIntRecArgs &A, int grid, hipStream_t s);
-
-struct ReduceArgs {
-    const float *slabs;
-    const int32_t *cnts;
-    float *G;
-    int32_t *n_k;
-    float *nk_f;
-    float *W;
-    const float *scale;
-    int32_t nblk, n_vf;
-    float alpha;
-    uint32_t apply;
-    int32_t nk_floor;
-    const int32_t *option_id;
-    int32_t *hist, *hist_zero, *perm;
-    int32_t n, nrow;
-    const float4 *outrec;
-    const float4 *qalt;
-    int32_t *invperm;
-    float *x, *y, *vx, *vy, *reward;
-    int32_t *option_id_out, *opt_steps, *ep_steps;
-    uint8_t *action, *done;
-    float *qcache;
-    int32_t sort;
-    const int32_t *fail_flag;
-    const uint8_t *c_events, *c_prev;
-    const int32_t *c_evlen, *c_count;
-    int32_t *c_rows;
-    uint32_t c_bits;
-    int32_t c_L, c_ring_len;
-};
 
 constexpr int SEG = 16;
 constexpr int RED_WAVES = 16;
@@ -203,10 +227,11 @@
     return pos;
 }
 
+template <bool XWG>
 __device__ __forceinline__ void commit_and_place_row(const ReduceArgs &R, int row, int wv, int lane, int (*s_x)[40]) {
     int zoff = 0;
     asm volatile("" : "+v"(zoff));
-    const int step_failed = R.fail_flag[zoff];
+    const int step_failed = XWG ? load_xwg(R.fail_flag + zoff) : R.fail_flag[zoff];
     const bool act = wv < 4 && row < R.nrow;
     const int e = row * 256 + wv * 64 + lane;
     const bool ok = act && e < R.n;
@@ -218,7 +243,7 @@
         for (int r = wv * 64 + lane; r < R.nrow; r += 256) {
 #pragma unroll
             for (int k = 0; k < NKEY; ++k) {
-                const int h = R.hist[r * HSTRIDE + k];
+                const int h = XWG ? load_xwg(&R.hist[r * HSTRIDE + k]) : R.hist[r * HSTRIDE + k];
                 tot[k] += h;
                 if (r < row) pre[k] += h;
             }
@@ -226,7 +251,16 @@
     }
     float4 ra = make_float4(0.0f, 0.0f, 0.0f, 0.0f), rb = ra, rq = ra;
     float q4 = 0.0f;
-    if (ok) {
+    if (ok && XWG) {
+        const __amdgpu_buffer_rsrc_t rs = xwg_rsrc(R.outrec), rsq = xwg_rsrc(R.qalt);
+        const int o = pos_old * (OREC * 16);
+        const float4 r3 = load_xwg(rs, o + 48);
+        ra = load_xwg(rs, o); rb = load_xwg(rs, o + 16); rq = load_xwg(rs, o + 32); q4 = r3.x;
+        if (__float_as_uint(r3.y) == OREC_DECLINED) {
+            rq = load_xwg(rsq, pos_old * 32); q4 = load_xwg(rsq, pos_old * 32 + 16).x;
+            rb.y = __uint_as_float(__float_as_uint(rb.y) | 0x01000000u);
+        }
+    } else if (ok) {
         const float4 *r = R.outrec + (size_t)pos_old * OREC;
         const float4 r3 = r[3];
         ra = r[0]; rb = r[1]; rq = r[2]; q4 = r3.x;
@@ -310,6 +344,96 @@
     if (wv == 0 && lane < HSTRIDE) R.hist_zero[row * HSTRIDE + lane] = 0;
 }
 
+template <int BATCH, bool XWG>
+__device__ __forceinline__ void reduce_columns(const ReduceArgs &R, int jx, int k, int wave, int lane, float4 (*s_T)[64], int *s_cnt) {
+    const int i4 = jx * 64 + lane;
+    const bool live = i4 < RED_COLS;
+    const size_t slab_stride = (size_t)R.n_vf * RED_COLS * sizeof(float4);
+    const char *slab_k = reinterpret_cast<const char *>(R.slabs) + (size_t)k * RED_COLS * sizeof(float4);
+    const unsigned col_off = (unsigned)(live ? i4 : 0) * (unsigned)sizeof(float4);
+    const int nseg = (R.nblk + SEG - 1) / SEG;
+    float4 S = make_float4(0.0f, 0.0f, 0.0f, 0.0f);
+    int nk = 0;
+    float4 w_old = make_float4(0.0f, 0.0f, 0.0f, 0.0f), sc = w_old;
+    int step_failed = 0;
+    for (int sg0 = 0; sg0 < nseg; sg0 += RED_WAVES * RED_SPW) {
+        int cs[RED_SPW];
+#pragma unroll
+        for (int j = 0; j < RED_SPW; ++j) {
+            const int bl = (sg0 + j * RED_WAVES + wave) * SEG + lane;
+            cs[j] = (lane < SEG && bl < R.nblk) ? (XWG ? load_xwg(&R.cnts[(unsigned)(bl * R.n_vf + k)]) : R.cnts[(unsigned)(bl * R.n_vf + k)]) : 0;
+        }
+#pragma unroll
+        for (int j = 0; j < RED_SPW; ++j) {
+            const int b0 = (sg0 + j * RED_WAVES + wave) * SEG;
+            int c = cs[j];
+            const unsigned mask = (unsigned)__ballot(c > 0);
+#pragma unroll
+            for (int m = 1; m < SEG; m <<= 1) c += __shfl_xor(c, m, 64);
+            float4 T = make_float4(0.0f, 0.0f, 0.0f, 0.0f);
+            if (mask) {
+                const __amdgpu_buffer_rsrc_t seg = __builtin_amdgcn_make_buffer_rsrc(
+                    const_cast<char *>(slab_k + (size_t)b0 * slab_stride), 0, 0x7fffffff, 0x00020000);
+#pragma unroll
+                for (int h = 0; h < SEG; h += BATCH) {
+                    if (!((mask >> h) & ((1u << BATCH) - 1u))) continue;
+                    u4v v[BATCH];
+#pragma unroll
+                    for (int u = 0; u < BATCH; ++u) {
+                        v[u] = (u4v){0u, 0u, 0u, 0u};
+                        if ((mask >> (h + u)) & 1u) v[u] = __builtin_amdgcn_raw_buffer_load_b128(seg, (int)col_off, (int)((h + u) * (unsigned)slab_stride), XWG ? XWG_AUX : 0);
+                    }
+#pragma unroll
+                    for (int u = 0; u < BATCH; ++u) {
+                        if ((mask >> (h + u)) & 1u) {
+                            T.x = T.x + __uint_as_float(v[u][0]); T.y = T.y + __uint_as_float(v[u][1]);
+                            T.z = T.z + __uint_as_float(v[u][2]); T.w = T.w + __uint_as_float(v[u][3]);
+                        }
+                    }
+                }
+            }
+            s_T[j * RED_WAVES + wave][lane] = T;
+            if (lane == 0) s_cnt[j * RED_WAVES + wave] = c;
+        }
+        if (wave == 0 && R.apply && sg0 + RED_WAVES * RED_SPW >= nseg) {
+            step_failed = XWG ? load_xwg(R.fail_flag) : *R.fail_flag;
+            int col = live ? i4 : 0;
+            asm volatile("" : "+v"(col));
+            w_old = reinterpret_cast<const float4 *>(R.W)[(size_t)k * RED_COLS + col];
+            sc = *reinterpret_cast<const float4 *>(R.scale + (col * 4) % NF);
+        }
+        __syncthreads();
+        if (wave == 0) {
+#pragma unroll
+            for (int u = 0; u < RED_WAVES * RED_SPW; ++u) {
+                const int cu = s_cnt[u];
+                if (cu > 0) {
+                    const float4 t = s_T[u][lane];
+                    S.x = S.x + t.x; S.y = S.y + t.y; S.z = S.z + t.z; S.w = S.w + t.w;
+                    nk += cu;
+                }
+            }
+        }
+        __syncthreads();
+    }
+    if (wave != 0) return;
+    if (jx == 0 && lane == 0) {
+        R.n_k[k] = nk;
+        if (R.nk_f) R.nk_f[k] = (float)nk;
+    }
+    if (!live) return;
+    reinterpret_cast<float4 *>(R.G)[(size_t)k * RED_COLS + i4] = S;
+    if (R.apply && nk > 0 && !step_failed) {
+        const float step = R.alpha / (float)max(nk, R.nk_floor);
+        float4 w = w_old;
+        w.x = fmaf(step * sc.x, S.x, w.x); w.y = fmaf(step * sc.y, S.y, w.y);
+        w.z = fmaf(step * sc.z, S.z, w.z); w.w = fmaf(step * sc.w, S.w, w.w);
+        int col = i4;
+        asm volatile("" : "+v"(col));
+        reinterpret_cast<float4 *>(R.W)[(size_t)k * RED_COLS + col] = w;
+    }
+}
+
 template <int BATCH>
 __global__ __launch_bounds__(RED_THREADS, BATCH == 16 ? 4 : 8) void reduce_kernel(const ReduceArgs R) {
     __shared__ float4 s_T[RED_WAVES * RED_SPW][64];
@@ -321,100 +445,106 @@
     const int tid = threadIdx.x, lane = tid & 63, wave = __builtin_amdgcn_readfirstlane(tid >> 6);
     if (k < 0) {
         const int row = rowy * (int)gridDim.x + blockIdx.x;
-        commit_and_place_row(R, row, wave, lane, s_x);
+        commit_and_place_row<false>(R, row, wave, lane, s_x);
         return;
     }
-    const int i4 = blockIdx.x * 64 + lane;
-    const bool live = i4 < RED_COLS;
-    const size_t slab_stride = (size_t)R.n_vf * RED_COLS * sizeof(float4);
-    const char *slab_k = reinterpret_cast<const char *>(R.slabs) + (size_t)k * RED_COLS * sizeof(float4);
-    const unsigned col_off = (unsigned)(live ? i4 : 0) * (unsigned)sizeof(float4);
-    const int nseg = (R.nblk + SEG - 1) / SEG;
-    float4 S = make_float4(0.0f, 0.0f, 0.0f, 0.0f);
-    int nk = 0;
-    float4 w_old = make_float4(0.0f, 0.0f, 0.0f, 0.0f), sc = w_old;
-    int step_failed = 0;
-    for (int sg0 = 0; sg0 < nseg; sg0 += RED_WAVES * RED_SPW) {
-        int cs[RED_SPW];
-#pragma unroll
-        for (int j = 0; j < RED_SPW; ++j) {
-            const int bl = (sg0 + j * RED_WAVES + wave) * SEG + lane;
-            cs[j] = (lane < SEG && bl < R.nblk) ? R.cnts[(unsigned)(bl * R.n_vf + k)] : 0;
-        }
-#pragma unroll
-        for (int j = 0; j < RED_SPW; ++j) {
-            const int b0 = (sg0 + j * RED_WAVES + wave) * SEG;
-            int c = cs[j];
-            const unsigned mask = (unsigned)__ballot(c > 0);
-#pragma unroll
-            for (int m = 1; m < SEG; m <<= 1) c += __shfl_xor(c, m, 64);
-            float4 T = make_float4(0.0f, 0.0f, 0.0f, 0.0f);
-            if (mask) {
-                const __amdgpu_buffer_rsrc_t seg = __builtin_amdgcn_make_buffer_rsrc(
-                    const_cast<char *>(slab_k + (size_t)b0 * slab_stride), 0, 0x7fffffff, 0x00020000);
-#pragma unroll
-                for (int h = 0; h < SEG; h += BATCH) {
-                    if (!((mask >> h) & ((1u << BATCH) - 1u))) continue;
-                    u4v v[BATCH];
-#pragma unroll
-                    for (int u = 0; u < BATCH; ++u) {
-                        v[u] = (u4v){0u, 0u, 0u, 0u};
-                        if ((mask >> (h + u)) & 1u) v[u] = __builtin_amdgcn_raw_buffer_load_b128(seg, (int)col_off, (int)((h + u) * (unsigned)slab_stride), 0);
-                    }
-#pragma unroll
-                    for (int u = 0; u < BATCH; ++u) {
-                        if ((mask >> (h + u)) & 1u) {
-                            T.x = T.x + __uint_as_float(v[u][0]); T.y = T.y + __uint_as_float(v[u][1]);
-                            T.z = T.z + __uint_as_float(v[u][2]); T.w = T.w + __uint_as_float(v[u][3]);
-                        }
-                    }
-                }
+    reduce_columns<BATCH, false>(R, (int)blockIdx.x, k, wave, lane, s_T, s_cnt);
+}
+
+constexpr uint32_t BAR_POISON = 0x80000000u, BAR_COUNT = 0xffffu;
+constexpr int BAR_TOP = 0, BAR_LEAVE = 32, BAR_GROUP = 64, BAR_GROUPS = 8, BAR_WORDS = BAR_GROUP + 32 * BAR_GROUPS;
+#ifndef SCG_TAIL_TICKS
+#define SCG_TAIL_TICKS 200000000ull
+#endif
+
+__device__ __forceinline__ int tail_barrier(uint32_t *bar, int b, int nblk, unsigned long long ticks, uint32_t *async_word) {
+    const int ng = min(nblk, BAR_GROUPS), grp = b & (BAR_GROUPS - 1);
+    const uint32_t gsize = (uint32_t)((nblk - grp + BAR_GROUPS - 1) / BAR_GROUPS);
+    uint32_t *gw = bar + BAR_GROUP + 32 * grp, *top = bar + BAR_TOP;
+#ifdef SCG_TEST_TAIL_NO_ARRIVE
+    const bool arrive = b != 1;
+#else
+    const bool arrive = true;
+#endif
+    if (arrive) {
+        const uint32_t old = __hip_atomic_fetch_add(gw, 1u, __ATOMIC_RELAXED, __HIP_MEMORY_SCOPE_AGENT);
+        if (old + 1u == gsize) {
+            __hip_atomic_store(gw, 0u, __ATOMIC_RELAXED, __HIP_MEMORY_SCOPE_AGENT);
+            __hip_atomic_fetch_add(top, 1u, __ATOMIC_RELAXED, __HIP_MEMORY_SCOPE_AGENT);
+        }
+    }
+    int res = 0;
+    unsigned spins = 0;
+    unsigned long long t0 = 0;
+    bool late = false;
+    for (;;) {
+        uint32_t v = __hip_atomic_load(top, __ATOMIC_RELAXED, __HIP_MEMORY_SCOPE_AGENT);
+        if (v & BAR_POISON) break;
+        if ((v & BAR_COUNT) >= (uint32_t)ng) { res = 1; break; }
+        if (late) {
+            if (__hip_atomic_compare_exchange_strong(top, &v, v | BAR_POISON, __ATOMIC_RELAXED, __ATOMIC_RELAXED, __HIP_MEMORY_SCOPE_AGENT)) {
+                if (async_word) __hip_atomic_fetch_or(async_word, SCG_ASYNC_TAIL_BARRIER, __ATOMIC_RELAXED, __HIP_MEMORY_SCOPE_SYSTEM);
+                break;
             }
-            s_T[j * RED_WAVES + wave][lane] = T;
-            if (lane == 0) s_cnt[j * RED_WAVES + wave] = c;
-        }
-        if (wave == 0 && R.apply && sg0 + RED_WAVES * RED_SPW >= nseg) {
-            step_failed = *R.fail_flag;
-            int col = live ? i4 : 0;
-            asm volatile("" : "+v"(col));
-            w_old = reinterpret_cast<const float4 *>(R.W)[(size_t)k * RED_COLS + col];
-            sc = *reinterpret_cast<const float4 *>(R.scale + (col * 4) % NF);
-        }
+            continue;
+        }
+        __builtin_amdgcn_s_sleep(1);
+        if ((++spins & 63u) == 0u) {
+            const unsigned long long now = __builtin_amdgcn_s_memrealtime();
+            if (t0 == 0) t0 = now;
+            else if (now - t0 > ticks) late = true;
+        }
+    }
+#ifdef SCG_TEST_TAIL_NO_ARRIVE
+    if (!arrive) {
+        const uint32_t old = __hip_atomic_fetch_add(gw, 1u, __ATOMIC_RELAXED, __HIP_MEMORY_SCOPE_AGENT);
+        if (old + 1u == gsize) {
+            __hip_atomic_store(gw, 0u, __ATOMIC_RELAXED, __HIP_MEMORY_SCOPE_AGENT);
+            __hip_atomic_fetch_add(top, 1u, __ATOMIC_RELAXED, __HIP_MEMORY_SCOPE_AGENT);
+        }
+    }
+#endif
+    if (__hip_atomic_fetch_add(bar + BAR_LEAVE, 1u, __ATOMIC_RELAXED, __HIP_MEMORY_SCOPE_AGENT) + 1u == (uint32_t)nblk) {
+        __hip_atomic_store(top, 0u, __ATOMIC_RELAXED, __HIP_MEMORY_SCOPE_AGENT);
+        __hip_atomic_store(bar + BAR_LEAVE, 0u, __ATOMIC_RELAXED, __HIP_MEMORY_SCOPE_AGENT);
+    }
+    return res;
+}
+
+struct TailLds {
+    float4 T[RED_WAVES * RED_SPW][64];
+    int cnt[RED_WAVES * RED_SPW];
+    int x[4][40];
+    int go;
+};
+
+__device__ __attribute__((noinline, noreturn)) void step_tail(int b, unsigned lds_base) {
+    StepArgs A;
+    __builtin_memcpy(&A, (const __attribute__((address_space(4))) void *)__builtin_amdgcn_kernarg_segment_ptr(), sizeof(A));
+    const ReduceArgs &R = A.R;
+    TailLds *L = (TailLds *)(__attribute__((address_space(3))) char *)(size_t)lds_base;
+    const int tid = threadIdx.x, lane = tid & 63, wave = __builtin_amdgcn_readfirstlane(tid >> 6);
+    const int nblk = (int)gridDim.x;
+    SCG_TAIL_LITE(0);
+    asm volatile("s_waitcnt vmcnt(0) lgkmcnt(0)\n\ts_barrier" ::: "memory");
+    if (tid == 0) L->go = tail_barrier(A.bar, b, nblk, A.bar_ticks, A.async_word);
+    __syncthreads();
+    const int go = L->go;
+    SCG_TAIL_LITE(1);
+    if (!go) __builtin_amdgcn_endpgm();
+    if (b < R.nrow) commit_and_place_row<true>(R, b, wave, lane, L->x);
+    const int njobs = RED_NCOL * R.n_vf;
+    for (int j = b; j < njobs; j += nblk) {
         __syncthreads();
-        if (wave == 0) {
-#pragma unroll
-            for (int u = 0; u < RED_WAVES * RED_SPW; ++u) {
-                const int cu = s_cnt[u];
-                if (cu > 0) {
-                    const float4 t = s_T[u][lane];
-                    S.x = S.x + t.x; S.y = S.y + t.y; S.z = S.z + t.z; S.w = S.w + t.w;
-                    nk += cu;
-                }
-            }
-        }
-        __syncthreads();
-    }
-    if (wave != 0) return;
-    if (blockIdx.x == 0 && lane == 0) {
-        R.n_k[k] = nk;
-        if (R.nk_f) R.nk_f[k] = (float)nk;
-    }
-    if (!live) return;
-    reinterpret_cast<float4 *>(R.G)[(size_t)k * RED_COLS + i4] = S;
-    if (R.apply && nk > 0 && !step_failed) {
-        const float step = R.alpha / (float)max(nk, R.nk_floor);
-        float4 w = w_old;
-        w.x = fmaf(step * sc.x, S.x, w.x); w.y = fmaf(step * sc.y, S.y, w.y);
-        w.z = fmaf(step * sc.z, S.z, w.z); w.w = fmaf(step * sc.w, S.w, w.w);
-        int col = i4;
-        asm volatile("" : "+v"(col));
-        reinterpret_cast<float4 *>(R.W)[(size_t)k * RED_COLS + col] = w;
-    }
+        reduce_columns<16, true>(R, j % RED_NCOL, j / RED_NCOL, wave, lane, L->T, L->cnt);
+    }
+    SCG_TAIL_LITE(2);
+    __builtin_amdgcn_endpgm();
 }
 
 __global__ __launch_bounds__(256) void commit_kernel(const ReduceArgs R) {
     __shared__ int s_x[4][40];
-    commit_and_place_row(R, blockIdx.x, threadIdx.x >> 6, threadIdx.x & 63, s_x);
+    commit_and_place_row<false>(R, blockIdx.x, threadIdx.x >> 6, threadIdx.x & 63, s_x);
 }
 
 __global__ __launch_bounds__(256) void apply_kernel(float *W, const float *G, const int32_t *n_k, const float *nk_f,
@@ -985,6 +1115,11 @@
     uint32_t *h_async;
     uint32_t *d_async;
     int32_t *d_fail;
+    uint32_t *d_bar;
+    bool tail_ok;
+    bool tail_on;
+    int last_step_launches;
+    int last_step_tail;
     double fit_timeout_s;
     float4 *d_outrec;
     float4 *d_qalt;
@@ -1052,6 +1187,10 @@
             snprintf(buf, n, "an earlier scg_step gave up inside a workgroup: a bounded hand-off poll between its wavefront subsets ran "
                      "out (a logic error or a hung wavefront); the block's partial gradients were dropped and the step's outputs for "
                      "its envs are unspecified — restore the state. scg_clear_async_error() re-arms the context");
+        else if (word & SCG_ASYNC_TAIL_BARRIER)
+            snprintf(buf, n, "an earlier scg_step gave up at the grid barrier in front of its reduce tail: a workgroup of the step kernel "
+                     "did not arrive within the bound (card shared with other work?); no workgroup ran the tail — nothing was committed, "
+                     "the weights and the env order are unchanged. scg_clear_async_error() re-arms the context");
         else if (word & SCG_ASYNC_PEER_TIMEOUT)
             snprintf(buf, n, "an earlier scg_peer_exchange_apply gave up: the peer wait ran out (a peer rank did not publish its "
                      "operand within the peer timeout: stopped, hung or out of step); the weights were left unchanged. "
@@ -1120,8 +1259,25 @@
     if (c->d_fail) {
         DeviceGuard g(c->cfg.device);
         if (g.ok) (void)hipMemset(c->d_fail, 0, sizeof(int32_t));
+        if (g.ok && c->d_bar) (void)hipMemset(c->d_bar, 0, BAR_WORDS * sizeof(uint32_t));
     }
     c->order_valid = false; c->hist_dirty = true; c->arm_rows_ready = false;
+    return SCG_OK;
+}
+
+int scg_set_fused_tail(scg_ctx *c, int32_t on) {
+    if (!c) return fail(nullptr, SCG_ERR_INVALID, "scg_set_fused_tail: null ctx");
+    if (on && !c->tail_ok)
+        return fail(c, SCG_ERR_STATE, "scg_set_fused_tail: the step kernel's workgroups of this context are not resident at once "
+                                      "(more workgroups than the card holds): the reduce launch stays");
+    c->tail_on = on != 0;
+    return SCG_OK;
+}
+
+int scg_last_step_launches(scg_ctx *c, int32_t *launches, int32_t *tail) {
+    if (!c) return fail(nullptr, SCG_ERR_INVALID, "scg_last_step_launches: null ctx");
+    if (launches) *launches = c->last_step_launches;
+    if (tail) *tail = c->last_step_tail;
     return SCG_OK;
 }
 
@@ -1204,6 +1360,15 @@
         *c->h_async = 0u;
         if (hipHostGetDevicePointer(reinterpret_cast<void **>(&c->d_async), c->h_async, 0) != hipSuccess) { st = SCG_ERR_HIP; break; }
         if (hipMalloc(&c->d_fail, sizeof(int32_t)) != hipSuccess || hipMemset(c->d_fail, 0, sizeof(int32_t)) != hipSuccess) { st = SCG_ERR_HIP; break; }
+        if (hipMalloc(&c->d_bar, BAR_WORDS * sizeof(uint32_t)) != hipSuccess || hipMemset(c->d_bar, 0, BAR_WORDS * sizeof(uint32_t)) != hipSuccess) { st = SCG_ERR_HIP; break; }
+        {
+            int per_cu = 0;
+            if (hipOccupancyMaxActiveBlocksPerMultiprocessor(&per_cu, td_kernel<MODE_FUSED_INT>, THREADS, 0) != hipSuccess) { per_cu = 0; (void)hipGetLastError(); }
+            c->tail_ok = per_cu > 0 && (long long)c->nblk <= (long long)per_cu * c->n_cu && c->nblk <= (int)BAR_COUNT &&
+                         (long long)c->nblk * BLOCK_ENVS * OREC * 16 < (1ll << 31);
+            const char *ev = getenv("SCG_FUSED_TAIL");
+            c->tail_on = c->tail_ok && ev && atoi(ev) != 0;
+        }
         if (hipMalloc(&c->d_outrec, (size_t)c->nblk * BLOCK_ENVS * OREC * sizeof(float4)) != hipSuccess) { st = SCG_ERR_HIP; break; }
         if (hipMalloc(&c->d_qalt, (size_t)c->nblk * BLOCK_ENVS * 2 * sizeof(float4)) != hipSuccess) { st = SCG_ERR_HIP; break; }
         if (hipMalloc(&c->d_invperm, (size_t)c->nblk * BLOCK_ENVS * sizeof(int32_t)) != hipSuccess) { st = SCG_ERR_HIP; break; }
@@ -1240,7 +1405,7 @@
     (void)hipFree(c->d_slabs); (void)hipFree(c->d_cnts); (void)hipFree(c->d_G); (void)hipFree(c->d_nk);
     (void)hipFree(c->d_hist2[0]); (void)hipFree(c->d_hist2[1]); (void)hipFree(c->d_outrec); (void)hipFree(c->d_qalt); (void)hipFree(c->d_invperm);
     (void)hipFree(c->d_edges); (void)hipFree(c->d_starts); (void)hipFree(c->d_scale); (void)hipFree(c->d_cellmask); (void)hipFree(c->d_perm); (void)hipFree(c->d_hist);
-    (void)hipFree(c->d_fit_part); (void)hipFree(c->d_collect_rows); (void)hipFree(c->d_frontier_rows); (void)hipFree(c->d_fail);
+    (void)hipFree(c->d_fit_part); (void)hipFree(c->d_collect_rows); (void)hipFree(c->d_frontier_rows); (void)hipFree(c->d_fail); (void)hipFree(c->d_bar);
     if (c->h_async) (void)hipHostFree(c->h_async);
     if (c->peer_region) {
         DeviceGuard g(c->cfg.device);
@@ -1348,9 +1513,7 @@
     A.async_word = c->d_async; A.fail_flag = c->d_fail;
 }
 
-static int launch_reduce(scg_ctx *c, float *W, uint32_t apply, int nblk, hipStream_t s,
-                         const StepArgs *st = nullptr, bool sort = false, bool reduce = true) {
-    ReduceArgs R;
+static void fill_reduce(scg_ctx *c, ReduceArgs &R, float *W, uint32_t apply, int nblk, const StepArgs *st, bool sort) {
     memset(&R, 0, sizeof(R));
     R.slabs = c->d_slabs; R.cnts = c->d_cnts; R.G = c->G_out; R.n_k = c->nk_out; R.nk_f = c->nkf_out; R.W = W; R.scale = c->d_scale;
     R.nblk = nblk; R.n_vf = c->n_vf; R.alpha = c->cfg.alpha; R.apply = apply; R.fail_flag = c->d_fail; R.nk_floor = c->cfg.update_count_floor;
@@ -1368,6 +1531,14 @@
             R.c_rows = c->d_collect_rows; R.c_bits = c->arm_bits; R.c_L = c->arm_L; R.c_ring_len = c->ring_len;
         }
     }
+}
+
+static int launch_reduce(scg_ctx *c, float *W, uint32_t apply, int nblk, hipStream_t s,
+                         const StepArgs *st = nullptr, bool sort = false, bool reduce = true) {
+    ReduceArgs R;
+    fill_reduce(c, R, W, apply, nblk, st, sort);
+    const int nrow = R.nrow;
+    c->last_step_launches += 1;
     if (!reduce) {
         hipLaunchKernelGGL(commit_kernel, dim3(nrow), dim3(256), 0, s, R);
         SCG_HIP(c, hipGetLastError());
@@ -1419,7 +1590,10 @@
     A.k_lo = 0; A.k_hi = c->n_vf - 1;
     A.enabled = enabled_mask; A.learn = (flags & SCG_STEP_LEARN) ? 1u : 0u; A.t = t;
     if (flags & 0x100u) A.k_hi = -1;
-    if (!(c->order_valid && c->order_ids == option_id)) {
+    c->last_step_launches = 1; c->last_step_tail = 0;
+    const bool sorted_already = c->order_valid && c->order_ids == option_id;
+    if (!sorted_already) {
+        c->last_step_launches += 2;
         const int nrow = (c->cfg.n_envs + 255) / 256;
         hipLaunchKernelGGL(sort_hist_kernel, dim3(nrow), dim3(256), 0, s, option_id, c->cfg.n_envs, c->n_vf, c->d_hist);
         hipLaunchKernelGGL(sort_scatter_kernel, dim3(nrow), dim3(256), 0, s, option_id, c->cfg.n_envs, c->n_vf, nrow,
@@ -1436,6 +1610,13 @@
     const bool fold = (flags & SCG_STEP_LEARN) && !(flags & 0x200u);
     A.hist_next = fold ? c->d_hist2[c->hist_parity] : nullptr;
     A.perm = c->d_perm; A.outrec = c->d_outrec; A.qalt = c->d_qalt;
+    const bool tail = c->tail_on && fold && (flags & SCG_STEP_APPLY) && sorted_already && !c->peer_n && !c->nkf_out &&
+                      !(c->arm_bits && c->events && c->ring_x) && A.k_hi >= 0;
+    if (tail) {
+        A.tail = 1u; A.bar = c->d_bar; A.bar_ticks = SCG_TAIL_TICKS;
+        fill_reduce(c, A.R, W, 1u, c->nblk, &A, true);
+        c->hist_dirty = true;
+    }
     hipEvent_t ev0 = nullptr, ev1 = nullptr;
     if (c->prof_on && (c->prof_seen++ % c->prof_every) == c->prof_every / 2) {
         if (!c->prof_ev) c->prof_ev = new std::vector<hipEvent_t>();
@@ -1455,6 +1636,13 @@
     SCG_HIP(c, hipGetLastError());
     if (ev1) SCG_HIP(c, hipEventRecord(ev1, s));
     c->arm_rows_ready = c->arm_bits && c->events && c->ring_x;
+    if (tail) {
+        c->last_step_tail = 1;
+        c->hist_dirty = false;
+        c->hist_parity ^= 1;
+        c->order_valid = true; c->order_ids = option_id;
+        return SCG_OK;
+    }
     if (!(flags & SCG_STEP_LEARN)) return launch_reduce(c, W, 0u, c->nblk, s, &A, false, false);
     PeerTarget peer_target(c);
     if (!fold) return launch_reduce(c, W, (flags & SCG_STEP_APPLY) ? 1u : 0u, c->nblk, s, &A, false);
diff --git a/skill-chaining-with-graphs_amd/csrc/scg_step_kernel.hpp b/skill-chaining-with-graphs_amd/csrc/scg_step_kernel.hpp
--- a/skill-chaining-with-graphs_amd/csrc/scg_step_kernel.hpp
+++ b/skill-chaining-with-graphs_amd/csrc/scg_step_kernel.hpp
@@ -468,11 +468,11 @@
                 s_r0[i] = rew; s_c0[i] = dn ? 0.0f : A.gamma; s_ro[i] = ro; s_co[i] = co;
                 {
                     const int osn = keep ? osteps + 1 : 0, epn = dn ? 0 : eps1;
-                    float4 *orec = A.outrec + (size_t)(e0 + i) * OREC;
-                    orec[0] = make_float4(nx, ny, nvx, nvy);
-                    orec[1] = make_float4(rew, __uint_as_float((unsigned)a | ((unsigned)dn << 8) | ((unsigned)on << 16) | ((unsigned)stay << 28)),
-                                          __int_as_float(osn), __int_as_float(epn));
-                    reinterpret_cast<float *>(orec + 3)[1] = 0.0f;
+                    const __amdgpu_buffer_rsrc_t ors = xwg_rsrc(A.outrec + (size_t)e0 * OREC);
+                    store_xwg(ors, i * 64, make_float4(nx, ny, nvx, nvy));
+                    store_xwg(ors, i * 64 + 16, make_float4(rew, __uint_as_float((unsigned)a | ((unsigned)dn << 8) | ((unsigned)on << 16) | ((unsigned)stay << 28)),
+                                                            __int_as_float(osn), __int_as_float(epn)));
+                    store_xwg(ors, i * 64 + 52, 0.0f);
                 }
                 if (A.ring_x) {
                     const size_t row = (size_t)(ep0 & A.ring_mask) * N + e;
@@ -592,7 +592,7 @@
     unsigned single = (FUSED && A.k_hi >= 0) ? (updm & present & ~1u & ~(kB >= 1 ? 1u << kB : 0u)) : 0u;
     const unsigned eval_only = (FUSED && A.k_hi >= 0) ? (present & ~updm & ~1u & ~(kB >= 1 ? 1u << kB : 0u)) : 0u;
     if (FUSED && tid < A.n_vf && A.cnts && tid != 0 && tid != kB && !((single >> tid) & 1u))
-        A.cnts[(size_t)b * A.n_vf + tid] = 0;
+        store_xwg(&A.cnts[(size_t)b * A.n_vf + tid], 0);
     const int n_pass0 = A.k_hi >= A.k_lo ? 1 : 0;
     const unsigned single0 = single;
     auto gate = [&](int kdec) {
@@ -608,7 +608,7 @@
         const float rm = (kdec >= 0 || single0 != 0u) ? s_qsa[BLOCK_ENVS + ti] : s_maxq[ti];
         if (cm >= rm) return;
         s_on[ti] = 0;
-        reinterpret_cast<float *>(A.outrec + (size_t)(e0 + ti) * OREC + 3)[1] = __uint_as_float(OREC_DECLINED);
+        store_xwg(xwg_rsrc(A.outrec + (size_t)e0 * OREC), ti * 64 + 52, __uint_as_float(OREC_DECLINED));
         if (A.hist_next) {
             const int e = A.perm ? A.perm[e0 + ti] : e0 + ti;
             atomicAdd(&A.hist_next[(e >> 8) * 8 + cand], -1);
@@ -626,10 +626,10 @@
             const float mo = kdec < 0 ? s_maxq[BLOCK_ENVS + ti] : s_maxq[ti];
             const float m0 = kdec < 0 ? s_maxq[ti] : s_qsa[BLOCK_ENVS + ti];
             if (mo >= m0) return;
-            float *rec = reinterpret_cast<float *>(A.outrec + (size_t)(e0 + ti) * OREC);
-            rec[5] = __uint_as_float((unsigned)s_a[ti] | ((s_ic[ti] & 7u) << 16));
-            rec[6] = __int_as_float(0);
-            rec[13] = __uint_as_float(OREC_DECLINED);
+            const __amdgpu_buffer_rsrc_t ors = xwg_rsrc(A.outrec + (size_t)e0 * OREC);
+            store_xwg(ors, ti * 64 + 20, __uint_as_float((unsigned)s_a[ti] | ((s_ic[ti] & 7u) << 16)));
+            store_xwg(ors, ti * 64 + 24, __int_as_float(0));
+            store_xwg(ors, ti * 64 + 52, __uint_as_float(OREC_DECLINED));
             if (A.hist_next) {
                 const int e = A.perm ? A.perm[e0 + ti] : e0 + ti;
                 atomicAdd(&A.hist_next[(e >> 8) * 8 + o], -1);
@@ -638,7 +638,7 @@
         }
     };
     const bool blk_fail = FUSED && __builtin_amdgcn_readfirstlane(s_misc[M_FAIL]) != 0;
-    if (blk_fail && tid < A.n_vf && A.cnts) A.cnts[(size_t)b * A.n_vf + tid] = 0;
+    if (blk_fail && tid < A.n_vf && A.cnts) store_xwg(&A.cnts[(size_t)b * A.n_vf + tid], 0);
     for (int pass = 0; pass < n_pass0 + MAX_VF && !blk_fail; ++pass) {
         int lane_p;
         asm volatile("v_mbcnt_lo_u32_b32 %0, -1, 0\n\tv_mbcnt_hi_u32_b32 %0, -1, %0" : "=v"(lane_p));
@@ -787,8 +787,8 @@
         }
         block_lds_sync();
         if (tid == 0 && A.cnts) {
-            A.cnts[(size_t)b * A.n_vf + kA] = nupd;
-            if (kBp >= 1) A.cnts[(size_t)b * A.n_vf + kBp] = nupdB;
+            store_xwg(&A.cnts[(size_t)b * A.n_vf + kA], nupd);
+            if (kBp >= 1) store_xwg(&A.cnts[(size_t)b * A.n_vf + kBp], nupdB);
         }
         if (pass == 0) SCG_LITE(4);
         const int npg = dense ? (nb + 7) >> 3 : 0;
@@ -836,9 +836,9 @@
                 asm volatile("" : "+v"(n16o), "+v"(go));
                 contract_mem<EO_TG>(A.W + (size_t)kg * NACT * NF, B, qo, n16o, go, ab_lane);
                 if (out_lane && have) {
-                    float4 *orec = A.outrec + (size_t)(e0 + il) * OREC;
-                    orec[2] = make_float4(qo[0], qo[1], qo[2], qo[3]);
-                    orec[3].x = qo[4];
+                    const __amdgpu_buffer_rsrc_t ors = xwg_rsrc(A.outrec + (size_t)e0 * OREC);
+                    store_xwg(ors, il * 64 + 32, make_float4(qo[0], qo[1], qo[2], qo[3]));
+                    store_xwg(ors, il * 64 + 48, qo[4]);
                     float mx = qo[0];
 #pragma unroll
                     for (int a = 1; a < NACT; ++a) mx = fmaxf(mx, qo[a]);
@@ -858,14 +858,14 @@
                         bool alt = kv == 0 && (s_ia[il] & IA_ENTERING);
                         if constexpr (INT) alt = alt || (kv == 0 && (s_ic[il] & IC_KEEP));
                         if (alt) {
-                            float4 *qa = A.qalt + (size_t)(e0 + il) * 2;
-                            qa[0] = make_float4(qo[0], qo[1], qo[2], qo[3]);
-                            qa[1].x = qo[4];
+                            const __amdgpu_buffer_rsrc_t qrs = xwg_rsrc(A.qalt + (size_t)e0 * 2);
+                            store_xwg(qrs, il * 32, make_float4(qo[0], qo[1], qo[2], qo[3]));
+                            store_xwg(qrs, il * 32 + 16, qo[4]);
                         }
                         if (s_on[il] == kv) {
-                            float4 *orec = A.outrec + (size_t)(e0 + il) * OREC;
-                            orec[2] = make_float4(qo[0], qo[1], qo[2], qo[3]);
-                            orec[3].x = qo[4];
+                            const __amdgpu_buffer_rsrc_t ors = xwg_rsrc(A.outrec + (size_t)e0 * OREC);
+                            store_xwg(ors, il * 64 + 32, make_float4(qo[0], qo[1], qo[2], qo[3]));
+                            store_xwg(ors, il * 64 + 48, qo[4]);
                         }
                     } else if (s_on[il] == kv) {
 #pragma unroll
@@ -1071,8 +1071,8 @@
                 }
             }
         } else if (tid == 0 && A.cnts) {
-            A.cnts[(size_t)b * A.n_vf + kA] = 0;
-            if (kBp >= 1) A.cnts[(size_t)b * A.n_vf + kBp] = 0;
+            store_xwg(&A.cnts[(size_t)b * A.n_vf + kA], 0);
+            if (kBp >= 1) store_xwg(&A.cnts[(size_t)b * A.n_vf + kBp], 0);
         }
         if (pass == 0) SCG_LITE(7);
         if (pass > 0) gate(kA);
@@ -1103,4 +1103,7 @@
         reinterpret_cast<unsigned *>(A.stamps + (size_t)blockIdx.x * STAMP_SLOTS + 34)[wave] = hwid;
     }
 #endif
+    if constexpr (FUSED) {
+        if (A.tail) step_tail(b, (unsigned)(size_t)(const __attribute__((address_space(3))) void *)smem);
+    }
 }
```

New measurement: 585.7 million. -30.4%, worse.
